# kronbichler/multigrid

Measured on AMD Instinct MI355X. Metric: DoFs/s for Laplace matvec + V-cycle, poisson_cube p=4 fp64, higher is better.
Workload: dtype f64; 1 GPU; poisson_cube FE_Q(4) 128^3 cells, 135005697 DoFs per GPU, 8 levels, step = 1 fp64 vmult + 1 V-cycle (Chebyshev degree 3, first kind); cells_per_dim=128, degree=4, n_dofs_per_gpu=135005697, global_dofs=135005697, parallelism=1 GPU

## Files before the change

### include/mgx.h

```cpp
#ifndef MGX_H
#define MGX_H

#include <stddef.h>
#include <stdint.h>

#ifdef __cplusplus
extern "C" {
#endif

#define MGX_OK 0
#define MGX_ERR_INVALID_ARGUMENT (-1)
#define MGX_ERR_NO_DEVICE (-2)
#define MGX_ERR_HIP (-3)
#define MGX_ERR_UNSUPPORTED (-4)
#define MGX_ERR_NOT_CONVERGED (-5)

#define MGX_F32 0
#define MGX_F64 1

#define MGX_INVALID_INDEX 0xFFFFFFFFu
#define MGX_MAX_DEGREE 9

typedef struct mgx_context_s  *mgx_context_t;
typedef struct mgx_operator_s *mgx_operator_t;
// ... 12 lines not shown
int mgx_device_memory_info(mgx_context_t ctx, size_t *free_bytes, size_t *total_bytes);
void *mgx_context_stream(mgx_context_t ctx);

typedef struct
{
  int   rank, size;
  void *user;
  int (*exchange)(void *user, int plan_id, int number, int n_neighbors, const int *ranks, const uint32_t *counts,
                  void *const *send, void *const *recv);
  int (*allreduce_sum)(void *user, double *values, int count);
  void *(*alloc_device)(void *user, size_t bytes);
} mgx_comm_desc;
int mgx_context_set_comm(mgx_context_t ctx, const mgx_comm_desc *comm);

#define MGX_RCCL_ID_BYTES 128
int mgx_rccl_unique_id(void *id_out);
int mgx_context_set_rccl(mgx_context_t ctx, int rank, int size, const void *id);
int mgx_context_use_rccl(mgx_context_t ctx, int enable);

typedef struct
{
  int                    plan_id;
  int                    n_neighbors;
  const int             *neighbor_rank;
  const uint32_t        *count;
  const uint32_t *const *index;
  const uint32_t        *shared;
  uint32_t               n_shared;
  const uint32_t        *not_owned;
  uint32_t               n_not_owned;
  void *const           *send_buf;
  void *const           *recv_buf;
} mgx_exchange_desc;

int mgx_profile_enable(mgx_context_t ctx, int enable);
int mgx_range_push(mgx_context_t ctx, const char *name);
int mgx_range_pop(mgx_context_t ctx);
int mgx_profile_read(mgx_context_t ctx, int form, uint64_t *launches, double *total_ms);

int mgx_malloc(mgx_context_t ctx, void **dptr, size_t bytes);
int mgx_free(mgx_context_t ctx, void *dptr);
int mgx_upload(mgx_context_t ctx, void *dptr, const void *hptr, size_t bytes);
int mgx_download(mgx_context_t ctx, void *hptr, const void *dptr, size_t bytes);
int mgx_memset_zero(mgx_context_t ctx, void *dptr, size_t bytes);
int mgx_copy_device(mgx_context_t ctx, void *dst, const void *src, size_t bytes);

int mgx_copy_cast(mgx_context_t ctx, void *dst, int dst_number, const void *src, int src_number, size_t n);
int mgx_add_cast(mgx_context_t ctx, void *dst, int dst_number, const void *src, int src_number, size_t n);
int mgx_sadd(mgx_context_t ctx, int number, void *x, double s, double a, const void *v, size_t n);
int mgx_dot(mgx_context_t ctx, int number, const void *x, const void *y, size_t n, double *result);
int mgx_l2_norm(mgx_context_t ctx, int number, const void *x, size_t n, double *result);
int mgx_operator_dot(mgx_operator_t op, const void *x, const void *y, double *result);
int mgx_operator_l2_norm(mgx_operator_t op, const void *x, double *result);
int mgx_set_entries(mgx_context_t ctx, int number, void *v, const uint32_t *idx_host,
                    const double *val_host, uint32_t count);

typedef struct
{
  int      degree;
  int      number;
  uint32_t n_cells;
  uint32_t n_dofs;
  const uint32_t *idx27;
  const uint32_t *idx27_plain;
  const uint32_t *constrained;
  uint32_t        n_constrained;
  double coef[6];
  const double *shape_values;
  const double *colloc_grad;
  const double *qweights;
  const uint8_t *brick_colour;
  const uint32_t *global_index;
  const mgx_exchange_desc *exchange;
  const double *coef_q;
} mgx_operator_desc;

int mgx_operator_create(mgx_context_t ctx, const mgx_operator_desc *desc, mgx_operator_t *op);
int mgx_operator_destroy(mgx_operator_t op);
uint32_t mgx_operator_n_dofs(mgx_operator_t op);
int mgx_operator_set_profiled(mgx_operator_t op, int profiled);
int mgx_operator_exchange_buffers(mgx_operator_t op, int k, void **send, void **recv, uint32_t *count, int *rank);
int mgx_exchange_add(mgx_operator_t op, void *vec);
int mgx_operator_number(mgx_operator_t op);
int mgx_vmult(mgx_operator_t op, void *dst, const void *src);
int mgx_compute_residual(mgx_operator_t op, void *dst, const void *src, const void *rhs_q);
int mgx_vmult_residual(mgx_operator_t op, const void *rhs, const void *lhs, void *residual);
int mgx_vmult_with_cg_update(mgx_operator_t op, double alpha, double beta, const void *r, void *q, void *p, void *x,
                             void *scratch, double sums[4]);
int mgx_compute_diagonal(mgx_operator_t op);
int mgx_get_inverse_diagonal(mgx_operator_t op, const void **dptr);

#define MGX_LAW_UNIT 0
#define MGX_LAW_MINIMAL_SURFACE 1
int mgx_operator_enable_coefficient_update(mgx_operator_t op, const double metric[6], double det_jacobian);
int mgx_operator_enable_coefficient_update_q(mgx_operator_t op, const double *unit_q, const double *jxw_q);
int mgx_evaluate_coefficient(mgx_operator_t op, int law, const void *state);
int mgx_compute_nonlinear_residual(mgx_operator_t op, int law, void *dst, const void *state);
int mgx_operator_get_coefficient(mgx_operator_t op, const void **dptr, size_t *n);

int mgx_smoother_create(mgx_operator_t op, double smoothing_range, int degree,
                        int eig_cg_n_iterations, mgx_smoother_t *smoother);
int mgx_smoother_destroy(mgx_smoother_t smoother);
typedef struct
{
  double lambda_min, lambda_max, theta, delta;
  int    degree, cg_iterations;
} mgx_smoother_info;
int mgx_smoother_get_info(mgx_smoother_t smoother, mgx_smoother_info *info);
#define MGX_CHEBYSHEV_FIRST_KIND 0
#define MGX_CHEBYSHEV_FOURTH_KIND 1
int mgx_smoother_set_polynomial_type(mgx_smoother_t smoother, int polynomial_type);
int mgx_smoother_vmult(mgx_smoother_t smoother, void *x, const void *b);
int mgx_smoother_step(mgx_smoother_t smoother, void *x, const void *b);

typedef struct
{
  const uint32_t *children;
  const double *prolong_1d;
  const uint8_t *weight_shift;
} mgx_transfer_desc;
int mgx_transfer_create(mgx_operator_t coarse, mgx_operator_t fine, const mgx_transfer_desc *desc,
                        mgx_transfer_t *transfer);
int mgx_transfer_destroy(mgx_transfer_t transfer);
int mgx_prolongate(mgx_transfer_t transfer, void *fine, const void *coarse, int add, int with_constraints);
int mgx_restrict_and_add(mgx_transfer_t transfer, void *coarse, const void *fine, int with_constraints);
int mgx_interpolate_to_coarse(mgx_transfer_t transfer, void *coarse, const void *fine);

typedef struct
{
  int n_levels;
  int degree_pre;
  int n_cycles;
  const mgx_operator_t *matrix;
  const mgx_operator_t *matrix_dp;
  const mgx_transfer_t *transfer;
  const mgx_transfer_t *transfer_dp;
  const double *const *rhs;
  const uint32_t *const *bc_index;
  const double *const   *bc_value;
  const uint32_t        *bc_count;
} mgx_solver_desc;

int mgx_solver_create(mgx_context_t ctx, const mgx_solver_desc *desc, mgx_solver_t *solver);
int mgx_solver_destroy(mgx_solver_t solver);
int mgx_solver_v_cycle(mgx_solver_t solver);
int mgx_solver_reset_smoother(mgx_solver_t solver, int level, double smoothing_range, int degree,
                              int eig_cg_n_iterations);
int mgx_solver_update_coefficient(mgx_solver_t solver, int law, const double *state_fine);
int mgx_solver_n_levels(mgx_solver_t solver);
int mgx_solver_get_operator(mgx_solver_t solver, int level, int fp64, mgx_operator_t *op);
int mgx_operator_device_indices(mgx_operator_t op, const uint32_t **idx27, uint32_t *n_cells, uint32_t *n_dofs,
                                int *degree);
int mgx_solver_set_polynomial_type(mgx_solver_t solver, int polynomial_type);
int mgx_solver_compute_rhs(mgx_solver_t solver, int level, const double *rhs_q);
int mgx_solver_solve(mgx_solver_t solver, int do_analyze, double *reduction_rate, double *trace);
typedef void (*mgx_level_hook)(void *user, int level, int stage);
int mgx_solver_solve_hooked(mgx_solver_t solver, int do_analyze, double *reduction_rate, double *trace,
                            mgx_level_hook hook, void *user);
int mgx_solver_solve_cg(mgx_solver_t solver, unsigned int *iterations, double *reduction_rate);
int mgx_solver_solve_cg_control(mgx_solver_t solver, unsigned int max_iterations, double abs_tol, double reduction,
                                unsigned int *iterations, double *reduction_rate);
int mgx_solver_cg_history(mgx_solver_t solver, double *history, int capacity, int *count);
int mgx_solver_vmult(mgx_solver_t solver, double *dst, const double *src);
int mgx_solver_set_agglomeration(mgx_solver_t solver, int level, mgx_solver_t coarse, const uint32_t *local_to_global,
                                 const uint8_t *owned, uint32_t n_local);
int mgx_solver_vmult_with_residual_update(mgx_solver_t solver, double *residual, double *update, double factor,
// ... 15 lines not shown
```

### multigrid_amd/__init__.py

```python
import ctypes as C
import os

import numpy as np

from . import _lib
from ._lib import F32, F64, INVALID_INDEX, MgxError, check

__all__ = ["Context", "DeviceVector", "Cube", "LaplaceOperator", "Chebyshev", "Transfer", "MultigridSolver",
           "Communicator", "process_grid", "F32", "F64", "INVALID_INDEX", "MgxError", "DGLaplaceOperator", "dg_cheby_mesh",
           "dg_box_neighbours", "dg_box_partition", "dg_partition", "DG_HERMITE", "DG_GAUSS_LOBATTO", "DG_GAUSS", "DGMultigridSolver",
           "spawn_ranks"]


def spawn_ranks(script, argv, n, one_gpu=False, grace=30.0):
    import os
    import socket
    import subprocess
    import sys
    import time
    with socket.socket() as sock:
        sock.bind(("127.0.0.1", 0))
        port = sock.getsockname()[1]
    procs = []
    for r in range(n):
# ... 441 lines not shown

    def rhs_quadrature(self, l):
        out = np.empty((self.n_cells(l), (self.degree + 1) ** 3))
        check(self.lib.mgx_cube_rhs_quadrature(self.h, l, out.ctypes.data_as(_lib.f64p)))
        return out

    def bc(self, l):
        n = self.lib.mgx_cube_bc_count(self.h, l)
        return self._arr("mgx_cube_bc_index", (n,), l), self._arr("mgx_cube_bc_value", (n,), l)

    def neighbors(self, l):
        out = []
        for k in range(self.lib.mgx_cube_n_neighbors(self.h, l)):
            n = self.lib.mgx_cube_neighbor_count(self.h, l, k)
            out.append((self.lib.mgx_cube_neighbor_rank(self.h, l, k),
                        self._arr("mgx_cube_neighbor_index", (n,), l, k)))
        return out

    def shared(self, l):
        return self._arr("mgx_cube_shared", (self.lib.mgx_cube_n_shared(self.h, l),), l)

    def not_owned(self, l):
        return self._arr("mgx_cube_not_owned", (self.lib.mgx_cube_n_not_owned(self.h, l),), l)

    def cells_per_dim3(self, l):
        a, b = (C.c_uint32 * 3)(), (C.c_uint32 * 3)()
        self.lib.mgx_cube_cells_per_dim3(self.h, l, C.byref(a), C.byref(b))
        return tuple(a), tuple(b)

    def l2_error_parts(self, l, solution):
        s = np.ascontiguousarray(solution, dtype=np.float64)
        e, v = C.c_double(), C.c_double()
        self.lib.mgx_cube_l2_error_parts(self.h, l, s.ctypes.data_as(_lib.f64p), C.byref(e), C.byref(v))
        return e.value, v.value

    def operator_desc(self, l, number=F64):
        d = _lib.OperatorDesc()
        check(self.lib.mgx_cube_operator_desc(self.h, l, number, C.byref(d)))
        return d

    def l2_error(self, l, solution):
        s = np.ascontiguousarray(solution, dtype=np.float64)
        assert s.size == self.n_dofs(l)
        return self.lib.mgx_cube_l2_error(self.h, l, s.ctypes.data_as(_lib.f64p))

    def seeded_vector(self, l, seed=42):
        out = np.empty(self.n_dofs(l))
        check(self.lib.mgx_cube_seeded_vector(self.h, l, seed, out.ctypes.data_as(_lib.f64p)))
        return out

    def affine_metric(self, l, jacobian=None):
        m, det = np.zeros(6), C.c_double()
        a = None if jacobian is None else np.ascontiguousarray(jacobian, dtype=np.float64).ravel()
        check(self.lib.mgx_cube_affine_metric(self.h, l, None if a is None else a.ctypes.data_as(_lib.f64p),
                                              m.ctypes.data_as(_lib.f64p), C.byref(det)))
        return m, det.value

    def unit_law_coefficient(self, l, jacobian=None):
        m, det = self.affine_metric(l, jacobian)
        w = self.qweights()
        jxw = (w[:, None, None] * w[None, :, None] * w[None, None, :]).ravel() * det
        return np.ascontiguousarray(np.broadcast_to(m[None, :, None] * jxw[None, None, :],
                                                    (self.n_cells(l), 6, jxw.size)))

    def dof_coordinates(self, l, jacobian=None):
        assert self.size == 1
        if self.shell is not None or (self.box_desc is not None and self.box_desc["geometry"] != "cartesian"):
            assert jacobian is None
            dofs = _cell_dofs(self.idx27_plain(l), self.degree)
            X = np.empty((self.n_dofs(l), 3))
            X[dofs.ravel()] = self.cell_nodes(l).transpose(0, 2, 1).reshape(-1, 3)
            return X
        p, g = self.degree, self.dof_grid(l).astype(np.int64)
        n = np.array(self.cells_per_dim3(l)[1], dtype=np.int64)
        G = n * p + 1
        ijk = np.stack([g % G[0], (g // G[0]) % G[1], g // (G[0] * G[1])], axis=1)
        cell = np.minimum(ijk // p, n[None, :] - 1)
        X = (cell + self.gll()[ijk - cell * p]) * self.cell_size(l)
        if jacobian is not None:
            X = X @ np.asarray(jacobian, dtype=np.float64).T
        return (-0.9 if self.box_desc is None else self.box_desc["origin"]) + X


def _cell_dofs(idx27, p):
    n = p + 1
    idx27 = np.asarray(idx27, dtype=np.int64).reshape(-1, 27)
    out = np.empty((idx27.shape[0], n, n, n), dtype=np.int64)
    code = [0 if a == 0 else (2 if a == p else 1) for a in range(n)]
    for k in range(n):
        for j in range(n):
            oz, oy = (k - 1 if code[k] == 1 else 0), (j - 1 if code[j] == 1 else 0)
            off = (p - 1 if code[j] == 1 else 1) * oz + oy
            for i in range(n):
                base = idx27[:, 9 * code[k] + 3 * code[j] + code[i]]
                out[:, k, j, i] = base + (off * (p - 1) + i - 1 if code[i] == 1 else off)
    return out.reshape(idx27.shape[0], n ** 3)


class LaplaceOperator:

    def __init__(self, ctx, desc=None, handle=None):
        self.ctx, self.lib = ctx, ctx.lib
        self.owned = handle is None
        if handle is None:
            h = C.c_void_p()
            check(self.lib.mgx_operator_create(ctx.h, C.byref(desc), C.byref(h)))
            self.h = h
        else:
            self.h = C.c_void_p(handle)
        self.number = self.lib.mgx_operator_number(self.h)

    @classmethod
    def from_cube(cls, ctx, cube, level, number=F64, coef_q=None):
        d = cube.operator_desc(level, number)
        if coef_q is not None:
            coef_q = np.ascontiguousarray(coef_q, dtype=np.float64)
            assert coef_q.size == cube.n_cells(level) * 6 * (cube.degree + 1) ** 3
            d.coef_q = coef_q.ctypes.data_as(_lib.f64p)
        return cls(ctx, d)

    def m(self):
        return self.lib.mgx_operator_n_dofs(self.h)

    def set_profiled(self, on=True):
        check(self.lib.mgx_operator_set_profiled(self.h, int(on)))

    def initialize_dof_vector(self):
        return DeviceVector(self.ctx, self.m(), self.number)

    def vmult(self, dst, src):
        check(self.lib.mgx_vmult(self.h, dst.ptr, src.ptr))

    def vmult_with_cg_update(self, alpha, beta, r, q, p, x):
        sums = np.zeros(4)
        check(self.lib.mgx_vmult_with_cg_update(self.h, alpha, beta, r.ptr, q.ptr, p.ptr, x.ptr, None,
                                                sums.ctypes.data_as(_lib.f64p)))
        return sums

    def vmult_residual(self, rhs, lhs, residual):
        check(self.lib.mgx_vmult_residual(self.h, rhs.ptr, lhs.ptr, residual.ptr))

    def compute_residual(self, dst, src=None, rhs_q=None):
        check(self.lib.mgx_compute_residual(self.h, dst.ptr, src.ptr if src is not None else None,
                                            rhs_q.ptr if rhs_q is not None else None))

    def compute_diagonal(self):
        check(self.lib.mgx_compute_diagonal(self.h))

    def enable_coefficient_update(self, metric, det_jacobian):
        m = np.ascontiguousarray(metric, dtype=np.float64)
        assert m.size == 6
        check(self.lib.mgx_operator_enable_coefficient_update(self.h, m.ctypes.data_as(_lib.f64p), float(det_jacobian)))

    def enable_coefficient_update_q(self, unit_q, jxw_q):
        u = np.ascontiguousarray(unit_q, dtype=np.float64)
        w = np.ascontiguousarray(jxw_q, dtype=np.float64)
        p, n = C.c_void_p(), C.c_size_t()
        check(self.lib.mgx_operator_get_coefficient(self.h, C.byref(p), C.byref(n)))
        assert u.size == n.value and 6 * w.size == n.value
        check(self.lib.mgx_operator_enable_coefficient_update_q(self.h, u.ctypes.data_as(_lib.f64p),
                                                                w.ctypes.data_as(_lib.f64p)))

    def evaluate_coefficient(self, law, state):
        check(self.lib.mgx_evaluate_coefficient(self.h, int(law), state.ptr))

    def compute_nonlinear_residual(self, law, dst, state):
        check(self.lib.mgx_compute_nonlinear_residual(self.h, int(law), dst.ptr, state.ptr))

    def get_coefficient(self):
        p, n = C.c_void_p(), C.c_size_t()
        check(self.lib.mgx_operator_get_coefficient(self.h, C.byref(p), C.byref(n)))
        return DeviceVector(self.ctx, n.value, self.number, ptr=p)

    def l2_norm(self, x):
        r = C.c_double()
        check(self.lib.mgx_operator_l2_norm(self.h, x.ptr, C.byref(r)))
        return r.value

    def get_matrix_diagonal_inverse(self):
        p = C.c_void_p()
        check(self.lib.mgx_get_inverse_diagonal(self.h, C.byref(p)))
        return DeviceVector(self.ctx, self.m(), self.number, ptr=p)

    def clear(self):
        if self.owned and self.h:
            self.lib.mgx_operator_destroy(self.h)
            self.h = None


class Chebyshev:

    POLYNOMIAL = {"first_kind": 0, "fourth_kind": 1}

    def __init__(self, op, smoothing_range=20., degree=3, eig_cg_n_iterations=15, handle=None, polynomial=None):
        self.op, self.lib = op, op.lib
        self.owned = handle is None
        if handle is None:
            h = C.c_void_p()
            check(self.lib.mgx_smoother_create(op.h, smoothing_range, degree, eig_cg_n_iterations, C.byref(h)))
            self.h = h
        else:
            self.h = C.c_void_p(handle)
        if polynomial is not None:
            self.set_polynomial_type(polynomial)

# ... 555 lines not shown
```

### multigrid_amd/_lib.py

```python
import ctypes as C
import os

_HERE = os.path.dirname(os.path.abspath(__file__))
LIB_PATH = os.environ.get("MGX_LIB_PATH") or os.path.join(_HERE, "libmgx.so")

F32, F64 = 0, 1
INVALID_INDEX = 0xFFFFFFFF

vp = C.c_void_p
u32p = C.POINTER(C.c_uint32)
f64p = C.POINTER(C.c_double)


class ExchangeDesc(C.Structure):
    _fields_ = [("plan_id", C.c_int), ("n_neighbors", C.c_int), ("neighbor_rank", C.POINTER(C.c_int)),
                ("count", u32p), ("index", C.POINTER(u32p)), ("shared", u32p), ("n_shared", C.c_uint32),
                ("not_owned", u32p), ("n_not_owned", C.c_uint32), ("send_buf", C.POINTER(vp)),
                ("recv_buf", C.POINTER(vp))]


EXCHANGE_FN = C.CFUNCTYPE(C.c_int, vp, C.c_int, C.c_int, C.c_int, C.POINTER(C.c_int), u32p, C.POINTER(vp), C.POINTER(vp))
ALLREDUCE_FN = C.CFUNCTYPE(C.c_int, vp, f64p, C.c_int)
ALLOC_FN = C.CFUNCTYPE(vp, vp, C.c_size_t)
LEVEL_HOOK_FN = C.CFUNCTYPE(None, vp, C.c_int, C.c_int)
# ... 15 lines not shown
                ("idx27", u32p), ("idx27_plain", u32p), ("constrained", u32p), ("n_constrained", C.c_uint32),
                ("coef", C.c_double * 6), ("shape_values", f64p), ("colloc_grad", f64p), ("qweights", f64p),
                ("brick_colour", C.POINTER(C.c_uint8)), ("global_index", u32p),
                ("exchange", C.POINTER(ExchangeDesc)), ("coef_q", f64p)]


class DGExchangeDesc(C.Structure):
    _fields_ = [("plan_id", C.c_int), ("n_neighbors", C.c_int), ("neighbor_rank", C.POINTER(C.c_int)),
                ("count", u32p), ("send_cells", C.POINTER(u32p)), ("recv_first", u32p)]


class DGOperatorDesc(C.Structure):
    _fields_ = [("degree", C.c_int), ("basis", C.c_int), ("number", C.c_int), ("n_cells", C.c_uint32),
                ("neighbours", C.POINTER(C.c_int32)), ("jacobian", C.c_double * 9),
                ("n_ghost_cells", C.c_uint32), ("exchange", C.POINTER(DGExchangeDesc))]


class DGSolverDesc(C.Structure):
    _fields_ = [("matrix_dg", vp), ("matrix_dg_dp", vp), ("cfe", vp), ("degree_pre", C.c_int),
                ("cell_global_id", u32p)]


class SmootherInfo(C.Structure):
    _fields_ = [("lambda_min", C.c_double), ("lambda_max", C.c_double), ("theta", C.c_double),
                ("delta", C.c_double), ("degree", C.c_int), ("cg_iterations", C.c_int)]


class TransferDesc(C.Structure):
    _fields_ = [("children", u32p), ("prolong_1d", f64p), ("weight_shift", C.POINTER(C.c_uint8))]


class SolverDesc(C.Structure):
    _fields_ = [("n_levels", C.c_int), ("degree_pre", C.c_int), ("n_cycles", C.c_int),
                ("matrix", C.POINTER(vp)), ("matrix_dp", C.POINTER(vp)),
                ("transfer", C.POINTER(vp)), ("transfer_dp", C.POINTER(vp)),
                ("rhs", C.POINTER(f64p)), ("bc_index", C.POINTER(u32p)), ("bc_value", C.POINTER(f64p)),
                ("bc_count", u32p)]


class CubeSolver(C.Structure):
    _fields_ = [("n_levels", C.c_int), ("matrix", C.POINTER(vp)), ("matrix_dp", C.POINTER(vp)),
                ("transfer", C.POINTER(vp)), ("transfer_dp", C.POINTER(vp)), ("solver", vp)]


SIGNATURES = {
    "mgx_last_error": (C.c_char_p, []),
    "mgx_version": (C.c_char_p, []),
    "mgx_context_create": (C.c_int, [C.POINTER(vp), C.c_int]),
    "mgx_context_set_option": (C.c_int, [vp, C.c_char_p, C.c_double]),
    "mgx_has_cells_form": (C.c_int, []),
    "mgx_context_destroy": (C.c_int, [vp]),
    "mgx_sync": (C.c_int, [vp]),
    "mgx_device_memory_info": (C.c_int, [vp, C.POINTER(C.c_size_t), C.POINTER(C.c_size_t)]),
    "mgx_context_stream": (vp, [vp]),
    "mgx_context_set_comm": (C.c_int, [vp, C.POINTER(CommDesc)]),
    "mgx_rccl_unique_id": (C.c_int, [vp]),
    "mgx_context_set_rccl": (C.c_int, [vp, C.c_int, C.c_int, vp]),
    "mgx_context_use_rccl": (C.c_int, [vp, C.c_int]),
    "mgx_copy_device": (C.c_int, [vp, vp, vp, C.c_size_t]),
    "mgx_operator_exchange_buffers": (C.c_int, [vp, C.c_int, C.POINTER(vp), C.POINTER(vp), u32p, C.POINTER(C.c_int)]),
    "mgx_exchange_add": (C.c_int, [vp, vp]),
    "mgx_profile_enable": (C.c_int, [vp, C.c_int]),
    "mgx_range_push": (C.c_int, [vp, C.c_char_p]),
    "mgx_range_pop": (C.c_int, [vp]),
    "mgx_profile_read": (C.c_int, [vp, C.c_int, C.POINTER(C.c_uint64), f64p]),
    "mgx_operator_set_profiled": (C.c_int, [vp, C.c_int]),
    "mgx_malloc": (C.c_int, [vp, C.POINTER(vp), C.c_size_t]),
    "mgx_free": (C.c_int, [vp, vp]),
    "mgx_upload": (C.c_int, [vp, vp, vp, C.c_size_t]),
    "mgx_download": (C.c_int, [vp, vp, vp, C.c_size_t]),
    "mgx_memset_zero": (C.c_int, [vp, vp, C.c_size_t]),
    "mgx_copy_cast": (C.c_int, [vp, vp, C.c_int, vp, C.c_int, C.c_size_t]),
    "mgx_add_cast": (C.c_int, [vp, vp, C.c_int, vp, C.c_int, C.c_size_t]),
    "mgx_sadd": (C.c_int, [vp, C.c_int, vp, C.c_double, C.c_double, vp, C.c_size_t]),
    "mgx_dot": (C.c_int, [vp, C.c_int, vp, vp, C.c_size_t, f64p]),
    "mgx_l2_norm": (C.c_int, [vp, C.c_int, vp, C.c_size_t, f64p]),
    "mgx_operator_dot": (C.c_int, [vp, vp, vp, f64p]),
    "mgx_operator_l2_norm": (C.c_int, [vp, vp, f64p]),
    "mgx_set_entries": (C.c_int, [vp, C.c_int, vp, u32p, f64p, C.c_uint32]),
    "mgx_operator_create": (C.c_int, [vp, C.POINTER(OperatorDesc), C.POINTER(vp)]),
    "mgx_operator_destroy": (C.c_int, [vp]),
    "mgx_operator_n_dofs": (C.c_uint32, [vp]),
    "mgx_operator_number": (C.c_int, [vp]),
    "mgx_vmult": (C.c_int, [vp, vp, vp]),
    "mgx_vmult_residual": (C.c_int, [vp, vp, vp, vp]),
    "mgx_compute_diagonal": (C.c_int, [vp]),
    "mgx_get_inverse_diagonal": (C.c_int, [vp, C.POINTER(vp)]),
    "mgx_smoother_create": (C.c_int, [vp, C.c_double, C.c_int, C.c_int, C.POINTER(vp)]),
    "mgx_smoother_destroy": (C.c_int, [vp]),
    "mgx_smoother_get_info": (C.c_int, [vp, C.POINTER(SmootherInfo)]),
    "mgx_smoother_vmult": (C.c_int, [vp, vp, vp]),
    "mgx_smoother_step": (C.c_int, [vp, vp, vp]),
    "mgx_transfer_create": (C.c_int, [vp, vp, C.POINTER(TransferDesc), C.POINTER(vp)]),
    "mgx_transfer_destroy": (C.c_int, [vp]),
    "mgx_prolongate": (C.c_int, [vp, vp, vp, C.c_int, C.c_int]),
    "mgx_restrict_and_add": (C.c_int, [vp, vp, vp, C.c_int]),
    "mgx_solver_create": (C.c_int, [vp, C.POINTER(SolverDesc), C.POINTER(vp)]),
    "mgx_solver_destroy": (C.c_int, [vp]),
    "mgx_solver_solve": (C.c_int, [vp, C.c_int, f64p, f64p]),
    "mgx_solver_solve_hooked": (C.c_int, [vp, C.c_int, f64p, f64p, LEVEL_HOOK_FN, vp]),
    "mgx_solver_solve_cg": (C.c_int, [vp, C.POINTER(C.c_uint), f64p]),
    "mgx_solver_cg_history": (C.c_int, [vp, f64p, C.c_int, C.POINTER(C.c_int)]),
    "mgx_solver_solve_cg_fused": (C.c_int, [vp, C.POINTER(C.c_uint), f64p]),
    "mgx_solver_vmult_with_residual_update": (C.c_int, [vp, vp, vp, C.c_double, f64p]),
    "mgx_vmult_with_cg_update": (C.c_int, [vp, C.c_double, C.c_double, vp, vp, vp, vp, vp, f64p]),
    "mgx_solver_vmult": (C.c_int, [vp, vp, vp]),
    "mgx_solver_do_matvec": (C.c_int, [vp]),
    "mgx_solver_do_matvec_smoother": (C.c_int, [vp]),
    "mgx_solver_get_solution": (C.c_int, [vp, C.c_int, C.c_int, C.POINTER(vp)]),
    "mgx_solver_get_vector": (C.c_int, [vp, C.c_int, C.c_int, C.POINTER(vp)]),
    "mgx_solver_get_smoother": (C.c_int, [vp, C.c_int, C.POINTER(vp)]),
    "mgx_solver_get_timings": (C.c_int, [vp, f64p]),
    "mgx_solver_enable_timings": (C.c_int, [vp, C.c_int]),
    "mgx_cube_create": (C.c_int, [C.c_int, C.c_int, C.c_int, C.POINTER(vp)]),
    "mgx_cube_create_numbered": (C.c_int, [C.c_int, C.c_int, C.c_int, C.c_int, C.POINTER(vp)]),
    "mgx_cube_create_box": (C.c_int, [C.POINTER(CubeBoxDesc), C.POINTER(vp)]),
    "mgx_cube_create_shell": (C.c_int, [C.c_int, C.c_int, C.c_int, C.c_int, C.POINTER(vp)]),
    "mgx_cube_create_shell_ranks": (C.c_int, [C.c_int, C.c_int, C.c_int, C.c_int, C.c_int, C.c_int, C.POINTER(vp)]),
    "mgx_cube_level_offset": (C.c_int, [vp]),
    "mgx_cube_cell_nodes": (C.c_int, [vp, C.c_int, f64p]),
    "mgx_cube_entity_multiplicity": (C.POINTER(C.c_uint8), [vp, C.c_int]),
    "mgx_cube_rank": (C.c_int, [vp]),
    "mgx_cube_size": (C.c_int, [vp]),
    "mgx_cube_cells_per_dim3": (None, [vp, C.c_int, C.POINTER(C.c_uint32 * 3), C.POINTER(C.c_uint32 * 3)]),
    "mgx_cube_n_neighbors": (C.c_int, [vp, C.c_int]),
    "mgx_cube_neighbor_rank": (C.c_int, [vp, C.c_int, C.c_int]),
    "mgx_cube_neighbor_count": (C.c_uint32, [vp, C.c_int, C.c_int]),
    "mgx_cube_neighbor_index": (u32p, [vp, C.c_int, C.c_int]),
    "mgx_cube_n_shared": (C.c_uint32, [vp, C.c_int]),
    "mgx_cube_shared": (u32p, [vp, C.c_int]),
    "mgx_cube_n_not_owned": (C.c_uint32, [vp, C.c_int]),
    "mgx_cube_not_owned": (u32p, [vp, C.c_int]),
    "mgx_cube_weight_shift": (C.POINTER(C.c_uint8), [vp, C.c_int]),
    "mgx_cube_exchange_desc": (C.c_int, [vp, C.c_int, C.c_int, C.POINTER(ExchangeDesc), C.POINTER(u32p),
                                        C.POINTER(C.c_int), u32p]),
    "mgx_cube_l2_error_parts": (None, [vp, C.c_int, f64p, f64p, f64p]),
    "mgx_cube_destroy": (C.c_int, [vp]),
    "mgx_cube_n_levels": (C.c_int, [vp]),
    "mgx_cube_degree": (C.c_int, [vp]),
    "mgx_cube_n_cells": (C.c_uint32, [vp, C.c_int]),
    "mgx_cube_n_dofs": (C.c_uint32, [vp, C.c_int]),
    "mgx_cube_n_constrained": (C.c_uint32, [vp, C.c_int]),
    "mgx_cube_cells_per_dim": (C.c_uint32, [vp, C.c_int]),
    "mgx_cube_cell_size": (C.c_double, [vp, C.c_int]),
    "mgx_cube_idx27": (u32p, [vp, C.c_int]),
    "mgx_cube_idx27_plain": (u32p, [vp, C.c_int]),
    "mgx_cube_constrained": (u32p, [vp, C.c_int]),
    "mgx_cube_children": (u32p, [vp, C.c_int]),
    "mgx_cube_cell_coords": (u32p, [vp, C.c_int]),
    "mgx_cube_dof_grid": (u32p, [vp, C.c_int]),
    "mgx_cube_shape_values": (f64p, [vp]),
    "mgx_cube_colloc_grad": (f64p, [vp]),
    "mgx_cube_qweights": (f64p, [vp]),
    "mgx_cube_qpoints": (f64p, [vp]),
    "mgx_cube_gll": (f64p, [vp]),
    "mgx_cube_prolong_1d": (f64p, [vp]),
    "mgx_cube_rhs": (f64p, [vp, C.c_int]),
    "mgx_cube_coef_q": (f64p, [vp, C.c_int]),
    "mgx_cube_jxw_q": (f64p, [vp, C.c_int]),
    "mgx_cube_bc_count": (C.c_uint32, [vp, C.c_int]),
    "mgx_cube_bc_index": (u32p, [vp, C.c_int]),
    "mgx_cube_bc_value": (f64p, [vp, C.c_int]),
    "mgx_cube_operator_desc": (C.c_int, [vp, C.c_int, C.c_int, C.POINTER(OperatorDesc)]),
    "mgx_cube_l2_error": (C.c_double, [vp, C.c_int, f64p]),
    "mgx_cube_seeded_vector": (C.c_int, [vp, C.c_int, C.c_uint64, f64p]),
    "mgx_cube_solver_create": (C.c_int, [vp, vp, C.c_int, C.c_int, C.c_int, C.POINTER(CubeSolver)]),
# ... 78 lines not shown
```

### multigrid_amd/csrc/mgx_api.cpp

```cpp
#include "../../include/mgx.h"
#include "mgx_bricks.hpp"
#include "mgx_internal.hpp"

#include <hip/hip_runtime.h>
#include <rccl/rccl.h>

#include <dlfcn.h>

#include <algorithm>
#include <chrono>
#include <cmath>
#include <cstdio>
#include <cstdlib>
#include <cstring>
#include <memory>
#include <string>
#include <type_traits>
#include <utility>
#include <vector>

using namespace mgx;

namespace
{
// ... 23 lines not shown
        return s_;        \
    }                     \
  while (0)

#define MGX_REQUIRE(cond, msg)                        \
  do                                                  \
    {                                                 \
      if (!(cond))                                    \
        return fail(MGX_ERR_INVALID_ARGUMENT, (msg)); \
    }                                                 \
  while (0)

  inline size_t number_size(int number) { return number == MGX_F64 ? 8 : 4; }

  bool g_trace = false;
  bool trace_on() { return g_trace; }
#define MGX_TRACE(...)                  \
  do                                    \
    {                                   \
      if (trace_on())                   \
        {                               \
          std::fprintf(stderr, "[mgx] " __VA_ARGS__); \
          std::fputc('\n', stderr);     \
          std::fflush(stderr);          \
        }                               \
    }                                   \
  while (0)
}

int mgx::report_error(int code, const char *message) { return fail(code, message ? message : ""); }

#ifndef MGX_CELLS_FORM
#define MGX_CELLS_FORM 0
#endif
extern "C" int mgx_has_cells_form(void) { return MGX_CELLS_FORM; }

mgx::Tunables mgx::Tunables::from_environment()
{
  Tunables t;
  auto     num = [](const char *name, uint32_t dflt) {
    const char *e = std::getenv(name);
    return e ? (uint32_t)std::strtoul(e, nullptr, 10) : dflt;
  };
  t.trace               = std::getenv("MGX_TRACE") != nullptr;
  t.brick_min           = num("MGX_BRICK_MIN", t.brick_min);
  t.brick_min_from_env  = std::getenv("MGX_BRICK_MIN") != nullptr;
  t.overlap_min         = num("MGX_OVERLAP_MIN_BRICKS", t.overlap_min);
  t.restrict_colour_min = num("MGX_RESTRICT_COLOUR_MIN", t.restrict_colour_min);
  t.cell_colour_min     = num("MGX_CELL_COLOUR_MIN", t.cell_colour_min);
  t.free_max_bricks     = num("MGX_FREE_MAX_BRICKS", t.free_max_bricks);
  t.free_one_max        = num("MGX_FREE_ONE_MAX", t.free_one_max);
  t.graph_max_dofs      = num("MGX_GRAPH_MAX_DOFS", t.graph_max_dofs);
  return t;
}

bool mgx::Tunables::set(const std::string &name, double value)
{
  const bool     on = value != 0.;
  const uint32_t u  = value <= 0. ? 0u : (value >= 4294967295. ? 0xFFFFFFFFu : (uint32_t)value);
  struct Entry
  {
    const char *name;
    bool       *flag;
    uint32_t   *number;
  };
  const Entry table[] = {
    {"trace", &trace, nullptr},
    {"brick_min", nullptr, &brick_min},
    {"overlap_min_bricks", nullptr, &overlap_min},
    {"restrict_colour_min", nullptr, &restrict_colour_min},
    {"cell_colour_min", nullptr, &cell_colour_min},
    {"free_max_bricks", nullptr, &free_max_bricks},
    {"free_one_max", nullptr, &free_one_max},
    {"graph_max_dofs", nullptr, &graph_max_dofs},
    {"general_kernel", &general_kernel, nullptr},
    {"no_bricks", &no_bricks, nullptr},
#if MGX_CELLS_FORM
    {"cells_form", &cells_form, nullptr},
    {"brick_wide_max", nullptr, &wide_max},
#endif
    {"macro_wg_per_cu_x16", nullptr, &macro_wg_x16},
    {"no_diag_table", &no_diag_table, nullptr},
    {"no_macro_v2", &no_macro_v2, nullptr},
    {"no_general_bricks", &no_general_bricks, nullptr},
    {"general_brick_min", nullptr, &general_brick_min},
    {"fused_prolong_min_bricks", nullptr, &fused_prolong_min_bricks},
    {"roctx", &roctx, nullptr},
    {"no_fused_init", &no_fused_init, nullptr},
    {"no_fused_restrict", &no_fused_restrict, nullptr},
    {"no_fused_prolong", &no_fused_prolong, nullptr},
    {"force_fused_transfers", &force_fused_transfers, nullptr},
    {"transfer_v1", &transfer_v1, nullptr},
    {"restrict_atomic", &restrict_atomic, nullptr},
    {"exchange_unfused", &exchange_unfused, nullptr},
    {"no_graph", &no_graph, nullptr},
    {"dg_no_overlap", &dg_no_overlap, nullptr},
    {"dg_unmerged_restrict", &dg_unmerged_restrict, nullptr},
    {"no_fused_decomposed", &no_fused_decomposed, nullptr},
    {"no_fused_assembly", &no_fused_assembly, nullptr},
    {"no_fused_residual", &no_fused_residual, nullptr},
    {"no_restrict_scratch", &no_restrict_scratch, nullptr},
    {"rccl_selftest", &rccl_selftest, nullptr},
  };
  for (const Entry &e : table)
    if (name == e.name)
      {
        if (e.flag)
          *e.flag = on;
        else
          *e.number = u;
        if (name == "brick_min")
          brick_min_from_env = true;
        return true;
      }
  return false;
}

struct ExchangePlan
{
  std::vector<uint32_t> not_owned_host;
  int                    plan_id = 0, number = MGX_F64, self_pos = 0;
  std::vector<int>       rank;
  std::vector<uint32_t>  count;
  std::vector<uint32_t *> index_dev;
  std::vector<void *>    send, recv;
  std::vector<uint8_t>   owns_buffers;
  uint32_t              *shared_dev = nullptr, *not_owned_dev = nullptr;
  uint32_t               n_shared = 0, n_not_owned = 0;
  void                  *own_buf = nullptr;
  std::vector<uint32_t>  start;
  uint32_t              *all_index_dev = nullptr, *csr_start_dev = nullptr, *csr_pos_dev = nullptr;
  uint8_t               *all_seg_dev = nullptr, *csr_k_dev = nullptr;
  bool                   fused = false;
};

struct RcclApi
{
  void *lib = nullptr;
  decltype(&ncclGetUniqueId)    GetUniqueId    = nullptr;
  decltype(&ncclCommInitRank)   CommInitRank   = nullptr;
  decltype(&ncclCommDestroy)    CommDestroy    = nullptr;
  decltype(&ncclGroupStart)     GroupStart     = nullptr;
  decltype(&ncclGroupEnd)       GroupEnd       = nullptr;
  decltype(&ncclSend)           Send           = nullptr;
  decltype(&ncclRecv)           Recv           = nullptr;
  decltype(&ncclAllReduce)      AllReduce      = nullptr;
  decltype(&ncclGetErrorString) GetErrorString = nullptr;
  bool load()
  {
    if (lib)
      return true;
    const char *names[] = {"librccl.so", "librccl.so.1", "/opt/rocm/lib/librccl.so.1"};
    for (const char *n : names)
      if ((lib = dlopen(n, RTLD_NOW | RTLD_NOLOAD)))
        break;
    if (!lib)
      for (const char *n : names)
        if ((lib = dlopen(n, RTLD_NOW | RTLD_GLOBAL)))
          break;
    if (!lib)
      return false;
#define MGX_RCCL_SYM(name)                                        \
  name = reinterpret_cast<decltype(name)>(dlsym(lib, "nccl" #name)); \
  if (!name)                                                      \
    {                                                             \
      lib = nullptr;                                              \
// ... 1113 lines not shown
              const int inner = (e % 3 == 1) + ((e / 3) % 3 == 1) + (e / 9 == 1);
              if (inner == 3 || (inner > 0 && pm1 == 0) || ix[e] == MGX_INVALID_INDEX)
                continue;
              mask |= used[ix[e]];
            }
          int col = 0;
          while (col < 32 && (mask >> col) & 1u)
            ++col;
          if (col == 32)
            {
              ok = false;
              break;
            }
          colour[c] = (uint8_t)col;
          ++count[col];
          n_colours = std::max(n_colours, col + 1);
          for (int e = 0; e < 27; ++e)
            {
              const int inner = (e % 3 == 1) + ((e / 3) % 3 == 1) + (e / 9 == 1);
              if (inner == 3 || (inner > 0 && pm1 == 0) || ix[e] == MGX_INVALID_INDEX)
                continue;
              used[ix[e]] |= 1u << col;
            }
        }
      if (ok)
        {
          std::vector<uint32_t> order(desc->n_cells), fill(33, 0);
          d.cell_colour_start[0] = 0;
          for (int k = 0; k < n_colours; ++k)
            d.cell_colour_start[k + 1] = d.cell_colour_start[k] + count[k];
          for (int k = 0; k < n_colours; ++k)
            fill[k] = d.cell_colour_start[k];
          for (uint32_t c = 0; c < desc->n_cells; ++c)
            order[fill[colour[c]]++] = c;
          d.n_cell_colours = n_colours;
          MGX_HIP(hipMalloc((void **)&d.cell_order, sizeof(uint32_t) * (size_t)desc->n_cells));
          MGX_HIP(hipMemcpy(d.cell_order, order.data(), sizeof(uint32_t) * (size_t)desc->n_cells, hipMemcpyHostToDevice));
          MGX_TRACE("operator_create: general branch, %u cells in %d colours", desc->n_cells, n_colours);
        }
    }
  const bool macro_covers = d.separable && (uint64_t)desc->n_dofs * number_size(d.number) < 0xFFFFFFF0ull;
  if (!tun.no_bricks && !general && (MGX_CELLS_FORM ? (p <= 4 || d.separable) : macro_covers))
    {
      BrickHost   bh;
      std::string why;
      const mgx_exchange_desc *ex = desc->exchange;
      const uint32_t brick_min   = tun.brick_min_from_env ? tun.brick_min : (p <= 2 ? 2 * tun.brick_min : tun.brick_min);
      const uint32_t brick_cells = p <= 4 ? 64u : 8u;
      const uint32_t overlap_min = tun.overlap_min;
      if (desc->n_dofs >= 0x3FFFFFFFu)
        MGX_TRACE("operator_create: per-cell kernel (%u DoFs do not fit the 30-bit entity index)", desc->n_dofs);
      else if (desc->n_cells / brick_cells < brick_min)
        MGX_TRACE("operator_create: per-cell kernel (%u bricks < %u)", desc->n_cells / brick_cells, brick_min);
      else if (build_bricks(p, desc->n_cells, desc->n_dofs, desc->idx27, desc->idx27_plain, desc->brick_colour,
                            ex ? ex->shared : nullptr, ex ? ex->n_shared : 0,
                            ex && desc->n_cells / brick_cells >= overlap_min, bh, why))
        {
          BrickData &b = d.bricks;
          b.n_bricks   = bh.n_bricks;
          b.n_colours  = bh.n_colours;
          b.n_iface_groups = bh.n_iface_groups;
          b.order      = bh.order;
          for (int c = 0; c <= bh.n_colours; ++c)
            b.colour_start[c] = bh.colour_start[c];
          for (size_t i = 0; i < bh.ent_base.size(); ++i)
            if (bh.ent_base[i] != MGX_INVALID_INDEX)
              bh.ent_base[i] |= (uint32_t)(bh.ent_flags[i] & 3u) << 30;
          MGX_HIP(hipMalloc((void **)&b.ent_base, sizeof(uint32_t) * bh.ent_base.size()));
          MGX_HIP(hipMemcpy(b.ent_base, bh.ent_base.data(), sizeof(uint32_t) * bh.ent_base.size(),
                            hipMemcpyHostToDevice));
          b.ent_flags = nullptr;
          if (d.separable)
            {
              std::vector<uint32_t> map;
              build_item_map(p, map);
              MGX_HIP(hipMalloc((void **)&b.item_map, sizeof(uint32_t) * map.size()));
              MGX_HIP(hipMemcpy(b.item_map, map.data(), sizeof(uint32_t) * map.size(), hipMemcpyHostToDevice));
              {
                std::vector<uint32_t> map2;
                build_item_map2(p, map2);
                MGX_HIP(hipMalloc((void **)&b.item_map2, sizeof(uint32_t) * map2.size()));
                MGX_HIP(hipMemcpy(b.item_map2, map2.data(), sizeof(uint32_t) * map2.size(), hipMemcpyHostToDevice));
              }
              const int n_classes = b.n_bricks <= tun.free_one_max ? 1 : 2;
              FreeHost  fh;
              if (!MGX_MACRO_PAIRS && !tun.cells_form && b.n_bricks <= tun.free_max_bricks &&
                  (uint64_t)desc->n_dofs * number_size(d.number) < 0xFFFFFFF0ull &&
                  build_free_schedule(p, bh, desc->n_dofs, ex ? ex->shared : nullptr, ex ? ex->n_shared : 0,
                                      bh.n_iface_groups > 0, n_classes, map, fh) &&
                  (size_t)b.n_bricks * fh.n_surf * number_size(d.number) < 0xFFFFFFF0ull && fh.n_groups <= 8)
                {
                  FreeSchedule &fr  = b.fr;
                  fr.n_classes      = n_classes;
                  fr.n_groups       = fh.n_groups;
                  fr.n_iface_groups = fh.n_iface_groups;
                  for (int g = 0; g <= fh.n_groups; ++g)
                    fr.group_start[g] = fh.group_start[g];
                  fr.n_surf        = fh.n_surf;
                  fr.n_surf_dofs   = (uint32_t)fh.surf_dof.size();
                  fr.n_surf_shared = fh.n_surf_shared;
                  fh.surf_dof.push_back(0);
                  fh.surf_pos.push_back(0);
                  auto up = [&](uint32_t *&dev, const std::vector<uint32_t> &v) {
                    if (hipMalloc((void **)&dev, sizeof(uint32_t) * v.size()) != hipSuccess)
                      return false;
                    return hipMemcpy(dev, v.data(), sizeof(uint32_t) * v.size(), hipMemcpyHostToDevice) == hipSuccess;
                  };
                  MGX_REQUIRE(up(fr.surf_off, fh.surf_off) && up(fr.surf_dof, fh.surf_dof) && up(fr.surf_start, fh.surf_start) &&
                                up(fr.surf_pos, fh.surf_pos),
                              "mgx_operator_create: out of device memory (reduced-colour schedule)");
                  MGX_HIP(hipMalloc(&fr.priv, (size_t)b.n_bricks * fh.n_surf * number_size(d.number) + 16));
                  MGX_REQUIRE(up(fr.ent, fh.ent), "mgx_operator_create: out of device memory (reduced-colour schedule)");
                  MGX_TRACE("operator_create: reduced-colour schedule, %d classes, %d groups, %u private values per brick, %u "
                            "private DoFs (%u shared)",
                            n_classes, fr.n_groups, fr.n_surf, fr.n_surf_dofs, fr.n_surf_shared);
                }
            }
          MGX_TRACE("operator_create: %u bricks, %d colours", b.n_bricks, b.n_colours);
        }
      else
        MGX_TRACE("operator_create: per-cell kernel (%s)", why.c_str());
    }
  if (general && p == 4 && !desc->exchange && !tun.no_bricks && !tun.no_general_bricks && desc->n_dofs < 0x3FFFFFFFu &&
      (uint64_t)desc->n_dofs * number_size(d.number) < 0xFFFFFFF0ull &&
      desc->n_cells / 64 >= tun.general_brick_min)
    {
      BrickHost   bh;
      std::string why;
      FreeHost    fh;
      std::vector<uint32_t> map;
      build_item_map(p, map);
      if (build_bricks(p, desc->n_cells, desc->n_dofs, desc->idx27, desc->idx27_plain, nullptr, nullptr, 0, false, bh, why) &&
          build_free_schedule(p, bh, desc->n_dofs, nullptr, 0, false, 1, map, fh) && fh.n_groups == 1 &&
          (size_t)bh.n_bricks * fh.n_surf * number_size(d.number) < 0xFFFFFFF0ull)
        {
          BrickData &g = d.gbricks;
          g.n_bricks   = bh.n_bricks;
          FreeSchedule &fr = g.fr;
          fr.n_classes = 1;
          fr.n_groups  = 1;
          fr.group_start[0] = 0;
          fr.group_start[1] = bh.n_bricks;
          fr.n_surf        = fh.n_surf;
          fr.n_surf_dofs   = (uint32_t)fh.surf_dof.size();
          fr.n_surf_shared = 0;
          fh.surf_dof.push_back(0);
          fh.surf_pos.push_back(0);
          auto up = [&](uint32_t *&dev, const std::vector<uint32_t> &v) {
            if (hipMalloc((void **)&dev, sizeof(uint32_t) * v.size()) != hipSuccess)
              return false;
            return hipMemcpy(dev, v.data(), sizeof(uint32_t) * v.size(), hipMemcpyHostToDevice) == hipSuccess;
          };
          MGX_REQUIRE(up(g.order_dev, bh.order) && up(g.item_map, map) && up(fr.surf_off, fh.surf_off) && up(fr.surf_dof, fh.surf_dof) &&
                        up(fr.surf_start, fh.surf_start) && up(fr.surf_pos, fh.surf_pos) && up(fr.ent, fh.ent),
                      "mgx_operator_create: out of device memory (brick schedule of the general operator)");
          MGX_HIP(hipMalloc(&fr.priv, (size_t)bh.n_bricks * fh.n_surf * number_size(d.number) + 16));
          MGX_TRACE("operator_create: general branch on %u bricks, %u private values per brick, %u private DoFs", bh.n_bricks,
                    fr.n_surf, fr.n_surf_dofs);
        }
      else
        MGX_TRACE("operator_create: general branch without bricks (%s)", why.c_str());
    }
  {
    const size_t     n3 = (size_t)n * n * n, n_local = n3 * desc->n_cells;
    if (!d.bricks.available() && !d.cell_order && n_local <= kAssemblyMaxEntries)
      {
// ... 158 lines not shown
                  }
                cnt[j]++;
              }
          if (ok)
            {
              std::vector<uint32_t> cs(e.n_shared + 1, 0);
              for (uint32_t j = 0; j < e.n_shared; ++j)
                cs[j + 1] = cs[j] + cnt[j] + 1;
              std::vector<uint8_t>  ck(cs.back() + 1, 0);
              std::vector<uint32_t> cp(cs.back() + 1, 0), fill(cs.begin(), cs.end() - 1);
              for (int k = 0; k <= e.n_neighbors; ++k)
                {
                  if (k == P->self_pos)
                    for (uint32_t j = 0; j < e.n_shared; ++j)
                      ck[fill[j]++] = 255;
                  if (k < e.n_neighbors)
                    for (uint32_t i = 0; i < e.count[k]; ++i)
                      {
                        const uint32_t j = slot[e.index[k][i]];
                        ck[fill[j]]   = (uint8_t)k;
                        cp[fill[j]++] = i;
                      }
                }
              MGX_HIP(hipMalloc((void **)&P->all_index_dev, sizeof(uint32_t) * all_index.size()));
              MGX_HIP(hipMalloc((void **)&P->all_seg_dev, all_seg.size()));
              MGX_HIP(hipMalloc((void **)&P->csr_start_dev, sizeof(uint32_t) * cs.size()));
              MGX_HIP(hipMalloc((void **)&P->csr_k_dev, ck.size()));
              MGX_HIP(hipMalloc((void **)&P->csr_pos_dev, sizeof(uint32_t) * cp.size()));
              MGX_HIP(hipMemcpy(P->all_index_dev, all_index.data(), sizeof(uint32_t) * all_index.size(), hipMemcpyHostToDevice));
              MGX_HIP(hipMemcpy(P->all_seg_dev, all_seg.data(), all_seg.size(), hipMemcpyHostToDevice));
              MGX_HIP(hipMemcpy(P->csr_start_dev, cs.data(), sizeof(uint32_t) * cs.size(), hipMemcpyHostToDevice));
              MGX_HIP(hipMemcpy(P->csr_k_dev, ck.data(), ck.size(), hipMemcpyHostToDevice));
              MGX_HIP(hipMemcpy(P->csr_pos_dev, cp.data(), sizeof(uint32_t) * cp.size(), hipMemcpyHostToDevice));
              P->fused = true;
            }
        }
      ctx->plans.push_back({(size_t)desc->n_dofs, P.get()});
      op->plan = std::move(P);
    }
  *out = op.release();
  return MGX_OK;
}

int mgx_operator_exchange_buffers(mgx_operator_t op, int k, void **send, void **recv, uint32_t *count, int *rank)
{
  MGX_REQUIRE(op && op->plan && k >= 0 && k < (int)op->plan->rank.size(), "mgx_operator_exchange_buffers: bad argument");
  if (send)
    *send = op->plan->send[k];
  if (recv)
    *recv = op->plan->recv[k];
  if (count)
    *count = op->plan->count[k];
  if (rank)
    *rank = op->plan->rank[k];
  return MGX_OK;
}

int mgx_exchange_add(mgx_operator_t op, void *vec)
{
  MGX_REQUIRE(op && vec, "mgx_exchange_add: null argument");
  return exchange_add(op, vec);
}

int mgx_operator_destroy(mgx_operator_t op)
{
  if (!op)
    return MGX_OK;
  (void)hipStreamSynchronize(op->ctx->stream);
  (void)hipFree(op->d.idx27);
  (void)hipFree(op->d.idx27_plain);
  (void)hipFree(op->d.constrained);
  (void)hipFree(op->d.basis);
  (void)hipFree(op->d.inv_diag);
  (void)hipFree(op->d.coef_q);
  (void)hipFree(op->d.grad_1d);
  (void)hipFree(op->d.cell_order);
  (void)hipFree(op->d.asm_start);
  (void)hipFree(op->d.asm_pos);
  (void)hipFree(op->d.cell_scratch);
  (void)hipFree(op->d.bricks.ent_base);
  (void)hipFree(op->d.bricks.ent_flags);
  (void)hipFree(op->d.bricks.item_map);
  (void)hipFree(op->d.bricks.item_map2);
  (void)hipFree(op->d.bricks.fr.ent);
  (void)hipFree(op->d.bricks.fr.surf_off);
  (void)hipFree(op->d.bricks.fr.priv);
  (void)hipFree(op->d.bricks.fr.surf_dof);
  (void)hipFree(op->d.bricks.fr.surf_start);
  (void)hipFree(op->d.bricks.fr.surf_pos);
  (void)hipFree(op->d.gbricks.item_map);
  (void)hipFree(op->d.gbricks.order_dev);
  (void)hipFree(op->d.gbricks.fr.ent);
  (void)hipFree(op->d.gbricks.fr.surf_off);
  (void)hipFree(op->d.gbricks.fr.priv);
  (void)hipFree(op->d.gbricks.fr.surf_dof);
  (void)hipFree(op->d.gbricks.fr.surf_start);
  (void)hipFree(op->d.gbricks.fr.surf_pos);
  (void)hipFree(op->d.diag_items);
  (void)hipFree(op->d.diag_items2);
  (void)hipFree(op->cg_partials);
  (void)hipFree(op->cg_result);
  (void)hipFree(op->cg_carrier);
  (void)hipFree(op->unit_q);
  (void)hipFree(op->jxw_q);
  (void)hipFree(op->global_index_dev);
  if (op->plan)
    {
      ExchangePlan *P = op->plan.get();
      auto         &v = op->ctx->plans;
      v.erase(std::remove_if(v.begin(), v.end(), [P](const std::pair<size_t, ExchangePlan *> &x) { return x.second == P; }),
              v.end());
      for (size_t k = 0; k < P->rank.size(); ++k)
        {
          (void)hipFree(P->index_dev[k]);
          if (P->owns_buffers[k])
            {
              (void)hipFree(P->send[k]);
              (void)hipFree(P->recv[k]);
            }
        }
      (void)hipFree(P->shared_dev);
      (void)hipFree(P->not_owned_dev);
      (void)hipFree(P->own_buf);
      (void)hipFree(P->all_index_dev);
      (void)hipFree(P->all_seg_dev);
      (void)hipFree(P->csr_start_dev);
      (void)hipFree(P->csr_k_dev);
      (void)hipFree(P->csr_pos_dev);
    }
  delete op;
  return MGX_OK;
}

uint32_t mgx_operator_n_dofs(mgx_operator_t op) { return op ? op->d.n_dofs : 0; }

int mgx_operator_set_profiled(mgx_operator_t op, int profiled)
{
  MGX_REQUIRE(op, "mgx_operator_set_profiled: null operator");
  op->profiled = profiled != 0;
  return MGX_OK;
}
int      mgx_operator_number(mgx_operator_t op) { return op ? op->d.number : -1; }

int mgx_vmult(mgx_operator_t op, void *dst, const void *src)
{
  MGX_REQUIRE(op && dst && src, "mgx_vmult: null argument");
  MGX_REQUIRE(dst != src, "mgx_vmult: dst and src must not alias (laplace_operator.h:573-601)");
  hipStream_t s = op->ctx->stream;
  bool identity_done = false;
  MGX_TRY(apply_plain(op, dst, src, true, &identity_done));
  if (!identity_done)
    launch_constrained_copy(s, op->d.number, dst, src, op->d.constrained, op->d.n_constrained);
  MGX_HIP(hipGetLastError());
  return MGX_OK;
}

int mgx_vmult_residual(mgx_operator_t op, const void *rhs, const void *lhs, void *res)
{
  MGX_REQUIRE(op && rhs && lhs && res, "mgx_vmult_residual: null argument");
  MGX_REQUIRE(res != lhs && res != rhs, "mgx_vmult_residual: residual must not alias rhs/lhs");
  hipStream_t s = op->ctx->stream;
  if (op->d.bricks.available())
    {
      const bool fr = op->d.bricks.fr.available();
      MGX_TRY(brick_loop_with_exchange(
        op, 1, res,
        [&](hipStream_t st, int g0, int g1) {
          launch_brick_loop(st, op->d, 1, lhs, rhs, nullptr, res, res, 0., 0., nullptr, 0., nullptr, nullptr, g0, g1, fr);
        },
        [&](hipStream_t st) {
          launch_list_residual(st, op->d.number, res, rhs, op->plan->shared_dev, op->plan->n_shared);
        },
        fr,
        [&](hipStream_t st, uint32_t first, uint32_t count) {
          launch_surf_finish(st, op->d, 1, first, count, res, lhs, res, rhs, nullptr, nullptr, 0., 0., 0.);
        }));
    }
  else
    {
      MGX_TRY(apply_plain(op, res, lhs));
      launch_rhs_minus(s, op->d.number, res, rhs, op->d.n_dofs);
    }
  launch_constrained_residual(s, op->d.number, res, rhs, lhs, op->d.constrained, op->d.n_constrained);
  MGX_HIP(hipGetLastError());
  return MGX_OK;
}

int mgx_vmult_with_cg_update(mgx_operator_t op, double alpha, double beta, const void *r, void *q, void *p, void *x,
                             void *scratch, double sums[4])
{
  MGX_REQUIRE(op && r && q && p && x && sums, "mgx_vmult_with_cg_update: null argument");
  MGX_REQUIRE(q != p && q != x && p != x && r != q && r != p && r != x, "mgx_vmult_with_cg_update: vectors must not alias");
  mgx_context_t ctx = op->ctx;
  hipStream_t   s   = ctx->stream;
  const int     num = op->d.number;
  const size_t  n   = op->d.n_dofs;
  constexpr uint32_t kCapacity = 1u << 16;
  if (!op->cg_partials)
    {
      MGX_HIP(hipMalloc((void **)&op->cg_partials, sizeof(double) * 4 * kCapacity));
      MGX_HIP(hipMalloc((void **)&op->cg_result, sizeof(double) * 4));
    }
  bool fused = op->d.bricks.available() && op->d.separable && op->d.bricks.item_map && !op->plan;
  if (fused)
    {
      void *carrier = scratch;
      if (!carrier)
        {
          if (!op->cg_carrier)
            MGX_HIP(hipMalloc(&op->cg_carrier, number_size(num) * n));
          carrier = op->cg_carrier;
        }
      uint32_t used = 0;
      {
        ProfileBracket pb(op, 8);
        fused = num == MGX_F64 ? launch_macro_cg_update_f64(s, op->d, alpha, beta, r, q, p, x, carrier, op->cg_partials,
                                                            kCapacity - 2048, &used)
                               : launch_macro_cg_update_f32(s, op->d, alpha, beta, r, q, p, x, carrier, op->cg_partials,
                                                            kCapacity - 2048, &used);
      }
      if (fused)
        {
          used += launch_cg_list_update(s, num, op->d.constrained, op->d.n_constrained, alpha, beta, r, q, p, x,
                                        op->cg_partials + 4 * (size_t)used);
          launch_reduce4(s, op->cg_partials, used, nullptr, op->cg_result);
// ... 207 lines not shown
      MGX_HIP(hipMemsetAsync(dst, 0, number_size(op->d.number) * op->d.n_dofs, s));
      launch_cell_nl_residual(s, op->d, ms, op->metric, op->det_jacobian, op->unit_q, op->jxw_q, dst, state, op->d.cell_order, op->d.cell_colour_start,
                              op->d.n_cell_colours);
    }
  else
    return fail(MGX_ERR_UNSUPPORTED, "mgx_compute_nonlinear_residual: the level has neither cell colours nor the ordered-assembly "
                                     "tables (more than 32 colours): no reproducible assembly");
  MGX_HIP(hipGetLastError());
  return MGX_OK;
}

int mgx_compute_diagonal(mgx_operator_t op)
{
  MGX_REQUIRE(op, "mgx_compute_diagonal: null argument");
  hipStream_t s = op->ctx->stream;
  const int   n = op->d.p + 1;
  double a1d[kMaxN], m1d[kMaxN];
  for (int i = 0; i < n; ++i)
    {
      double a = 0, m = 0;
      for (int q = 0; q < n; ++q)
        {
          double g = 0;
          for (int r = 0; r < n; ++r)
            g += op->D[q * n + r] * op->S[r * n + i];
          a += op->w[q] * g * g;
          m += op->w[q] * op->S[q * n + i] * op->S[q * n + i];
        }
      a1d[i] = a;
      m1d[i] = m;
    }
  MGX_HIP(hipMemsetAsync(op->d.inv_diag, 0, number_size(op->d.number) * op->d.n_dofs, s));
  if (op->d.bricks.available())
    {
      std::vector<uint32_t> lists, list_start;
      brick_cell_lists(op, lists, list_start);
      uint32_t *lists_dev = nullptr;
      MGX_HIP(hipMalloc((void **)&lists_dev, sizeof(uint32_t) * (lists.size() + 1)));
      MGX_HIP(hipMemcpyAsync(lists_dev, lists.data(), sizeof(uint32_t) * lists.size(), hipMemcpyHostToDevice, s));
      launch_cell_diagonal(s, op->d, op->d.inv_diag, a1d, m1d, lists_dev, list_start.data(), (int)list_start.size() - 1);
      MGX_HIP(hipStreamSynchronize(s));
      MGX_HIP(hipFree(lists_dev));
    }
  else if (op->d.cell_order)
    launch_cell_diagonal(s, op->d, op->d.inv_diag, a1d, m1d, op->d.cell_order, op->d.cell_colour_start, op->d.n_cell_colours);
  else
    launch_cell_diagonal(s, op->d, op->d.inv_diag, a1d, m1d);
  MGX_TRY(exchange_add(op, op->d.inv_diag));
  launch_constrained_set(s, op->d.number, op->d.inv_diag, 1.0, op->d.constrained, op->d.n_constrained);
  launch_invert(s, op->d.number, op->d.inv_diag, op->d.n_dofs);
  MGX_HIP(hipGetLastError());
  op->has_diag = true;
  for (int which = 0; which < 2; ++which)
    {
      void          *&slot = which == 0 ? op->d.diag_items : op->d.diag_items2;
      const uint32_t *map  = which == 0 ? op->d.bricks.item_map : op->d.bricks.item_map2;
      if (slot)
        {
          MGX_HIP(hipFree(slot));
          slot = nullptr;
        }
      if (!map || !op->d.separable || op->ctx->tun.no_diag_table)
        continue;
      const uint32_t nb = op->d.p <= 4 ? 4 : 2, g = nb * op->d.p + 1, npts = g * g * g;
      void          *table = nullptr;
      uint32_t      *flag  = nullptr, mismatch = 1;
      MGX_HIP(hipMalloc(&table, number_size(op->d.number) * npts));
      MGX_HIP(hipMalloc((void **)&flag, sizeof(uint32_t)));
      MGX_HIP(hipMemsetAsync(table, 0, number_size(op->d.number) * npts, s));
      MGX_HIP(hipMemsetAsync(flag, 0, sizeof(uint32_t), s));
      if (op->d.number == MGX_F64)
        macro_diag_table_f64(s, op->d, map, table, flag);
      else
        macro_diag_table_f32(s, op->d, map, table, flag);
      MGX_HIP(hipMemcpyAsync(&mismatch, flag, sizeof(uint32_t), hipMemcpyDeviceToHost, s));
      MGX_HIP(hipStreamSynchronize(s));
      MGX_HIP(hipFree(flag));
      if (mismatch == 0)
        slot = table;
      else
        MGX_HIP(hipFree(table));
      if (which == 0)
        MGX_TRACE("compute_diagonal: diagonal %s per brick item", mismatch == 0 ? "uniform" : "not uniform");
    }
  return MGX_OK;
}

int mgx_get_inverse_diagonal(mgx_operator_t op, const void **dptr)
{
  MGX_REQUIRE(op && dptr, "mgx_get_inverse_diagonal: null argument");
  MGX_REQUIRE(op->has_diag, "mgx_get_inverse_diagonal: call mgx_compute_diagonal first");
  *dptr = op->d.inv_diag;
  return MGX_OK;
}

int mgx_smoother_create(mgx_operator_t op, double smoothing_range, int degree, int eig_cg_n_iterations,
                        mgx_smoother_t *out)
{
  MGX_REQUIRE(op && out, "mgx_smoother_create: null argument");
  MGX_REQUIRE(eig_cg_n_iterations > 2, "mgx_smoother_create: eig_cg_n_iterations must be > 2");
  if (!op->has_diag)
    MGX_TRY(mgx_compute_diagonal(op));
  mgx_context_t ctx = op->ctx;
  hipStream_t   s   = ctx->stream;
  const int     num = op->d.number;
  const size_t  n   = op->d.n_dofs, bytes = number_size(num) * n;
  std::unique_ptr<mgx_smoother_s, int (*)(mgx_smoother_t)> sm(new mgx_smoother_s, mgx_smoother_destroy);
  sm->op            = op;
  sm->req_range     = smoothing_range;
  sm->req_degree    = degree;
  sm->req_eig_its   = eig_cg_n_iterations;
  MGX_HIP(hipMalloc(&sm->x_old, bytes));
  MGX_HIP(hipMalloc(&sm->tmp, bytes));
  void *r = nullptr, *z = nullptr, *d = nullptr, *h = sm->tmp, *x = sm->x_old;
  struct Scratch
  {
    void *&a, *&b, *&c;
    ~Scratch()
    {
      (void)hipFree(a);
      (void)hipFree(b);
      (void)hipFree(c);
    }
  } scratch{r, z, d};
  MGX_HIP(hipMalloc(&r, bytes));
  MGX_HIP(hipMalloc(&z, bytes));
  MGX_HIP(hipMalloc(&d, bytes));
  {
    double sc[2] = {op->start_sum, op->start_count};
    MGX_TRY(comm_allreduce(ctx, sc, 2));
    launch_index_mod11(s, num, r, op->global_index_dev, sc[0] / sc[1], n);
  }
  MGX_HIP(hipMemsetAsync(x, 0, bytes, s));
  std::vector<double> diag, off;
  double              res = 0, rz = 0, rz_old = 0, alpha = 0, alpha_old = 0, beta = 0;
  MGX_TRY(dot(ctx, num, r, r, n, &res, op->plan.get()));
  res    = std::sqrt(res);
  int it = 0;
  MGX_TRACE("smoother_create: n=%zu eig_its=%d res0=%g", n, eig_cg_n_iterations, res);
  while (it < eig_cg_n_iterations && res > 1e-10)
    {
      ++it;
      rz_old = rz;
      launch_jacobi_dot(s, num, z, op->d.inv_diag, r, n, ctx->partial_dev, ctx->result_dev);
      if (ctx->has_comm)
        MGX_TRY(dot(ctx, num, r, z, n, &rz, op->plan.get()));
      else
        MGX_TRY(read_result(ctx, &rz));
      if (it > 1)
        {
          beta = rz / rz_old;
          launch_xpby(s, num, d, z, beta, n);
        }
      else
        launch_copy_cast(s, d, num, z, num, n);
      alpha_old = alpha;
      MGX_TRY(mgx_vmult(op, h, d));
      double dh = 0;
      MGX_TRY(dot(ctx, num, d, h, n, &dh, op->plan.get()));
      alpha = rz / dh;
      launch_cg_update(s, num, x, r, d, h, alpha, n, ctx->partial_dev, ctx->result_dev);
      if (ctx->has_comm)
        MGX_TRY(dot(ctx, num, r, r, n, &res, op->plan.get()));
      else
        MGX_TRY(read_result(ctx, &res));
      res = std::sqrt(res);
// ... 1839 lines not shown
```

### multigrid_amd/csrc/mgx_bricks.cpp

```cpp
#include "mgx_bricks.hpp"

#include <omp.h>

#include <algorithm>
#include <array>
#include <cstring>
#include <parallel/algorithm>

namespace mgx
{
  namespace
  {
    constexpr uint32_t kInvalid    = 0xFFFFFFFFu;
    constexpr int      kMaxColours = 32;
    constexpr uint32_t kUnset      = 0xFFFFFFFEu;

    inline int compact3(int m)
    {
      return (m & 1) | ((m >> 2) & 2);
    }

    struct SurfaceRef
    {
      uint32_t key;
// ... 458 lines not shown
      for (int m = 0; m < NB * NB * NB; ++m)
        {
          const int bx = compact3(m), by = compact3(m >> 1), bz = compact3(m >> 2);
          for (int j = 0; j < 8; ++j)
            {
              const int  cx = 1 + (j & 1), cy = 1 + ((j >> 1) & 1), cz = 1 + (j >> 2);
              const int  nx = cx == 1 ? p - 1 : 1, ny = cy == 1 ? p - 1 : 1, nz = cz == 1 ? p - 1 : 1;
              ItemEntity e;
              e.slot = ((2 * bz + cz) * E1 + 2 * by + cy) * E1 + 2 * bx + cx;
              for (int kl = 0; kl < nx * ny * nz; ++kl)
                {
                  const int ox = kl % nx, oy = (kl / nx) % ny, oz = kl / (nx * ny);
                  const int lx = cx == 1 ? 1 + ox : p, ly = cy == 1 ? 1 + oy : p, lz = cz == 1 ? 1 + oz : p;
                  e.pnt.push_back(((bz * p + lz) * G + by * p + ly) * G + bx * p + lx);
                }
              if (!e.pnt.empty())
                ents.push_back(e);
            }
        }
      for (int ez = 0; ez < E1; ++ez)
        for (int ey = 0; ey < E1; ++ey)
          for (int ex = 0; ex < E1; ++ex)
            {
              if (ex != 0 && ey != 0 && ez != 0)
                continue;
              const int  nx = (ex & 1) ? p - 1 : 1, ny = (ey & 1) ? p - 1 : 1, nz = (ez & 1) ? p - 1 : 1;
              ItemEntity e;
              e.slot = (ez * E1 + ey) * E1 + ex;
              for (int kl = 0; kl < nx * ny * nz; ++kl)
                {
                  const int ox = kl % nx, oy = (kl / nx) % ny, oz = kl / (nx * ny);
                  const int gx = (ex / 2) * p + ((ex & 1) ? 1 + ox : 0), gy = (ey / 2) * p + ((ey & 1) ? 1 + oy : 0),
                            gz = (ez / 2) * p + ((ez & 1) ? 1 + oz : 0);
                  e.pnt.push_back((gz * G + gy) * G + gx);
                }
              if (!e.pnt.empty())
                ents.push_back(e);
            }
    }
  }

  void build_item_map(int p, std::vector<uint32_t> &map)
  {
    const int               NB = p <= 4 ? 4 : 2, G = NB * p + 1;
    std::vector<ItemEntity> ents;
    enumerate_item_entities(p, ents);
    map.clear();
    map.reserve((size_t)G * G * G);
    if (MGX_MACRO_PAIRS)
      {
        for (const ItemEntity &e : ents)
          for (size_t k = 0; k + 1 < e.pnt.size(); k += 2)
            {
              map.push_back(item_word(e.slot, e.pnt[k], (int)k));
              map.push_back(item_word(e.slot, e.pnt[k + 1], (int)k + 1));
            }
        for (const ItemEntity &e : ents)
          if (e.pnt.size() % 2)
            map.push_back(item_word(e.slot, e.pnt.back(), (int)e.pnt.size() - 1));
      }
    else
      for (const ItemEntity &e : ents)
        for (size_t k = 0; k < e.pnt.size(); ++k)
          map.push_back(item_word(e.slot, e.pnt[k], (int)k));
  }

  void build_item_map2(int p, std::vector<uint32_t> &map)
  {
    const int               NB = p <= 4 ? 4 : 2, G = NB * p + 1, E1 = 2 * NB + 1;
    std::vector<ItemEntity> ents;
    enumerate_item_entities(p, ents);
    auto on_surface = [&](int slot) {
      const int ex = slot % E1, ey = (slot / E1) % E1, ez = slot / (E1 * E1);
      return ex == 0 || ex == E1 - 1 || ey == 0 || ey == E1 - 1 || ez == 0 || ez == E1 - 1;
    };
    map.clear();
    map.reserve((size_t)G * G * G);
    for (int pass = 0; pass < 2; ++pass)
      for (const ItemEntity &e : ents)
        if ((int)on_surface(e.slot) == pass)
          for (size_t k = 0; k < e.pnt.size(); ++k)
            map.push_back(item_word(e.slot, e.pnt[k], (int)k));
  }
}
```

### multigrid_amd/csrc/mgx_bricks.hpp

```cpp
#pragma once

#include <cstdint>
#include <string>
#include <vector>

namespace mgx
{
  struct BrickHost
  {
    uint32_t              n_bricks  = 0;
    int                   n_colours = 0;
    int                   n_iface_groups = 0;
    int                   n_entities = 729;
    std::vector<uint32_t> colour_start;
    std::vector<uint32_t> ent_base;
    std::vector<uint8_t>  ent_flags;
    std::vector<uint32_t> order;
  };

  bool build_bricks(int p, uint32_t n_cells, uint32_t n_dofs, const uint32_t *idx27, const uint32_t *idx27_plain,
                    const uint8_t *colour_hint, const uint32_t *shared, uint32_t n_shared, bool split_interface,
                    BrickHost &out, std::string &why);

  struct FreeHost
  {
    int                   n_groups = 0, n_iface_groups = 0;
    std::vector<uint32_t> group_start;
    std::vector<uint32_t> ent;
    std::vector<uint32_t> surf_off;
    uint32_t              n_surf = 0;
    std::vector<uint32_t> surf_dof, surf_start, surf_pos;
    uint32_t              n_surf_shared = 0;
  };
  bool build_free_schedule(int p, const BrickHost &bh, uint32_t n_dofs, const uint32_t *shared, uint32_t n_shared,
                           bool split_interface, int n_classes, const std::vector<uint32_t> &item_map, FreeHost &out);

#ifndef MGX_MACRO_PAIRS
#define MGX_MACRO_PAIRS 0
#endif
  void build_item_map(int p, std::vector<uint32_t> &map);
  void build_item_map2(int p, std::vector<uint32_t> &map);
}
```

### multigrid_amd/csrc/mgx_internal.hpp

```cpp
#pragma once

#include <hip/hip_runtime.h>

#include <cstddef>
#include <cstdint>
#include <string>
#include <vector>

struct mgx_context_s;

namespace mgx
{
  constexpr int      kMaxN    = 10;
  constexpr uint32_t kInvalid = 0xFFFFFFFFu;

  struct Tunables
  {
    bool     trace            = false;
    bool     general_kernel   = false;
    bool     no_bricks        = false;
    uint32_t brick_min        = 512;
    bool     brick_min_from_env = false;
    uint32_t overlap_min      = 16384;
    bool     cells_form       = false;
    uint32_t wide_max         = 1024;
    bool     dg_no_overlap    = false;
    bool     no_restrict_scratch = false;
    bool     no_fused_residual = false;
    bool     no_fused_assembly = false;
    bool     no_fused_decomposed = false;
    bool     dg_unmerged_restrict = false;
    uint32_t macro_wg_x16     = 0;
    bool     no_diag_table    = false;
    bool     roctx            = false;
    uint32_t fused_prolong_min_bricks = 8192;
    bool     no_general_bricks = false;
    uint32_t general_brick_min = 2048;
    bool     no_macro_v2      = false;
    bool     no_fused_init    = false;
    bool     no_fused_restrict = false;
    bool     no_fused_prolong = false;
    bool     force_fused_transfers = false;
    bool     transfer_v1      = false;
    bool     restrict_atomic  = false;
    uint32_t restrict_colour_min = 16384;
    bool     exchange_unfused = false;
    uint32_t cell_colour_min  = 0xFFFFFFFFu;
    uint32_t free_max_bricks  = 16384;
    uint32_t free_one_max     = 1024;
    bool     no_graph         = false;
    uint32_t graph_max_dofs   = 600000;
    bool     rccl_selftest    = false;
    static Tunables from_environment();
    bool            set(const std::string &name, double value);
  };

  template <typename T>
  struct EOMat
  {
    T ee[(kMaxN / 2) * (kMaxN / 2)];
    T eo[(kMaxN / 2) * (kMaxN / 2)];
    T mc[kMaxN / 2];
    T mhh;
  };

  template <typename T>
  struct Basis1D
  {
    T S[kMaxN * kMaxN];
    T D[kMaxN * kMaxN];
    T w[kMaxN];
    T P1[2 * kMaxN * kMaxN];
    EOMat<T> mass, lapl;
    T P1eo[2 * kMaxN * kMaxN];
  };

  struct FreeSchedule
  {
    int       n_classes = 0;
    int       n_groups = 0, n_iface_groups = 0;
    uint32_t  group_start[9] = {0};
    uint32_t *ent         = nullptr;
    uint32_t *surf_off    = nullptr;
    uint32_t  n_surf      = 0;
    void     *priv        = nullptr;
    uint32_t *surf_dof    = nullptr, *surf_start = nullptr, *surf_pos = nullptr;
    uint32_t  n_surf_dofs = 0, n_surf_shared = 0;
    bool      available() const { return ent != nullptr; }
  };

  struct BrickData
  {
    uint32_t  n_bricks  = 0;
    int       n_colours = 0;
    int       n_iface_groups = 0;
    uint32_t  colour_start[33] = {0};
    uint32_t *ent_base  = nullptr;
    uint8_t  *ent_flags = nullptr;
    uint32_t *item_map  = nullptr;
    uint32_t *item_map2 = nullptr;
    std::vector<uint32_t> order;
    uint32_t *order_dev = nullptr;
    bool      available() const { return n_bricks > 0; }
    FreeSchedule fr;
  };
  constexpr int kBrickEntities = 729;
  constexpr int kMaxColours    = 32;

  struct OperatorData
  {
    int       p        = 0;
    int       number   = 1;
    uint32_t  n_cells  = 0;
    uint32_t  n_dofs   = 0;
    uint32_t  n_constrained = 0;
    uint32_t *idx27         = nullptr;
    uint32_t *idx27_plain   = nullptr;
    uint32_t *constrained   = nullptr;
    void     *basis         = nullptr;
    void     *inv_diag      = nullptr;
    double    coef[6]       = {0, 0, 0, 0, 0, 0};
    bool      full_tensor   = false;
    void     *coef_q        = nullptr;
    void     *grad_1d       = nullptr;
    uint32_t *cell_order    = nullptr;
    int       n_cell_colours = 0;
    uint32_t  cell_colour_start[33] = {0};
    uint32_t *asm_start     = nullptr;
    uint32_t *asm_pos       = nullptr;
    void     *cell_scratch  = nullptr;
    BrickData bricks;
    BrickData gbricks;
    bool      cells_form    = false;
    uint32_t  wide_max      = 1024;
    uint32_t  macro_wg_x16  = 0;
    bool      separable     = true;
    void     *diag_items    = nullptr;
    void     *diag_items2   = nullptr;
    bool      macro_v2      = true;
  };

  struct TransferData
  {
    const OperatorData *coarse = nullptr, *fine = nullptr;
    uint32_t           *children = nullptr;
    uint8_t            *weight_shift = nullptr;
    uint32_t           *own27 = nullptr;
    uint32_t           *patch = nullptr;
    uint32_t           *coarse_blocks = nullptr;
    void               *coarse_scratch = nullptr;
    uint32_t           *cs_start = nullptr, *cs_pos = nullptr;
    uint32_t           *ifr_cdof = nullptr, *ifr_start = nullptr, *ifr_fdof = nullptr;
    void               *ifr_w = nullptr;
    uint32_t            n_ifr = 0;
    uint32_t           *ifp_start = nullptr, *ifp_cdof = nullptr;
    void               *ifp_w = nullptr;
    uint32_t            n_ifp = 0;
    mutable uint32_t    pipe_grid[4] = {0, 0, 0, 0};
    bool                owner_weights = false;
    bool                coarse_coloured = false;
    uint32_t            n_cus = 256;
    uint32_t            colour_min = 16384;
  };

  int  exchange_buffers(struct ::mgx_context_s *ctx, int plan_id, int number, int n_neighbors, const int *ranks,
                        const uint32_t *counts, void *const *send, void *const *recv, hipStream_t stream = nullptr);
  hipStream_t side_stream_begin(struct ::mgx_context_s *ctx);
  int         side_stream_end(struct ::mgx_context_s *ctx);
  int  allreduce_sum(struct ::mgx_context_s *ctx, double *values, int count);
  int  dot_owned_prefix(struct ::mgx_context_s *ctx, int number, const void *x, const void *y, size_t n, double *out);
  bool context_has_comm(struct ::mgx_context_s *ctx);
  const Tunables &context_tunables(struct ::mgx_context_s *ctx);

  int report_error(int code, const char *message);

  void launch_prolongate_pipe(hipStream_t s, const TransferData &t, void *fine, const void *coarse, bool add,
                              bool with_constraints);
  void launch_restrict_add_pipe(hipStream_t s, const TransferData &t, void *coarse, const void *fine,
                                bool with_constraints);

  struct ChebPost
  {
    void       *x_old;
    const void *b, *dinv;
    double      f1, f2;
    bool        three_term;
  };
  void launch_cell_loop(hipStream_t s, const OperatorData &op, void *dst, const void *src, const void *tail_src = nullptr,
                        uint32_t n_head = 0,
                        const ChebPost *post = nullptr);
  void launch_general_bricks(hipStream_t s, const OperatorData &op, void *dst, const void *src);
  void launch_assemble(hipStream_t s, const OperatorData &op, int mode, void *dst, const void *tail_src, uint32_t n_head);
  void launch_brick_loop(hipStream_t s, const OperatorData &op, int mode, const void *src, const void *a,
                         const void *b, void *out, void *partial, double f1, double f2, const void *old = nullptr,
                         double f0 = 0., void *coarse = nullptr, const uint32_t *coarse_blocks = nullptr,
                         int group_begin = 0, int group_end = -1, bool free_schedule = false);
  void launch_cell_residual(hipStream_t s, const OperatorData &op, void *dst, const void *src, const void *rhs_q,
                            const uint32_t *lists = nullptr, const uint32_t *list_start = nullptr, int n_lists = 0);
  void launch_cell_nl_residual(hipStream_t s, const OperatorData &op, bool minimal_surface, const double *metric, double det,
                               const void *unit_q, const void *jxw_q, void *dst, const void *src, const uint32_t *lists = nullptr,
                               const uint32_t *list_start = nullptr, int n_lists = 0);
  void launch_evaluate_coefficient(hipStream_t s, const OperatorData &op, void *coef_q, int coef_number, bool minimal_surface,
                                   const double *metric, double det, const void *unit_q, const void *jxw_q, const void *state);
  void launch_interpolate_to_coarse(hipStream_t s, const TransferData &t, const void *r1d, const uint32_t *own_c, void *coarse,
                                    const void *fine);
  void launch_surf_finish(hipStream_t s, const OperatorData &op, int mode, uint32_t first, uint32_t count, void *carrier,
                          const void *x, void *out, const void *a, const void *dinv, const void *old, double f1, double f2,
                          double f0, const uint32_t *constrained = nullptr, uint32_t n_constrained = 0,
                          const FreeSchedule *schedule = nullptr);
  bool launch_macro_loop_f64(hipStream_t s, const OperatorData &op, int mode, const void *src, const void *a,
                             const void *b, void *out, void *partial, double f1, double f2, const void *old,
                             double f0, void *coarse, const uint32_t *coarse_blocks, int group_begin, int group_end,
                             bool free_schedule);
  bool launch_macro_loop_f32(hipStream_t s, const OperatorData &op, int mode, const void *src, const void *a,
                             const void *b, void *out, void *partial, double f1, double f2, const void *old,
                             double f0, void *coarse, const uint32_t *coarse_blocks, int group_begin, int group_end,
                             bool free_schedule);
  bool launch_macro_cg_update_f64(hipStream_t s, const OperatorData &op, double alpha, double beta, const void *r, void *q,
                                  void *p, void *x, void *carrier, double *partials, uint32_t capacity,
                                  uint32_t *n_partials);
  bool launch_macro_cg_update_f32(hipStream_t s, const OperatorData &op, double alpha, double beta, const void *r, void *q,
// ... 95 lines not shown
```

### multigrid_amd/csrc/mgx_macro.hip

```cpp
#include "mgx_macro_device.hpp"

#include <hip/hip_runtime.h>

#include <algorithm>
#include <cstdlib>

#ifndef MGX_MACRO_CHUNK
#define MGX_MACRO_CHUNK (MGX_MACRO_PAIRS ? 3 : 4)
#endif
#ifndef MGX_MACRO_CHUNK_CHEB
#define MGX_MACRO_CHUNK_CHEB (MGX_MACRO_PAIRS ? 2 : 3)
#endif
#ifndef MGX_MACRO_T
#define MGX_MACRO_T double
#endif

#ifdef MGX_MACRO_STAMPS
#ifndef MGX_MACRO_STAMP_MODE
#define MGX_MACRO_STAMP_MODE -1
#endif
__device__ unsigned long long g_mgx_stamps[8192 * 16];
#define MGX_STAMP(k)                                                                    \
  do                                                                                    \
    {                                                                                   \
      if (threadIdx.x == 0 && blockIdx.x < 8192 && (MGX_MACRO_STAMP_MODE < 0 || MODE == MGX_MACRO_STAMP_MODE)) \
        g_mgx_stamps[blockIdx.x * 16 + (k)] = ((k) == 15 || (k) == 13) ? __builtin_amdgcn_s_memrealtime() \
                                                        : __builtin_amdgcn_s_memtime();  \
    }                                                                                   \
  while (0)
extern "C" int mgx_debug_read_stamps(unsigned long long *host, int n_blocks)
{
  return (int)hipMemcpyFromSymbol(host, HIP_SYMBOL(g_mgx_stamps), sizeof(unsigned long long) * 16 * n_blocks);
}
#define MGX_STAMP_IT(k)      \
  do                         \
    {                        \
      if (mgx_iter == 3)     \
        MGX_STAMP(k);        \
    }                        \
  while (0)
#define MGX_STAMP_NEXT() ++mgx_iter
#define mgx_iter_is(k) (mgx_iter == (k))
#else
#define MGX_STAMP(k) ((void)0)
#define MGX_STAMP_IT(k) ((void)0)
#define MGX_STAMP_NEXT() ((void)0)
#define mgx_iter_is(k) false
#endif

namespace mgx
{
  template <int P, typename T, int MODE, bool DTAB, bool FREE = false>
  __global__ void __launch_bounds__((MCfg<P, T>::THREADS), (MCfg<P, T>::MINW))
    brick_macro_kernel(const T *__restrict__ src, uint32_t brick_first, uint32_t brick_count,
                       const uint32_t *__restrict__ ent_base, const uint32_t *__restrict__ item_map,
                       const Basis1D<T> *__restrict__ B, T c0, T c1, T c2, BrickPost<T> post, uint32_t vec_bytes)
  {
    using C              = MCfg<P, T>;
    constexpr int G      = C::G;
    constexpr int NT     = C::THREADS;
    constexpr int IT     = C::IT;
    constexpr int LINES  = C::LINES;
    constexpr int NEW    = (C::NE + NT - 1) / NT;
    constexpr int N = P + 1, NB = C::NB;
    constexpr int REM    = LINES - NT;
    constexpr bool kKeepX = is_cheb_mode(MODE) || MODE == kCgUpdate;
    constexpr int  NG     = ((MODE == kChebInit && !DTAB) || MODE == kCgUpdate) ? 2 : 1;
    __shared__ T U[C::ASZ];
    __shared__ T W[C::ASZ];

    const int tid = threadIdx.x;
    uint32_t  b   = blockIdx.x;
    if (b >= brick_count)
      return;
    MGX_STAMP(0);
    MGX_STAMP(15);
#ifdef MGX_MACRO_STAGGER
    if (__builtin_amdgcn_s_getreg(6 | (0 << 6) | ((8 - 1) << 11)) != 0)
      for (int i = 0; i < MGX_MACRO_STAGGER; ++i)
        __builtin_amdgcn_s_sleep(64);
#endif
    constexpr int NP = C::NPAIR, NS = C::NSINGLE, JP = C::JP, JS = C::JS, NU = JP + JS;
    auto live_p = [&](int j) { return (j + 1) * NT <= NP || tid + j * NT < NP; };
    auto live_s = [&](int j) { return (j + 1) * NT <= NS || tid + j * NT < NS; };
    auto live   = [&](int v) { return v < 2 * JP ? live_p(v / 2) : live_s(v - 2 * JP); };
    uint32_t mw[IT];
#pragma unroll
    for (int j = 0; j < JP; ++j)
      {
        const int     q = tid + j * NT;
        const u32x2_t m = reinterpret_cast<const u32x2_t *>(item_map)[q < NP ? q : 0];
        mw[2 * j]       = m.x;
        mw[2 * j + 1]   = m.y;
      }
#pragma unroll
    for (int j = 0; j < JS; ++j)
      {
        const int q    = tid + j * NT;
        mw[2 * JP + j] = item_map[2 * NP + (q < NS ? q : 0)];
      }
    T dv[DTAB ? IT : 1];
    if (DTAB)
      {
#pragma unroll
        for (int j = 0; j < JP; ++j)
          {
            const int q                = tid + j * NT;
            dv[DTAB ? 2 * j : 0]       = post.b[2 * (q < NP ? q : 0)];
            dv[DTAB ? 2 * j + 1 : 0]   = post.b[2 * (q < NP ? q : 0) + 1];
          }
#pragma unroll
        for (int j = 0; j < JS; ++j)
          {
            const int q               = tid + j * NT;
            dv[DTAB ? 2 * JP + j : 0] = post.b[2 * NP + (q < NS ? q : 0)];
          }
      }
    const rsrc_t      rsrc = make_rsrc(src, vec_bytes);
    const PostRsrc<T> R{make_rsrc(post.a, vec_bytes),   make_rsrc(post.b, vec_bytes),       make_rsrc(post.old, vec_bytes),
                        make_rsrc(post.out, vec_bytes), make_rsrc(post.partial, vec_bytes), rsrc,
                        make_rsrc((MODE == kCgUpdate || MODE == kChebFirstProlong) ? post.src_w : post.out, vec_bytes),
                        make_rsrc(MODE == kCgUpdate ? post.x_w : post.out, vec_bytes),
                        make_rsrc(FREE ? (const void *)post.priv : (const void *)post.out, FREE ? post.priv_bytes : vec_bytes)};
    double cg[4] = {0., 0., 0., 0.};
    const EOMat<T>   &M = B->mass, &K = B->lapl;

    uint32_t ec[NEW], en[NEW];
    uint32_t sc[FREE ? NEW : 1];
    if (FREE)
      {
#pragma unroll
        for (int j = 0; j < NEW; ++j)
          {
            const int i      = tid + j * NT;
            sc[FREE ? j : 0] = post.surf_off[i < C::NE ? i : 0];
          }
      }
    auto table_load = [&](uint32_t brick, uint32_t(&e)[NEW]) {
#pragma unroll
      for (int j = 0; j < NEW; ++j)
        {
          const int i = tid + j * NT;
          e[j]        = ent_base[(size_t)(brick_first + brick) * C::NE + (i < C::NE ? i : 0)];
        }
    };
    auto table_store = [&](uint32_t *E, const uint32_t(&e)[NEW]) {
#pragma unroll
      for (int j = 0; j < NEW; ++j)
        if (tid + j * NT < C::NE)
          E[tid + j * NT] = e[j];
    };
    auto unit_offset = [&](uint32_t w, uint32_t m, int it = 0, uint32_t brick = 0) {
#ifdef MGX_MACRO_CONTIG
      return w != kInvalid ? ((brick_first + brick) * (uint32_t)(C::NB * C::NB * C::NB * P * P * P) + (uint32_t)(tid + it * NT)) * (uint32_t)sizeof(T) : kOob;
#else
      return w != kInvalid ? (ent_index(w) + item_offset(m)) * (uint32_t)sizeof(T) : kOob;
#endif
    };
    constexpr bool kProlong = MODE == kChebFirstProlong;
    constexpr int  CNP = (C::NB / 2) * P + 1, NCV = CNP * CNP * CNP / NT + 1, CE3 = (C::NB + 1) * (C::NB + 1) * (C::NB + 1);
    T              cvv[NCV];
    T    g[NG][IT];
    uint32_t cw[NCV];
    auto coarse_words = [&](uint32_t brick) {
      if (kProlong)
        {
          const uint32_t *ctab = post.coarse_blocks + (size_t)(brick_first + brick) * CE3;
#pragma unroll
          for (int k = 0; k < NCV; ++k)
            {
              const int l = tid + k * NT;
              int       slot = 0, pnt;
              uint32_t  off;
              if (l < CNP * CNP * CNP)
                coarse_point<P>(l, slot, off, pnt);
              cw[k] = ctab[slot];
            }
        }
    };
    auto coarse_values = [&]() {
      if (kProlong)
        {
#pragma unroll
          for (int k = 0; k < NCV; ++k)
            {
              const int l = tid + k * NT;
              cvv[k]      = T(0);
              if (l < CNP * CNP * CNP)
                {
                  int      slot, pnt;
                  uint32_t off;
                  coarse_point<P>(l, slot, off, pnt);
                  const uint32_t w = cw[k];
                  const T        v = post.coarse[w != kInvalid ? w + off : 0u];
                  cvv[k]           = w != kInvalid ? v : T(0);
                }
            }
        }
    };
    auto gather_issue = [&](const uint32_t *E, uint32_t brick) {
      const rsrc_t r0 = MODE == kChebInit ? (DTAB ? R.a : R.b) : rsrc;
      const rsrc_t r1 = MODE == kCgUpdate ? R.b : R.a;
#pragma unroll
      for (int j = 0; j < JP; ++j)
        {
#pragma unroll
          for (int e = 0; e < 2; ++e)
            g[0][2 * j + e] = g[NG - 1][2 * j + e] = T(0);
          if (live_p(j))
            {
              const uint32_t off = unit_offset(E[item_slot(mw[2 * j])], mw[2 * j], 2 * j, brick);
              buf_ld2(r0, off, g[0][2 * j], g[0][2 * j + 1]);
              if (NG == 2)
                buf_ld2(r1, off, g[NG - 1][2 * j], g[NG - 1][2 * j + 1]);
            }
        }
#pragma unroll
      for (int j = 0; j < JS; ++j)
        {
          const int v = 2 * JP + j;
          g[0][v] = g[NG - 1][v] = T(0);
          if (live_s(j))
            {
              const uint32_t off = unit_offset(E[item_slot(mw[v])], mw[v], v, brick);
              g[0][v]            = buf_ld(r0, off, T());
              if (NG == 2)
                g[NG - 1][v] = buf_ld(r1, off, T());
            }
        }
    };
    T    xs[kKeepX ? IT : 1];
    auto gather_land = [&]() {
#pragma unroll
      for (int it = 0; it < IT; ++it)
        {
          T v = g[0][it];
          if (MODE == kChebInit)
            v = DTAB ? post.f0 * dv[DTAB ? it : 0] * g[0][it] : post.f0 * g[0][it] * g[NG - 1][it];
          if (MODE == kCgUpdate)
            v = post.f1 == T(0) ? g[NG - 1][it] : post.f2 * g[0][it] + g[NG - 1][it];
          if (live(it))
            U[item_point(mw[it])] = v;
          if (kKeepX)
            xs[it] = v;
        }
    };

    auto interpolate = [&]() {
      if (kProlong)
        {
          lds_barrier();
          prolong_brick<P, T, NT>(tid, W, B->P1eo, cvv);
        }
    };
    auto add_correction = [&]() {
      if (kProlong)
        {
#pragma unroll
          for (int it = 0; it < IT; ++it)
            if (live(it))
              {
                const uint32_t pnt = item_point(mw[it]);
                xs[kKeepX ? it : 0] += W[pnt];
                U[pnt] = xs[kKeepX ? it : 0];
              }
        }
    };

    table_load(b, ec);
    table_store(reinterpret_cast<uint32_t *>(W), ec);
    __syncthreads();
    MGX_STAMP(1);
    gather_issue(reinterpret_cast<const uint32_t *>(W), b);
    coarse_words(b);
    coarse_values();
    interpolate();
    gather_land();
    add_correction();
    MGX_STAMP(2);
    __syncthreads();

#ifdef MGX_MACRO_STAMPS
    int mgx_iter = 0;
#endif
    for (;;)
      {
        if (mgx_iter_is(4))
          MGX_STAMP(11);
        const uint32_t bn       = b + gridDim.x;
        const bool     has_next = bn < brick_count;
        MGX_STAMP_IT(3);
        if (has_next)
          {
            table_load(bn, en);
            coarse_words(bn);
          }
#pragma unroll
        for (int it = 0; it < IT; ++it)
          asm volatile("" : "+v"(mw[it]));
        if (DTAB && (MODE == kChebInit || MODE == kChebOldInit))
          {
#pragma unroll
            for (int it = 0; it < IT; ++it)
              asm volatile("" : "+v"(dv[DTAB ? it : 0]));
          }
#ifndef MGX_MACRO_NOSWEEP
        if (kSlicedSweeps<P, MODE>)
          brick_sweeps_sliced<P, T>(
            tid, U, W, B, c0, c1, c2, [&](int i) { MGX_STAMP_IT(4 + i); }, [&]() { __syncthreads(); });
        else
          {
        if (tid < LINES)
          {
            const int l = tid;
            T         in[G], t1[G], k1[G];
#pragma unroll
            for (int j = 0; j < G; ++j)
              in[j] = U[l * G + j];
            macro_apply2<P, T>(M, K, in, t1, k1);
#pragma unroll
            for (int j = 0; j < G; ++j)
              {
                W[l * G + j] = t1[j];
                U[l * G + j] = k1[j];
              }
          }
        if (REM > 0 && tid < REM * NB)
          {
            const int l = NT + tid / NB, c = tid % NB, base = l * G + c * P;
            T         seg[N], y[N], z[N];
#pragma unroll
            for (int i = 0; i < N; ++i)
              seg[i] = U[base + i];
            cell_apply2<P, T>(M, K, seg, y, z);
            const T yn = next_lane(y[0]), zn = next_lane(z[0]);
            if (c + 1 < NB)
              {
                y[P] += yn;
                z[P] += zn;
              }
#pragma unroll
            for (int i = 1; i < N; ++i)
              {
                W[base + i] = y[i];
                U[base + i] = z[i];
// ... 52 lines not shown
            for (int j = 0; j < G; ++j)
              W[base + j * G] = t2[j];
#pragma unroll
            for (int j = 0; j < G; ++j)
              a[j] = U[base + j * G];
            macro_apply<P, T>(M, a, t2);
#pragma unroll
            for (int j = 0; j < G; ++j)
              U[base + j * G] = fma(c0, t2[j], c1 * s2[j]);
          }
        __syncthreads();
        MGX_STAMP_IT(5);
        if (REM > 0 && tid < REM * NB)
          {
            const int l = NT + tid / NB, c = tid % NB, base = l + c * P * (G * G);
            T         seg[N], y[N], r[N];
#pragma unroll
            for (int i = 0; i < N; ++i)
              seg[i] = W[base + i * (G * G)];
            cell_apply<P, T>(K, seg, r);
#pragma unroll
            for (int i = 0; i < N; ++i)
              seg[i] = U[base + i * (G * G)];
            cell_apply<P, T>(M, seg, y);
#pragma unroll
            for (int i = 0; i < N; ++i)
              y[i] = fma(c2, r[i], y[i]);
            const T yn = next_lane(y[0]);
            if (c + 1 < NB)
              y[P] += yn;
#pragma unroll
            for (int i = 1; i < N; ++i)
              W[base + i * (G * G)] = y[i];
            if (c == 0)
              W[base] = y[0];
          }
        if (tid < LINES)
          {
            const int l = tid;
            T         a[G], r[G], o[G];
#pragma unroll
            for (int j = 0; j < G; ++j)
              a[j] = W[l + j * (G * G)];
            macro_apply<P, T>(K, a, r);
#pragma unroll
            for (int j = 0; j < G; ++j)
              a[j] = U[l + j * (G * G)];
            macro_apply<P, T>(M, a, o);
#pragma unroll
            for (int j = 0; j < G; ++j)
              W[l + j * (G * G)] = fma(c2, r[j], o[j]);
          }
          }
#endif
        __syncthreads();
        MGX_STAMP_IT(6);
        uint32_t *ebase = reinterpret_cast<uint32_t *>(U), *E2 = ebase + C::NE;
        table_store(ebase, ec);
        if (has_next)
          table_store(E2, en);
        const uint32_t *sbase = ebase + 2 * C::NE;
        if (FREE)
          {
#pragma unroll
            for (int j = 0; j < NEW; ++j)
              if (tid + j * NT < C::NE)
                ebase[2 * C::NE + tid + j * NT] = sc[FREE ? j : 0];
          }
        __syncthreads();
        constexpr bool kPipeGather = (MODE != kChebInit || DTAB) && MODE != kCgUpdate && MODE != kChebFirstProlong;
        if (has_next && kPipeGather)
          gather_issue(E2, bn);
        if (has_next)
          coarse_values();
        MGX_STAMP_IT(7);

        {
          constexpr int kChunk = MODE == kPlain ? NU : (MODE == kResidual ? (NU + 1) / 2 : (kKeepX ? MGX_MACRO_CHUNK_CHEB : MGX_MACRO_CHUNK)),
                        NCH    = (NU + kChunk - 1) / kChunk;
          PostOps<T>    ops[2][kChunk];
          uint32_t      iw[2][kChunk];
          uint32_t      pw[2][FREE ? kChunk : 1];
          const uint32_t priv0 = FREE ? (brick_first + b) * post.n_surf : 0u;
          auto slot0 = [&](int u) { return u < JP ? 2 * u : JP + u; };
          auto ulive = [&](int u) { return u < JP ? live_p(u) : live_s(u - JP); };
          auto issue = [&](int c, PostOps<T>(&o)[kChunk], uint32_t(&w)[kChunk], uint32_t(&pv)[FREE ? kChunk : 1]) {
#pragma unroll
            for (int j = 0; j < kChunk; ++j)
              {
                const int u = c * kChunk + j;
                w[j]        = kInvalid;
                if (u < NU && ulive(u))
                  w[j] = ebase[item_slot(mw[slot0(u)])];
                if (FREE)
                  {
                    const uint32_t so = (u < NU && ulive(u)) ? sbase[item_slot(mw[slot0(u < NU ? u : 0)])] : kInvalid;
                    const bool     vd = w[j] != kInvalid;
                    if (vd && so != kInvalid)
                      w[j] = ent_index(w[j]) | 0x40000000u;
                    pv[FREE ? j : 0] = (vd && so != kInvalid)
                                         ? (priv0 + so + item_offset(mw[slot0(u < NU ? u : 0)])) * (uint32_t)sizeof(T)
                                         : kOob;
                  }
              }
#pragma unroll
            for (int j = 0; j < kChunk; ++j)
              {
                const int u = c * kChunk + j;
                if (u < JP)
                  post_issue<T, MODE, DTAB, true>(R, w[j], unit_offset(w[j], mw[slot0(u < NU ? u : 0)], slot0(u < NU ? u : 0), b), o[j]);
                else if (u < NU)
                  post_issue<T, MODE, DTAB, false>(R, w[j], unit_offset(w[j], mw[slot0(u < NU ? u : 0)], slot0(u < NU ? u : 0), b), o[j]);
              }
          };
          issue(0, ops[0], iw[0], pw[0]);
#pragma unroll
          for (int c = 0; c < NCH; ++c)
            {
              if (c + 1 < NCH)
                issue(c + 1, ops[(c + 1) & 1], iw[(c + 1) & 1], pw[(c + 1) & 1]);
              __builtin_amdgcn_sched_barrier(0);
              T val[kChunk][2];
#pragma unroll
              for (int j = 0; j < kChunk; ++j)
                {
                  const int u = c * kChunk + j;
                  val[j][0] = val[j][1] = T(0);
                  if (u < NU && ulive(u))
                    {
                      val[j][0] = W[item_point(mw[slot0(u)])];
                      if (u < JP)
                        val[j][1] = W[item_point(mw[slot0(u) + 1])];
                    }
                }
#pragma unroll
              for (int j = 0; j < kChunk; ++j)
                {
                  const int u = c * kChunk + j;
                  if (u < NU)
                    {
                      const int         v0   = slot0(u);
                      const bool        pair = u < JP;
                      const uint32_t    w    = iw[c & 1][j];
                      const bool        vld  = w != kInvalid, last = vld && (w >> 31);
                      const uint32_t    off  = unit_offset(w, mw[v0], v0, b);
                      const PostOps<T> &o    = ops[c & 1][j];
                      T                 res[2];
#pragma unroll
                      for (int e = 0; e < 2; ++e)
                        res[e] = (e == 0 || pair)
                                   ? post_finish<T, MODE>(post, o.pv[e], o.av[e], o.ov[e], DTAB ? dv[DTAB ? v0 + e : 0] : o.bv[e],
                                                          last, val[j][e], xs[kKeepX ? v0 + e : 0])
                                   : T(0);
                      constexpr int kStAux = (MODE == kPlain || MODE == kResidual) ? kAuxNt : 0;
                      auto          st     = [&](rsrc_t r, uint32_t f) {
                        if (pair)
                          buf_st2(r, f, res[0], res[1]);
                        else
                          buf_st<kStAux>(r, f, res[0]);
                      };
                      if (MODE == kResidualRestrict)
                        {
                          if (ulive(u))
                            {
                              W[item_point(mw[v0])] = vld ? res[0] : T(0);
                              if (pair)
                                W[item_point(mw[v0 + 1])] = vld ? res[1] : T(0);
                            }
                        }
                      else if (MODE == kCgUpdate)
                        {
                          st(R.out, last ? off : kOob);
                          if (__builtin_amdgcn_ballot_w64(vld && !last) != 0)
                            st(R.partial, last ? kOob : off);
                          const T xn = o.ov[0] + post.f1 * o.bv[0];
                          buf_st(R.srcw, last ? off : kOob, xs[kKeepX ? v0 : 0]);
                          if (post.f1 != T(0))
                            buf_st(R.xw, last ? off : kOob, xn);
                          if (last)
                            {
                              const double qv = (double)res[0], pn = (double)xs[kKeepX ? v0 : 0], rv = (double)o.av[0];
                              cg[0] += qv * pn;
                              cg[1] += rv * rv;
                              cg[2] += qv * rv;
                              cg[3] += qv * qv;
                            }
                        }
                      else
                        {
                          st(R.out, last ? off : kOob);
                          if (FREE)
                            {
                              const uint32_t po = pw[c & 1][FREE ? j : 0];
                              if (__builtin_amdgcn_ballot_w64(po != kOob) != 0)
                                st(R.priv, po);
                              if (__builtin_amdgcn_ballot_w64(vld && !last && po == kOob) != 0)
                                st(R.partial, (last || po != kOob) ? kOob : off);
                            }
#ifndef MGX_MACRO_NOCARRIER
                          else if (__builtin_amdgcn_ballot_w64(vld && !last) != 0)
                            st(R.partial, last ? kOob : off);
#endif
                          if (MODE == kChebFirstProlong)
                            buf_st(R.srcw, last ? off : kOob, xs[kKeepX ? v0 : 0]);
                        }
                    }
                }
              __builtin_amdgcn_sched_barrier(0);
            }
        }
        MGX_STAMP_IT(8);
        if (MODE == kResidualRestrict)
          {
            constexpr int CE1 = C::NB + 1;
            __syncthreads();
            const uint32_t *ctab = post.coarse_blocks + (size_t)(brick_first + b) * (CE1 * CE1 * CE1);
            if (post.coarse_scratch)
              restrict_brick<P, T, NT, true>(tid, W, B->P1eo, nullptr, ctab,
                                             post.coarse_scratch + (size_t)(brick_first + b) * (CNP * CNP * CNP));
            else
              restrict_brick<P, T, NT, false>(tid, W, B->P1eo, post.coarse, ctab);
          }
        if (!has_next)
          break;
        if (!kPipeGather)
          gather_issue(E2, bn);
        __syncthreads();
#pragma unroll
        for (int j = 0; j < NEW; ++j)
          ec[j] = en[j];
        interpolate();
        gather_land();
        add_correction();
        MGX_STAMP_IT(9);
        __syncthreads();
        MGX_STAMP_IT(10);
        b = bn;
        MGX_STAMP_NEXT();
      }
    if (MODE == kCgUpdate)
      {
        static_assert(MODE != kCgUpdate || !MGX_MACRO_PAIRS, "kCgUpdate is written for single items");
        __syncthreads();
        double *red = reinterpret_cast<double *>(U);
#pragma unroll
        for (int k = 0; k < 4; ++k)
          red[k * NT + tid] = cg[k];
        __syncthreads();
        constexpr int P2 = NT <= 64 ? 64 : (NT <= 128 ? 128 : (NT <= 256 ? 256 : 512));
        for (int stride = P2 / 2; stride > 0; stride >>= 1)
// ... 2 lines not shown
              {
#pragma unroll
                for (int k = 0; k < 4; ++k)
                  red[k * NT + tid] += red[k * NT + tid + stride];
              }
            __syncthreads();
          }
        if (tid < 4)
          post.sums[blockIdx.x * 4 + tid] = red[tid * NT];
      }
#ifdef MGX_MACRO_STAMPS
    asm volatile("s_waitcnt vmcnt(0)" ::: "memory");
    MGX_STAMP(14);
    MGX_STAMP(13);
#endif
  }

  static uint32_t macro_cus(const OperatorData &op)
  {
    static const int cus = [] {
      int dev = 0, n = 256;
      if (hipGetDevice(&dev) == hipSuccess)
        (void)hipDeviceGetAttribute(&n, hipDeviceAttributeMultiprocessorCount, dev);
      return std::max(1, n);
    }();
    return op.macro_wg_x16 ? std::max<uint32_t>(1u, (uint32_t)cus * op.macro_wg_x16 / 16u) : (uint32_t)cus;
  }

  template <int P, typename T, int MODE>
  static void macro_launch_free(hipStream_t s, const OperatorData &op, const T *src, const BrickPost<T> &post_in, int g0, int g1)
  {
    using C             = MCfg<P, T>;
    const FreeSchedule &fr = op.bricks.fr;
    BrickPost<T>        post = post_in;
    post.priv       = (T *)fr.priv;
    post.surf_off   = fr.surf_off;
    post.n_surf     = fr.n_surf;
    post.priv_bytes = (uint32_t)((size_t)op.bricks.n_bricks * fr.n_surf * sizeof(T));
    constexpr bool kUsesDiag = is_cheb_mode(MODE);
    if (kUsesDiag && op.diag_items)
      post.b = (const T *)op.diag_items;
    for (int g = g0; g < g1; ++g)
      {
        const uint32_t first = fr.group_start[g], count = fr.group_start[g + 1] - first;
        if (count == 0)
          continue;
        const uint32_t grid = std::min<uint32_t>(count, (uint32_t)(op.macro_wg_x16 ? 1 : C::WGS) * macro_cus(op));
        if (kUsesDiag && op.diag_items)
          hipLaunchKernelGGL((brick_macro_kernel<P, T, MODE, kUsesDiag, true>), dim3(grid), dim3(C::THREADS), 0, s, src, first,
                             count, fr.ent, op.bricks.item_map, (const Basis1D<T> *)op.basis, (T)op.coef[0], (T)op.coef[1],
                             (T)op.coef[2], post, (uint32_t)(op.n_dofs * sizeof(T)));
        else
          hipLaunchKernelGGL((brick_macro_kernel<P, T, MODE, false, true>), dim3(grid), dim3(C::THREADS), 0, s, src, first,
                             count, fr.ent, op.bricks.item_map, (const Basis1D<T> *)op.basis, (T)op.coef[0], (T)op.coef[1],
                             (T)op.coef[2], post, (uint32_t)(op.n_dofs * sizeof(T)));
      }
  }

  template <int P, typename T, int MODE>
  static void macro_launch(hipStream_t s, const OperatorData &op, const T *src, const BrickPost<T> &post, int g0, int g1,
                           bool free_schedule = false)
  {
    using C             = MCfg<P, T>;
    const BrickData &bd = op.bricks;
    if (free_schedule)
      {
        if constexpr (MODE <= kChebOldInit)
          return macro_launch_free<P, T, MODE>(s, op, src, post, g0, g1);
      }
    const bool one_launch = MODE == kResidualRestrict && post.coarse_scratch != nullptr;
    for (int c = g0; c < g1; ++c)
      {
        uint32_t first = bd.colour_start[c], count = bd.colour_start[c + 1] - first;
        if (one_launch)
          {
            if (c != g0)
              break;
            count = bd.colour_start[g1] - first;
          }
        if (count == 0)
          continue;
        const uint32_t grid = std::min<uint32_t>(count, (uint32_t)(op.macro_wg_x16 ? 1 : C::WGS) * macro_cus(op));
        constexpr bool kUsesDiag = is_cheb_mode(MODE);
        if (kUsesDiag && op.diag_items)
          {
            BrickPost<T> pt = post;
            pt.b            = (const T *)op.diag_items;
            hipLaunchKernelGGL((brick_macro_kernel<P, T, MODE, kUsesDiag>), dim3(grid), dim3(C::THREADS), 0, s, src, first,
                               count, bd.ent_base, bd.item_map, (const Basis1D<T> *)op.basis, (T)op.coef[0],
                               (T)op.coef[1], (T)op.coef[2], pt, (uint32_t)(op.n_dofs * sizeof(T)));
          }
        else
          hipLaunchKernelGGL((brick_macro_kernel<P, T, MODE, false>), dim3(grid), dim3(C::THREADS), 0, s, src, first,
                             count, bd.ent_base, bd.item_map, (const Basis1D<T> *)op.basis, (T)op.coef[0],
                             (T)op.coef[1], (T)op.coef[2], post, (uint32_t)(op.n_dofs * sizeof(T)));
      }
  }

  template <int P, typename T>
  static void macro_modes(hipStream_t s, const OperatorData &op, int mode, const T *src, const BrickPost<T> &post, int g0,
                          int g1, bool fr)
  {
    switch (mode)
      {
        case kPlain: macro_launch<P, T, kPlain>(s, op, src, post, g0, g1, fr); break;
        case kResidual: macro_launch<P, T, kResidual>(s, op, src, post, g0, g1, fr); break;
        case kCheb: macro_launch<P, T, kCheb>(s, op, src, post, g0, g1, fr); break;
        case kChebFirst: macro_launch<P, T, kChebFirst>(s, op, src, post, g0, g1, fr); break;
        case kChebZeroOld: macro_launch<P, T, kChebZeroOld>(s, op, src, post, g0, g1, fr); break;
        case kChebInit: macro_launch<P, T, kChebInit>(s, op, src, post, g0, g1, fr); break;
        case kChebOldInit: macro_launch<P, T, kChebOldInit>(s, op, src, post, g0, g1, fr); break;
        case kResidualRestrict: macro_launch<P, T, kResidualRestrict>(s, op, src, post, g0, g1); break;
        case kChebFirstProlong: macro_launch<P, T, kChebFirstProlong>(s, op, src, post, g0, g1); break;
        default: break;
      }
  }

#if MGX_MACRO_IS_F64
  __global__ void reduce4_kernel(const double *__restrict__ partials, uint32_t n, const double *__restrict__ extra,
                                 double *__restrict__ sums)
  {
    __shared__ double red[4 * 256];
    const int         tid = threadIdx.x;
    double            acc[4] = {0., 0., 0., 0.};
    for (uint32_t i = tid; i < n; i += 256)
      for (int k = 0; k < 4; ++k)
        acc[k] += partials[4 * (size_t)i + k];
    for (int k = 0; k < 4; ++k)
      red[k * 256 + tid] = acc[k];
    __syncthreads();
    for (int stride = 128; stride > 0; stride >>= 1)
      {
        if (tid < stride)
          for (int k = 0; k < 4; ++k)
            red[k * 256 + tid] += red[k * 256 + tid + stride];
        __syncthreads();
      }
    if (tid < 4)
      sums[tid] = red[tid * 256] + (extra ? extra[tid] : 0.);
  }
#endif

  template <typename T, bool VERIFY>
  __global__ void diag_table_kernel(const T *__restrict__ inv_diag, const uint32_t *__restrict__ ent_base,
                                    const uint32_t *__restrict__ item_map, uint32_t ne, uint32_t npts, T *table,
                                    uint32_t *flag)
  {
    const uint32_t brick = blockIdx.x;
    for (uint32_t i = threadIdx.x; i < npts; i += blockDim.x)
      {
        const uint32_t m = item_map[i], w = ent_base[(size_t)brick * ne + item_slot(m)];
        if (w == kInvalid)
          continue;
        const T v = inv_diag[ent_index(w) + item_offset(m)];
        if (!VERIFY)
          table[i] = v;
        else
          {
            const T    t   = table[i];
            const T    tol = (sizeof(T) == 8 ? T(1e-14) : T(2e-6)) * (t < 0 ? -t : t);
            const T    dvt = v - t;
            const bool same = (dvt < 0 ? -dvt : dvt) <= tol;
            if (!same)
              atomicOr(flag, 1u);
          }
      }
  }

#define MGX_CAT2(a, b) a##b
#define MGX_CAT(a, b) MGX_CAT2(a, b)
  void MGX_CAT(macro_diag_table_, MGX_MACRO_SUFFIX)(hipStream_t s, const OperatorData &op, const uint32_t *item_map, void *table,
                                                    uint32_t *flag_dev)
  {
    using T             = MGX_MACRO_T;
    const BrickData &bd = op.bricks;
    const uint32_t   nb = op.p <= 4 ? 4 : 2, g = nb * op.p + 1, npts = g * g * g, e1 = 2 * nb + 1, ne = e1 * e1 * e1;
    hipLaunchKernelGGL((diag_table_kernel<T, false>), dim3(bd.n_bricks), dim3(256), 0, s, (const T *)op.inv_diag,
                       bd.ent_base, item_map, ne, npts, (T *)table, flag_dev);
    hipLaunchKernelGGL((diag_table_kernel<T, true>), dim3(bd.n_bricks), dim3(256), 0, s, (const T *)op.inv_diag,
                       bd.ent_base, item_map, ne, npts, (T *)table, flag_dev);
  }

  bool MGX_CAT(launch_macro_cg_update_, MGX_MACRO_SUFFIX)(hipStream_t s, const OperatorData &op, double alpha, double beta,
                                                           const void *r, void *q, void *p, void *x, void *carrier,
                                                           double *partials, uint32_t capacity, uint32_t *n_partials)
  {
    using T = MGX_MACRO_T;
    if (MGX_MACRO_PAIRS || (uint64_t)op.n_dofs * sizeof(T) >= 0xFFFFFFF0ull)
      return false;
    BrickPost<T> post{};
    post.a       = (const T *)r;
    post.b       = (const T *)q;
    post.old     = (const T *)x;
    post.out     = (T *)q;
    post.partial = (T *)carrier;
    post.f1      = (T)alpha;
    post.f2      = (T)beta;
    post.src_w   = (T *)p;
    post.x_w     = (T *)x;
    const BrickData &bd   = op.bricks;
    uint32_t         used = 0;
    auto             run  = [&](auto cfg) {
      using C = decltype(cfg);
      uint64_t total = 0;
      for (int c = 0; c < bd.n_colours; ++c)
        total += std::min<uint32_t>(bd.colour_start[c + 1] - bd.colour_start[c],
                                    (uint32_t)(op.macro_wg_x16 ? 1 : C::WGS) * macro_cus(op));
      if (total > capacity)
        return false;
      for (int c = 0; c < bd.n_colours; ++c)
        {
          const uint32_t first = bd.colour_start[c], count = bd.colour_start[c + 1] - first;
          if (count == 0)
            continue;
          const uint32_t grid = std::min<uint32_t>(count, (uint32_t)(op.macro_wg_x16 ? 1 : C::WGS) * macro_cus(op));
          post.sums = partials + 4 * (size_t)used;
          used += grid;
          hipLaunchKernelGGL((brick_macro_kernel<C::N - 1, T, kCgUpdate, false>), dim3(grid), dim3(C::THREADS), 0, s,
                             (const T *)p, first, count, bd.ent_base, bd.item_map, (const Basis1D<T> *)op.basis,
                             (T)op.coef[0], (T)op.coef[1], (T)op.coef[2], post, (uint32_t)(op.n_dofs * sizeof(T)));
        }
      return true;
    };
    bool ok = false;
    switch (op.p)
      {
#ifdef MGX_MACRO_ONLY_P
        case MGX_MACRO_ONLY_P: ok = run(MCfg<MGX_MACRO_ONLY_P, T>()); break;
#else
        case 1: ok = run(MCfg<1, T>()); break;
        case 2: ok = run(MCfg<2, T>()); break;
        case 3: ok = run(MCfg<3, T>()); break;
        case 4: ok = run(MCfg<4, T>()); break;
        case 5: ok = run(MCfg<5, T>()); break;
        case 6: ok = run(MCfg<6, T>()); break;
        case 7: ok = run(MCfg<7, T>()); break;
        case 8: ok = run(MCfg<8, T>()); break;
        case 9: ok = run(MCfg<9, T>()); break;
#endif
        default: break;
      }
    *n_partials = used;
    return ok;
  }

#if MGX_MACRO_IS_F64
  void launch_reduce4(hipStream_t s, const double *partials, uint32_t n, const double *extra, double *sums)
  {
    hipLaunchKernelGGL(reduce4_kernel, dim3(1), dim3(256), 0, s, partials, n, extra, sums);
  }
#endif

  bool MGX_CAT(launch_macro_loop_, MGX_MACRO_SUFFIX)(hipStream_t s, const OperatorData &op, int mode, const void *src,
                                                     const void *a, const void *b, void *out, void *partial,
                                                     double f1, double f2, const void *old, double f0, void *coarse,
                                                     const uint32_t *coarse_blocks, int g0, int g1, bool free_schedule)
  {
    using T = MGX_MACRO_T;
    const bool fr = free_schedule && op.bricks.fr.available() && mode <= kChebOldInit && !MGX_MACRO_PAIRS;
    if (free_schedule && !fr)
      return false;
    if (!free_schedule && op.macro_v2 && !MGX_MACRO_PAIRS &&
        MGX_CAT(launch_macro2_loop_, MGX_MACRO_SUFFIX)(s, op, mode, src, a, out, partial, coarse, coarse_blocks, g0, g1, f1, f2, f0, old))
// ... 38 lines not shown
```

### multigrid_amd/csrc/mgx_macro2.hip

```cpp
#include "mgx_macro_device.hpp"

#include <hip/hip_runtime.h>

#include <algorithm>
#include <cstdlib>

#ifndef MGX_MACRO_T
#define MGX_MACRO_T double
#endif
#ifndef MGX_MACRO2_CHUNK
#define MGX_MACRO2_CHUNK 3
#endif

#ifdef MGX_MACRO_STAMPS
#ifndef MGX_MACRO_STAMP_MODE
#define MGX_MACRO_STAMP_MODE -1
#endif
__device__ unsigned long long g_mgx_stamps2[8192 * 16];
#define MGX_STAMP(k)                                                                                              \
  do                                                                                                              \
    {                                                                                                             \
      if (threadIdx.x == 0 && blockIdx.x < 8192 && (MGX_MACRO_STAMP_MODE < 0 || MODE == MGX_MACRO_STAMP_MODE))      \
        g_mgx_stamps2[blockIdx.x * 16 + (k)] = ((k) == 15 || (k) == 13) ? __builtin_amdgcn_s_memrealtime()         \
                                                                         : __builtin_amdgcn_s_memtime();           \
// ... 116 lines not shown
            z[P] += zn;
          }
#pragma unroll
        for (int i = 1; i < N; ++i)
          {
            W[base + i * G] = y[i];
            U[base + i * G] = z[i];
          }
        if (c == 0)
          {
            W[base] = y[0];
            U[base] = z[0];
          }
      }
    if (tid < LINES)
      {
        const int l    = tid;
        const int base = (l / G) * (G * G) + l % G;
        T         a[G], t2[G], s2[G];
#pragma unroll
        for (int j = 0; j < G; ++j)
          a[j] = W[base + j * G];
        macro_apply2<P, T>(M, K, a, t2, s2);
#pragma unroll
        for (int j = 0; j < G; ++j)
          W[base + j * G] = t2[j];
#pragma unroll
        for (int j = 0; j < G; ++j)
          a[j] = U[base + j * G];
        macro_apply<P, T>(M, a, t2);
#pragma unroll
        for (int j = 0; j < G; ++j)
          U[base + j * G] = fma(c0, t2[j], c1 * s2[j]);
      }
    lds_barrier();
    mark(1);
    if (REM > 0 && tid < REM * NB)
      {
        const int l = NT + tid / NB, c = tid % NB, base = l + c * P * (G * G);
        T         seg[N], y[N], r[N];
#pragma unroll
        for (int i = 0; i < N; ++i)
          seg[i] = W[base + i * (G * G)];
        cell_apply<P, T>(K, seg, r);
#pragma unroll
        for (int i = 0; i < N; ++i)
          seg[i] = U[base + i * (G * G)];
        cell_apply<P, T>(M, seg, y);
#pragma unroll
        for (int i = 0; i < N; ++i)
          y[i] = fma(c2, r[i], y[i]);
        const T yn = next_lane(y[0]);
        if (c + 1 < NB)
          y[P] += yn;
#pragma unroll
        for (int i = 1; i < N; ++i)
          W[base + i * (G * G)] = y[i];
        if (c == 0)
          W[base] = y[0];
      }
    if (tid < LINES)
      {
        const int l = tid;
        T         a[G], r[G], o[G];
#pragma unroll
        for (int j = 0; j < G; ++j)
          a[j] = W[l + j * (G * G)];
        macro_apply<P, T>(K, a, r);
#pragma unroll
        for (int j = 0; j < G; ++j)
          a[j] = U[l + j * (G * G)];
        macro_apply<P, T>(M, a, o);
#pragma unroll
        for (int j = 0; j < G; ++j)
          W[l + j * (G * G)] = fma(c2, r[j], o[j]);
      }
  }

  __host__ __device__ constexpr bool macro2_covers(int mode, int p = 4)
  {
    return mode == kPlain || mode == kResidual || ((mode == kResidualRestrict || mode == kChebInit) && p <= 4) || mode == kChebOldInit;
  }

  template <int P, typename T, int MODE>
  __global__ void __launch_bounds__((M2Cfg<P, T>::THREADS), (M2Cfg<P, T>::MINW))
    brick_macro2_kernel(const T *__restrict__ src, uint32_t brick_first, uint32_t brick_count,
                        const uint32_t *__restrict__ ent_base, const uint32_t *__restrict__ item_map,
                        const Basis1D<T> *__restrict__ B, T c0, T c1, T c2, BrickPost<T> post, uint32_t vec_bytes)
  {
    static_assert(macro2_covers(MODE, (MODE == kResidualRestrict || MODE == kChebInit) ? 4 : P), "form not covered by this pipeline");
    using C            = M2Cfg<P, T>;
    constexpr int NT   = C::THREADS, IT = C::IT, JINT = C::JINT, JSURF = C::JSURF, NE = C::NE;
    constexpr int NEW  = (NE + NT - 1) / NT;
    __shared__ T        U[C::ASZ];
    __shared__ T        W[C::ASZ];
    __shared__ uint32_t E[NE];

    const int tid = threadIdx.x;
    uint32_t  b   = blockIdx.x;
    if (b >= brick_count)
      return;
    MGX_STAMP(0);
    MGX_STAMP(15);
#ifdef MGX_MACRO_STAMPS
    int mgx_iter = 0;
#endif
    auto live = [&](int j) { return (j + 1) * NT <= C::NPTS || tid + j * NT < C::NPTS; };
    uint32_t mw[IT];
#pragma unroll
    for (int j = 0; j < IT; ++j)
      mw[j] = item_map[live(j) ? tid + j * NT : 0];
    const rsrc_t rsrc = make_rsrc(src, vec_bytes), r_a = make_rsrc(post.a, vec_bytes), r_out = make_rsrc(post.out, vec_bytes),
                 r_partial = make_rsrc(post.partial, vec_bytes), r_old = make_rsrc(post.old, vec_bytes);
    const EOMat<T> &M = B->mass, &K = B->lapl;
    constexpr bool kKeepX = is_cheb_mode(MODE);
    T              dv[kKeepX ? IT : 1];
    if (kKeepX)
      {
#pragma unroll
        for (int j = 0; j < IT; ++j)
          dv[kKeepX ? j : 0] = post.b[live(j) ? tid + j * NT : 0];
      }

    uint32_t en[NEW] = {};
    auto     table_load = [&](uint32_t brick, uint32_t(&e)[NEW]) {
#pragma unroll
      for (int j = 0; j < NEW; ++j)
        {
          const int i = tid + j * NT;
          e[j]        = ent_base[(size_t)(brick_first + brick) * NE + (i < NE ? i : 0)];
        }
    };
    auto table_store = [&](uint32_t *dst, const uint32_t(&e)[NEW]) {
#pragma unroll
      for (int j = 0; j < NEW; ++j)
        if (tid + j * NT < NE)
          dst[tid + j * NT] = e[j];
    };
    auto unit_offset = [&](uint32_t w, uint32_t m) {
      return w != kInvalid ? (ent_index(w) + item_offset(m)) * (uint32_t)sizeof(T) : kOob;
    };
    T    g[IT];
    auto gather_issue = [&](const uint32_t *tab) {
#pragma unroll
      for (int j = 0; j < IT; ++j)
        {
          g[j] = T(0);
          if (live(j))
            g[j] = buf_ld(MODE == kChebInit ? r_a : rsrc, unit_offset(tab[item_slot(mw[j])], mw[j]), T());
        }
    };
    T    xs[kKeepX ? IT : 1];
    auto gather_land = [&]() {
#pragma unroll
      for (int j = 0; j < IT; ++j)
        {
          T v = g[j];
          if (MODE == kChebInit)
            v = post.f0 * dv[kKeepX ? j : 0] * g[j];
          if (live(j))
            U[item_point(mw[j])] = v;
          if (kKeepX)
            xs[kKeepX ? j : 0] = v;
        }
    };
    constexpr bool kCarrier = MODE != kResidualRestrict;
    T              pp[JSURF];
    auto           partial_issue = [&]() {
#pragma unroll
      for (int j = JINT; j < IT; ++j)
        {
          pp[j - JINT] = T(0);
          if (!kCarrier)
            continue;
#ifndef MGX_MACRO_NOCARRIER
          const uint32_t w    = live(j) ? E[item_slot(mw[j])] : kInvalid;
          const bool     need = w != kInvalid && !(w & 0x40000000u);
          if (__builtin_amdgcn_ballot_w64(need) != 0)
            pp[j - JINT] = buf_ld(r_partial, need ? unit_offset(w, mw[j]) : kOob, T());
#endif
        }
    };

    constexpr bool kRhs = MODE == kResidual || MODE == kResidualRestrict;
    T              av[kRhs ? IT : 1];
    auto           rhs_issue = [&]() {
      if (kRhs)
        {
#pragma unroll
          for (int j = 0; j < IT; ++j)
            {
              const uint32_t w    = live(j) ? E[item_slot(mw[j])] : kInvalid;
              const bool     last = w != kInvalid && (j < JINT || (w >> 31));
              av[kRhs ? j : 0]    = buf_ld(r_a, last ? unit_offset(w, mw[j]) : kOob, T());
            }
        }
    };

    {
      uint32_t e0[NEW];
      table_load(b, e0);
      if (b + gridDim.x < brick_count)
        table_load(b + gridDim.x, en);
      table_store(E, e0);
      lds_barrier();
      MGX_STAMP(1);
      gather_issue(E);
      gather_land();
      MGX_STAMP(2);
      lds_barrier();
    }

    for (;;)
      {
        const uint32_t bn = b + gridDim.x;
        const bool     has_next = bn < brick_count;
        MGX_STAMP_IT(3);
#ifdef MGX_MACRO_STAMPS
        if (mgx_iter == 4)
          MGX_STAMP(11);
#endif
        partial_issue();
        rhs_issue();
#pragma unroll
        for (int j = 0; j < IT; ++j)
          asm volatile("" : "+v"(mw[j]));
        if (MODE == kChebInit || MODE == kChebOldInit)
          {
#pragma unroll
            for (int j = 0; j < IT; ++j)
              asm volatile("" : "+v"(dv[kKeepX ? j : 0]));
          }
        MGX_STAMP_IT(4);
#ifndef MGX_MACRO_NOSWEEP
        if (kSlicedSweeps<P, MODE> && P >= 9)
          brick_sweeps_sliced<P, T>(
            tid, U, W, B, c0, c1, c2, [&](int k) { MGX_STAMP_IT(5 + k); }, [&]() { lds_barrier(); });
        else
          brick_sweeps<P, T>(tid, U, W, M, K, c0, c1, c2, [&](int k) { MGX_STAMP_IT(5 + k); });
#endif
        lds_barrier();
        MGX_STAMP_IT(7);
        if (has_next)
          {
            table_store(reinterpret_cast<uint32_t *>(U), en);
            lds_barrier();
            gather_issue(reinterpret_cast<const uint32_t *>(U));
          }
        MGX_STAMP_IT(8);

        if constexpr (kKeepX)
          {
            constexpr int kChunk = MGX_MACRO2_CHUNK < IT ? MGX_MACRO2_CHUNK : IT, NCH = (IT + kChunk - 1) / kChunk;
            struct Ops
            {
              T        av, ov;
              uint32_t w, off;
            };
            Ops  ops[2][kChunk];
            auto issue = [&](int c, Ops(&o)[kChunk]) {
#pragma unroll
              for (int k = 0; k < kChunk; ++k)
                {
                  const int j = c * kChunk + k;
                  if (j < IT)
                    o[k].w = live(j) ? E[item_slot(mw[j])] : kInvalid;
                }
#pragma unroll
              for (int k = 0; k < kChunk; ++k)
                {
                  const int j = c * kChunk + k;
                  if (j >= IT)
                    continue;
                  if (j < JINT && o[k].w != kInvalid)
                    o[k].w |= 0xC0000000u;
                  const bool last  = o[k].w != kInvalid && (o[k].w >> 31);
                  o[k].off         = unit_offset(o[k].w, mw[j]);
                  const uint32_t ol = last ? o[k].off : kOob;
                  o[k].av          = buf_ld(r_a, ol, T());
                  o[k].ov          = MODE == kCheb ? buf_ld(r_old, ol, T()) : T(0);
                }
            };
            issue(0, ops[0]);
#pragma unroll
            for (int c = 0; c < NCH; ++c)
              {
                if (c + 1 < NCH)
                  issue(c + 1, ops[(c + 1) & 1]);
                __builtin_amdgcn_sched_barrier(0);
                T val[kChunk];
#pragma unroll
                for (int k = 0; k < kChunk; ++k)
                  {
                    const int j = c * kChunk + k;
                    val[k]      = (j < IT && live(j)) ? W[item_point(mw[j])] : T(0);
                  }
#pragma unroll
                for (int k = 0; k < kChunk; ++k)
                  {
                    const int j = c * kChunk + k;
                    if (j >= IT)
                      continue;
                    const Ops &o   = ops[c & 1][k];
                    const bool vld = o.w != kInvalid, last = vld && (o.w >> 31);
                    const T    res = post_finish<T, MODE>(post, j >= JINT ? pp[j >= JINT ? j - JINT : 0] : T(0), o.av, o.ov,
                                                          dv[kKeepX ? j : 0], last, val[k], xs[kKeepX ? j : 0]);
                    if (j < JINT)
                      buf_st(r_out, o.off, res);
                    else
                      {
                        buf_st(r_out, last ? o.off : kOob, res);
#ifndef MGX_MACRO_NOCARRIER
                        if (__builtin_amdgcn_ballot_w64(vld && !last) != 0)
                          buf_st(r_partial, last ? kOob : o.off, res);
#endif
                      }
                  }
                __builtin_amdgcn_sched_barrier(0);
              }
          }
        else
          {
          {
            uint32_t w[IT];
  #pragma unroll
            for (int j = 0; j < IT; ++j)
              w[j] = live(j) ? E[item_slot(mw[j])] : kInvalid;
  #pragma unroll
            for (int j = 0; j < IT; ++j)
              {
                if (j < JINT && w[j] != kInvalid)
                  w[j] |= 0xC0000000u;
                const bool     vld = w[j] != kInvalid, last = vld && (w[j] >> 31);
                const uint32_t off = unit_offset(w[j], mw[j]);
                T              val = live(j) ? W[item_point(mw[j])] : T(0);
                if (j >= JINT && kCarrier)
                  val += pp[j >= JINT ? j - JINT : 0];
                if (MODE == kResidualRestrict)
                  {
                    if (live(j))
                      W[item_point(mw[j])] = vld ? (last ? av[kRhs ? j : 0] : T(0)) - val : T(0);
                    continue;
                  }
                if (MODE == kResidual && last)
                  val = av[kRhs ? j : 0] - val;
                if (j < JINT)
                  buf_st<kAuxNt>(r_out, off, val);
                else
                  {
                    buf_st<kAuxNt>(r_out, last ? off : kOob, val);
  #ifndef MGX_MACRO_NOCARRIER
                    if (__builtin_amdgcn_ballot_w64(vld && !last) != 0)
                      buf_st(r_partial, last ? kOob : off, val);
  #endif
                  }
              }
          }
          }
        if (MODE == kResidualRestrict)
          {
            constexpr int CE1 = C::NB + 1, CNP = (C::NB / 2) * P + 1;
            lds_barrier();
            const uint32_t *ctab = post.coarse_blocks + (size_t)(brick_first + b) * (CE1 * CE1 * CE1);
            if (post.coarse_scratch)
              restrict_brick<P, T, NT, true>(tid, W, B->P1eo, nullptr, ctab,
                                             post.coarse_scratch + (size_t)(brick_first + b) * (CNP * CNP * CNP));
            else
              restrict_brick<P, T, NT, false>(tid, W, B->P1eo, post.coarse, ctab);
          }
        MGX_STAMP_IT(9);
        if (!has_next)
          break;
        lds_barrier();
        gather_land();
        table_store(E, en);
        if (bn + gridDim.x < brick_count)
          table_load(bn + gridDim.x, en);
        MGX_STAMP_IT(10);
        lds_barrier();
        b = bn;
#ifdef MGX_MACRO_STAMPS
        ++mgx_iter;
#endif
      }
#ifdef MGX_MACRO_STAMPS
    asm volatile("s_waitcnt vmcnt(0)" ::: "memory");
    MGX_STAMP(14);
    MGX_STAMP(13);
#endif
  }

  static uint32_t macro2_cus(const OperatorData &op)
  {
    static const int cus = [] {
      int dev = 0, n = 256;
      if (hipGetDevice(&dev) == hipSuccess)
        (void)hipDeviceGetAttribute(&n, hipDeviceAttributeMultiprocessorCount, dev);
      return std::max(1, n);
    }();
    return op.macro_wg_x16 ? std::max<uint32_t>(1u, (uint32_t)cus * op.macro_wg_x16 / 16u) : (uint32_t)cus;
  }

  template <int P, typename T, int MODE>
  static void macro2_launch(hipStream_t s, const OperatorData &op, const T *src, const BrickPost<T> &post, int g0, int g1)
  {
    using C             = M2Cfg<P, T>;
    const BrickData &bd = op.bricks;
    const bool one_launch = MODE == kResidualRestrict && post.coarse_scratch != nullptr;
    for (int c = g0; c < g1; ++c)
      {
        uint32_t first = bd.colour_start[c], count = bd.colour_start[c + 1] - first;
        if (one_launch)
          {
            if (c != g0)
              break;
            count = bd.colour_start[g1] - first;
          }
        if (count == 0)
          continue;
        const uint32_t grid = std::min<uint32_t>(count, (uint32_t)(op.macro_wg_x16 ? 1 : C::WGS) * macro2_cus(op));
        hipLaunchKernelGGL((brick_macro2_kernel<P, T, MODE>), dim3(grid), dim3(C::THREADS), 0, s, src, first, count, bd.ent_base,
                           bd.item_map2, (const Basis1D<T> *)op.basis, (T)op.coef[0], (T)op.coef[1], (T)op.coef[2], post,
                           (uint32_t)(op.n_dofs * sizeof(T)));
      }
  }

  template <int P, typename T>
  static void macro2_modes(hipStream_t s, const OperatorData &op, int mode, const T *src, const BrickPost<T> &post, int g0, int g1)
  {
    switch (mode)
      {
        case kPlain: macro2_launch<P, T, kPlain>(s, op, src, post, g0, g1); break;
        case kResidual: macro2_launch<P, T, kResidual>(s, op, src, post, g0, g1); break;
        case kChebInit:
          if constexpr (P <= 4)
            macro2_launch<P, T, kChebInit>(s, op, src, post, g0, g1);
          break;
        case kChebOldInit: macro2_launch<P, T, kChebOldInit>(s, op, src, post, g0, g1); break;
        case kResidualRestrict:
          if constexpr (P <= 4)
            macro2_launch<P, T, kResidualRestrict>(s, op, src, post, g0, g1);
          break;
        default: break;
      }
  }

#define MGX_CAT2(a, b) a##b
#define MGX_CAT(a, b) MGX_CAT2(a, b)
  bool MGX_CAT(launch_macro2_loop_, MGX_MACRO_SUFFIX)(hipStream_t s, const OperatorData &op, int mode, const void *src, const void *a,
                                                      void *out, void *partial, void *coarse, const uint32_t *coarse_blocks, int g0,
                                                      int g1, double f1, double f2, double f0, const void *old)
  {
    using T = MGX_MACRO_T;
    if (!macro2_covers(mode, op.p) || !op.bricks.item_map2 || (uint64_t)op.n_dofs * sizeof(T) >= 0xFFFFFFF0ull)
      return false;
    if (is_cheb_mode(mode) && !op.diag_items2)
      return false;
    BrickPost<T> post{};
    post.b   = (const T *)op.diag_items2;
    post.old = (const T *)old;
    post.f1  = (T)f1;
    post.f2  = (T)f2;
    post.f0  = (T)f0;
    post.a              = (const T *)a;
    post.out            = (T *)out;
    post.partial        = (T *)partial;
    post.coarse         = (T *)coarse;
    post.coarse_blocks  = coarse_blocks;
    post.coarse_scratch = mode == kResidualRestrict ? (T *)partial : nullptr;
    switch (op.p)
      {
#ifdef MGX_MACRO_ONLY_P
        case MGX_MACRO_ONLY_P: macro2_modes<MGX_MACRO_ONLY_P, T>(s, op, mode, (const T *)src, post, g0, g1); break;
#else
        case 1: macro2_modes<1, T>(s, op, mode, (const T *)src, post, g0, g1); break;
        case 2: macro2_modes<2, T>(s, op, mode, (const T *)src, post, g0, g1); break;
        case 3: macro2_modes<3, T>(s, op, mode, (const T *)src, post, g0, g1); break;
        case 4: macro2_modes<4, T>(s, op, mode, (const T *)src, post, g0, g1); break;
        case 5: macro2_modes<5, T>(s, op, mode, (const T *)src, post, g0, g1); break;
        case 6: macro2_modes<6, T>(s, op, mode, (const T *)src, post, g0, g1); break;
        case 7: macro2_modes<7, T>(s, op, mode, (const T *)src, post, g0, g1); break;
        case 8: macro2_modes<8, T>(s, op, mode, (const T *)src, post, g0, g1); break;
        case 9: macro2_modes<9, T>(s, op, mode, (const T *)src, post, g0, g1); break;
#endif
        default: return false;
      }
    return true;
  }
}
```

### multigrid_amd/csrc/mgx_macro_device.hpp

```cpp
#pragma once

#include "mgx_brick_device.hpp"
#include "mgx_bricks.hpp"

#include <hip/hip_runtime.h>

namespace mgx
{
  template <int P, typename T>
  struct MCfg
  {
    using C = BCfg<P>;
    static constexpr int NB = C::NB, G = C::G, NE = C::NE, N = P + 1;
    static constexpr int LINES   = G * G;
    static constexpr int THREADS = (LINES > 128 && LINES % 64 <= 40) ? (LINES / 64) * 64 : ((LINES + 63) / 64) * 64;
    static constexpr int NPTS    = G * G * G;
    static constexpr int ent_count(int t) { return (t == 0 || t == 3 ? 1 : 3) * ipow(NB, t) * ipow(NB + 1, 3 - t); }
    static constexpr int ipow(int b, int e) { return e == 0 ? 1 : b * ipow(b, e - 1); }
    static constexpr int ent_size(int t) { return ipow(P - 1, t); }
    static constexpr int NPAIR   = MGX_MACRO_PAIRS ? ent_count(0) * (ent_size(0) / 2) + ent_count(1) * (ent_size(1) / 2) +
                                                     ent_count(2) * (ent_size(2) / 2) + ent_count(3) * (ent_size(3) / 2)
                                                 : 0;
    static constexpr int NSINGLE = NPTS - 2 * NPAIR;
    static constexpr int JP      = (NPAIR + THREADS - 1) / THREADS;
// ... 174 lines not shown
#pragma unroll
        for (int j = 0; j < G; ++j)
          a[j] = U[lb + j * G];
        macro_apply<P, T>(M, a, t2);
#pragma unroll
        for (int j = 0; j < G; ++j)
          U[lb + j * G] = fma(c0, t2[j], c1 * s2[j]);
      }
    if (rm)
      {
        T         seg[N], y[N], z[N], r[N];
        const int base = (rl / G) * (G * G) + rl % G + rc * P * G;
#pragma unroll
        for (int i = 0; i < N; ++i)
          seg[i] = W[base + i * G];
        cell_apply<P, T>(coef_reload(&B->lapl), seg, z);
        const EOMat<T> &M = coef_reload(&B->mass);
        cell_apply<P, T>(M, seg, y);
#pragma unroll
        for (int i = 0; i < N; ++i)
          seg[i] = U[base + i * G];
        cell_apply<P, T>(M, seg, r);
#pragma unroll
        for (int i = 0; i < N; ++i)
          z[i] = fma(c0, r[i], c1 * z[i]);
        seam(y);
        seam(z);
#pragma unroll
        for (int i = 1; i < N; ++i)
          {
            W[base + i * G] = y[i];
            U[base + i * G] = z[i];
          }
        if (rc == 0)
          {
            W[base] = y[0];
            U[base] = z[0];
          }
      }
    barrier();
    mark(1);
    if (ln)
      {
        T a[G], r[G], o[G];
#pragma unroll
        for (int j = 0; j < G; ++j)
          a[j] = W[tid + j * (G * G)];
        macro_apply<P, T>(coef_reload(&B->lapl), a, r);
#pragma unroll
        for (int j = 0; j < G; ++j)
          a[j] = U[tid + j * (G * G)];
        macro_apply<P, T>(coef_reload(&B->mass), a, o);
#pragma unroll
        for (int j = 0; j < G; ++j)
          W[tid + j * (G * G)] = fma(c2, r[j], o[j]);
      }
    if (rm)
      {
        T         seg[N], y[N], q[N];
        const int base = rl + rc * P * (G * G);
#pragma unroll
        for (int i = 0; i < N; ++i)
          seg[i] = W[base + i * (G * G)];
        cell_apply<P, T>(coef_reload(&B->lapl), seg, q);
#pragma unroll
        for (int i = 0; i < N; ++i)
          seg[i] = U[base + i * (G * G)];
        cell_apply<P, T>(coef_reload(&B->mass), seg, y);
#pragma unroll
        for (int i = 0; i < N; ++i)
          y[i] = fma(c2, q[i], y[i]);
        seam(y);
#pragma unroll
        for (int i = 1; i < N; ++i)
          W[base + i * (G * G)] = y[i];
        if (rc == 0)
          W[base] = y[0];
      }
  }

  __device__ __forceinline__ uint32_t item_slot(uint32_t m) { return m & 1023u; }
  __device__ __forceinline__ uint32_t item_point(uint32_t m) { return (m >> 10) & 8191u; }
  __device__ __forceinline__ uint32_t item_offset(uint32_t m) { return m >> 23; }

  __host__ __device__ constexpr bool is_cheb_mode(int mode)
  {
    return (mode >= kCheb && mode <= kChebOldInit) || mode == kChebFirstProlong;
  }

  using rsrc_t = __amdgpu_buffer_rsrc_t;
  typedef unsigned int u32x2_t __attribute__((ext_vector_type(2)));
  constexpr uint32_t kOob = 0xFFFFFFF0u;
  constexpr int kAuxNt = 2;
  __device__ __forceinline__ rsrc_t make_rsrc(const void *p, uint32_t bytes)
  {
    return __builtin_amdgcn_make_buffer_rsrc(const_cast<void *>(p), 0, bytes, 0x00020000);
  }
  __device__ __forceinline__ double buf_ld(rsrc_t r, uint32_t off, double)
  {
    return __builtin_bit_cast(double, __builtin_amdgcn_raw_buffer_load_b64(r, off, 0, 0));
  }
  __device__ __forceinline__ float buf_ld(rsrc_t r, uint32_t off, float)
  {
    return __builtin_bit_cast(float, __builtin_amdgcn_raw_buffer_load_b32(r, off, 0, 0));
  }
  template <int AUX = 0>
  __device__ __forceinline__ void buf_st(rsrc_t r, uint32_t off, double v)
  {
    __builtin_amdgcn_raw_buffer_store_b64(__builtin_bit_cast(u32x2_t, v), r, off, 0, AUX);
  }
  template <int AUX = 0>
  __device__ __forceinline__ void buf_st(rsrc_t r, uint32_t off, float v)
  {
    __builtin_amdgcn_raw_buffer_store_b32(__builtin_bit_cast(unsigned int, v), r, off, 0, AUX);
  }

  typedef unsigned int u32x4_t __attribute__((ext_vector_type(4)));
  __device__ __forceinline__ void buf_ld2(rsrc_t r, uint32_t off, double &a, double &b)
  {
    const u32x4_t v = __builtin_bit_cast(u32x4_t, __builtin_amdgcn_raw_buffer_load_b128(r, off, 0, 0));
    a               = __builtin_bit_cast(double, u32x2_t{v.x, v.y});
    b               = __builtin_bit_cast(double, u32x2_t{v.z, v.w});
  }
  __device__ __forceinline__ void buf_ld2(rsrc_t r, uint32_t off, float &a, float &b)
  {
    const unsigned long long u = __builtin_bit_cast(unsigned long long, __builtin_amdgcn_raw_buffer_load_b64(r, off, 0, 0));
    a                          = __builtin_bit_cast(float, (unsigned int)u);
    b                          = __builtin_bit_cast(float, (unsigned int)(u >> 32));
  }
  __device__ __forceinline__ void buf_st2(rsrc_t r, uint32_t off, double a, double b)
  {
    const u32x2_t lo = __builtin_bit_cast(u32x2_t, a), hi = __builtin_bit_cast(u32x2_t, b);
    __builtin_amdgcn_raw_buffer_store_b128(u32x4_t{lo.x, lo.y, hi.x, hi.y}, r, off, 0, 0);
  }
  __device__ __forceinline__ void buf_st2(rsrc_t r, uint32_t off, float a, float b)
  {
    __builtin_amdgcn_raw_buffer_store_b64(u32x2_t{__builtin_bit_cast(unsigned int, a), __builtin_bit_cast(unsigned int, b)}, r,
                                          off, 0, 0);
  }

  template <typename T>
  struct PostRsrc
  {
    rsrc_t a, b, old, out, partial, src, srcw, xw, priv;
  };

  template <typename T>
  struct PostOps
  {
    T pv[2], av[2], bv[2], ov[2];
  };

  template <typename T, int MODE, bool DTAB, bool PAIR>
  __device__ __forceinline__ void post_issue(const PostRsrc<T> &R, uint32_t w, uint32_t off, PostOps<T> &o)
  {
    const bool valid        = w != kInvalid;
    const bool need_partial = valid && !(w & 0x40000000u) && MODE != kResidualRestrict;
    const bool last         = valid && (w >> 31);
    o.pv[0] = o.pv[1] = o.av[0] = o.av[1] = o.bv[0] = o.bv[1] = o.ov[0] = o.ov[1] = T(0);
    const uint32_t ol = last ? off : kOob, op = need_partial ? off : kOob;
    auto           ld = [&](rsrc_t r, uint32_t f, T(&v)[2]) {
      if (PAIR)
        buf_ld2(r, f, v[0], v[1]);
      else
        v[0] = buf_ld(r, f, T());
    };
#ifndef MGX_MACRO_NOCARRIER
    if (__builtin_amdgcn_ballot_w64(need_partial) != 0)
      ld(R.partial, op, o.pv);
#endif
    if (MODE != kPlain)
      ld(R.a, ol, o.av);
    if (is_cheb_mode(MODE) && !DTAB)
      ld(R.b, ol, o.bv);
    if (MODE == kCheb || MODE == kCgUpdate)
      ld(R.old, ol, o.ov);
    if (MODE == kCgUpdate)
      ld(R.src, ol, o.bv);
  }

  template <typename T, int MODE>
  __device__ __forceinline__ T post_finish(const BrickPost<T> &post, T pv, T av, T ov, T bv, bool last, T val, T xi)
  {
    val += pv;
    if (MODE == kPlain || MODE == kCgUpdate)
      return val;
    else if (MODE == kResidualRestrict)
// ... 17 lines not shown
```

Before: 14.83 billion DoFs/s.

## Compress per-brick entity table into 27 group words with shared offsets

Replaces the per-brick table of entity base words (one word per entity slot) with 27 group words per brick plus a brick-independent offset table. Item-map words are re-encoded to carry the group index and offset, and the diagonal tables are permuted to match. This cuts the index metadata each workgroup loads per brick and double-buffers the table prefetch. The cost is extra host-side construction and validation, a fallback path when the compression does not fit, and more complex kernel addressing.

```diff
diff --git a/include/mgx.h b/include/mgx.h
--- a/include/mgx.h
+++ b/include/mgx.h
@@ -118,6 +118,11 @@
 int mgx_operator_exchange_buffers(mgx_operator_t op, int k, void **send, void **recv, uint32_t *count, int *rank);
 int mgx_exchange_add(mgx_operator_t op, void *vec);
 int mgx_operator_number(mgx_operator_t op);
+int mgx_operator_uses_group_table(mgx_operator_t op);
+int mgx_host_group_table(int degree, uint32_t n_cells, uint32_t n_dofs, const uint32_t *idx27, const uint32_t *idx27_plain,
+                         const uint8_t *brick_colour, const uint32_t *shared, uint32_t n_shared, int split_interface,
+                         uint32_t *n_bricks, uint32_t *n_entities, uint32_t *ent_words, uint32_t *grp, uint32_t *ent_off,
+                         uint32_t *item_map, int *grouped);
 int mgx_vmult(mgx_operator_t op, void *dst, const void *src);
 int mgx_compute_residual(mgx_operator_t op, void *dst, const void *src, const void *rhs_q);
 int mgx_vmult_residual(mgx_operator_t op, const void *rhs, const void *lhs, void *residual);
diff --git a/multigrid_amd/__init__.py b/multigrid_amd/__init__.py
--- a/multigrid_amd/__init__.py
+++ b/multigrid_amd/__init__.py
@@ -547,6 +547,26 @@
         return (-0.9 if self.box_desc is None else self.box_desc["origin"]) + X
 
 
+def host_group_table(cube, level, split_interface=False):
+    lib, p = _lib.load(), cube.degree
+    nb, ne, grouped = C.c_uint32(), C.c_uint32(), C.c_int()
+    idx, plain = lib.mgx_cube_idx27(cube.h, level), lib.mgx_cube_idx27_plain(cube.h, level)
+    desc = cube.operator_desc(level)
+    shared = np.ascontiguousarray(cube.shared(level), dtype=np.uint32)
+    args = (p, cube.n_cells(level), cube.n_dofs(level), idx, plain, desc.brick_colour,
+            shared.ctypes.data_as(_lib.u32p) if shared.size else None, shared.size, int(split_interface), C.byref(nb), C.byref(ne))
+    check(lib.mgx_host_group_table(*args, None, None, None, None, None))
+    g = (4 if p <= 4 else 2) * p + 1
+    words = np.empty((nb.value, ne.value), np.uint32)
+    grp, off, items = np.empty((nb.value, 27), np.uint32), np.empty(ne.value, np.uint32), np.empty(g ** 3, np.uint32)
+    ptr = lambda a: a.ctypes.data_as(_lib.u32p)
+    check(lib.mgx_host_group_table(*args, ptr(words), ptr(grp), ptr(off), ptr(items), C.byref(grouped)))
+    out = {"n_bricks": nb.value, "n_entities": ne.value, "ent_words": words, "grouped": bool(grouped.value)}
+    if grouped.value:
+        out.update(grp=grp, ent_off=off, item_map=items)
+    return out
+
+
 def _cell_dofs(idx27, p):
     n = p + 1
     idx27 = np.asarray(idx27, dtype=np.int64).reshape(-1, 27)
@@ -586,6 +606,9 @@
 
     def m(self):
         return self.lib.mgx_operator_n_dofs(self.h)
+
+    def uses_group_table(self):
+        return bool(self.lib.mgx_operator_uses_group_table(self.h))
 
     def set_profiled(self, on=True):
         check(self.lib.mgx_operator_set_profiled(self.h, int(on)))
diff --git a/multigrid_amd/_lib.py b/multigrid_amd/_lib.py
--- a/multigrid_amd/_lib.py
+++ b/multigrid_amd/_lib.py
@@ -121,6 +121,9 @@
     "mgx_operator_destroy": (C.c_int, [vp]),
     "mgx_operator_n_dofs": (C.c_uint32, [vp]),
     "mgx_operator_number": (C.c_int, [vp]),
+    "mgx_operator_uses_group_table": (C.c_int, [vp]),
+    "mgx_host_group_table": (C.c_int, [C.c_int, C.c_uint32, C.c_uint32, u32p, u32p, C.POINTER(C.c_uint8), u32p, C.c_uint32,
+                                      C.c_int, u32p, u32p, u32p, u32p, u32p, u32p, C.POINTER(C.c_int)]),
     "mgx_vmult": (C.c_int, [vp, vp, vp]),
     "mgx_vmult_residual": (C.c_int, [vp, vp, vp, vp]),
     "mgx_compute_diagonal": (C.c_int, [vp]),
diff --git a/multigrid_amd/csrc/mgx_api.cpp b/multigrid_amd/csrc/mgx_api.cpp
--- a/multigrid_amd/csrc/mgx_api.cpp
+++ b/multigrid_amd/csrc/mgx_api.cpp
@@ -129,6 +129,7 @@
     {"macro_wg_per_cu_x16", nullptr, &macro_wg_x16},
     {"no_diag_table", &no_diag_table, nullptr},
     {"no_macro_v2", &no_macro_v2, nullptr},
+    {"no_group_table", &no_group_table, nullptr},
     {"no_general_bricks", &no_general_bricks, nullptr},
     {"general_brick_min", nullptr, &general_brick_min},
     {"fused_prolong_min_bricks", nullptr, &fused_prolong_min_bricks},
@@ -1408,6 +1409,24 @@
                 MGX_HIP(hipMalloc((void **)&b.item_map2, sizeof(uint32_t) * map2.size()));
                 MGX_HIP(hipMemcpy(b.item_map2, map2.data(), sizeof(uint32_t) * map2.size(), hipMemcpyHostToDevice));
               }
+              if (tun.no_group_table || MGX_MACRO_PAIRS || tun.cells_form)
+                MGX_TRACE("operator_create: no group table (%s)", tun.no_group_table ? "option no_group_table" : "build option");
+              else
+                {
+                  GroupHost   gh;
+                  std::string no;
+                  if (build_group_table(p, bh.n_bricks, bh.ent_base.data(), gh, no))
+                    {
+                      MGX_HIP(hipMalloc((void **)&b.grp, sizeof(uint32_t) * gh.grp.size()));
+                      MGX_HIP(hipMemcpy(b.grp, gh.grp.data(), sizeof(uint32_t) * gh.grp.size(), hipMemcpyHostToDevice));
+                      MGX_HIP(hipMalloc((void **)&b.item_map_g, sizeof(uint32_t) * gh.item_map.size()));
+                      MGX_HIP(hipMemcpy(b.item_map_g, gh.item_map.data(), sizeof(uint32_t) * gh.item_map.size(), hipMemcpyHostToDevice));
+                      b.item_map_g_host = gh.item_map;
+                      MGX_TRACE("operator_create: group table, 27 words per brick");
+                    }
+                  else
+                    MGX_TRACE("operator_create: no group table (%s)", no.c_str());
+                }
               const int n_classes = b.n_bricks <= tun.free_one_max ? 1 : 2;
               FreeHost  fh;
               if (!MGX_MACRO_PAIRS && !tun.cells_form && b.n_bricks <= tun.free_max_bricks &&
@@ -1732,6 +1751,8 @@
   (void)hipFree(op->d.bricks.ent_flags);
   (void)hipFree(op->d.bricks.item_map);
   (void)hipFree(op->d.bricks.item_map2);
+  (void)hipFree(op->d.bricks.grp);
+  (void)hipFree(op->d.bricks.item_map_g);
   (void)hipFree(op->d.bricks.fr.ent);
   (void)hipFree(op->d.bricks.fr.surf_off);
   (void)hipFree(op->d.bricks.fr.priv);
@@ -1748,6 +1769,8 @@
   (void)hipFree(op->d.gbricks.fr.surf_pos);
   (void)hipFree(op->d.diag_items);
   (void)hipFree(op->d.diag_items2);
+  (void)hipFree(op->d.diag_items_g);
+  (void)hipFree(op->d.diag_items2_g);
   (void)hipFree(op->cg_partials);
   (void)hipFree(op->cg_result);
   (void)hipFree(op->cg_carrier);
@@ -1791,6 +1814,44 @@
   return MGX_OK;
 }
 int      mgx_operator_number(mgx_operator_t op) { return op ? op->d.number : -1; }
+
+int mgx_operator_uses_group_table(mgx_operator_t op)
+{
+  if (!op || !op->d.bricks.grp)
+    return 0;
+  const bool diag_ok = (!op->d.diag_items || op->d.diag_items_g) && (!op->d.diag_items2 || op->d.diag_items2_g);
+  return diag_ok ? 1 : 0;
+}
+
+int mgx_host_group_table(int degree, uint32_t n_cells, uint32_t n_dofs, const uint32_t *idx27, const uint32_t *idx27_plain,
+                         const uint8_t *brick_colour, const uint32_t *shared, uint32_t n_shared, int split_interface,
+                         uint32_t *n_bricks, uint32_t *n_entities, uint32_t *ent_words, uint32_t *grp, uint32_t *ent_off,
+                         uint32_t *item_map, int *grouped)
+{
+  MGX_REQUIRE(idx27 && n_bricks && n_entities && (shared || n_shared == 0), "mgx_host_group_table: null argument");
+  BrickHost   bh;
+  std::string why;
+  if (!build_bricks(degree, n_cells, n_dofs, idx27, idx27_plain, brick_colour, shared, n_shared, split_interface != 0, bh, why))
+    return mgx::report_error(MGX_ERR_INVALID_ARGUMENT, ("mgx_host_group_table: " + why).c_str());
+  for (size_t i = 0; i < bh.ent_base.size(); ++i)
+    if (bh.ent_base[i] != MGX_INVALID_INDEX)
+      bh.ent_base[i] |= (uint32_t)(bh.ent_flags[i] & 3u) << 30;
+  *n_bricks   = bh.n_bricks;
+  *n_entities = (uint32_t)bh.n_entities;
+  if (ent_words)
+    std::memcpy(ent_words, bh.ent_base.data(), sizeof(uint32_t) * bh.ent_base.size());
+  GroupHost  gh;
+  const bool ok = build_group_table(degree, bh.n_bricks, bh.ent_base.data(), gh, why);
+  if (grouped)
+    *grouped = ok;
+  if (ok && grp)
+    std::memcpy(grp, gh.grp.data(), sizeof(uint32_t) * gh.grp.size());
+  if (ok && ent_off)
+    std::memcpy(ent_off, gh.ent_off.data(), sizeof(uint32_t) * gh.ent_off.size());
+  if (ok && item_map)
+    std::memcpy(item_map, gh.item_map.data(), sizeof(uint32_t) * gh.item_map.size());
+  return MGX_OK;
+}
 
 int mgx_vmult(mgx_operator_t op, void *dst, const void *src)
 {
@@ -2164,6 +2225,32 @@
         MGX_HIP(hipFree(table));
       if (which == 0)
         MGX_TRACE("compute_diagonal: diagonal %s per brick item", mismatch == 0 ? "uniform" : "not uniform");
+      void *&slot_g = which == 0 ? op->d.diag_items_g : op->d.diag_items2_g;
+      if (slot_g)
+        {
+          MGX_HIP(hipFree(slot_g));
+          slot_g = nullptr;
+        }
+      const std::vector<uint32_t> &map_g = op->d.bricks.item_map_g_host;
+      if (slot && op->d.bricks.grp)
+        {
+          MGX_REQUIRE(map_g.size() == npts, "mgx_compute_diagonal: group-form item table of another size");
+          std::vector<uint32_t> host_map;
+          if (which == 0)
+            build_item_map(op->d.p, host_map);
+          else
+            build_item_map2(op->d.p, host_map);
+          const size_t         ns = number_size(op->d.number);
+          std::vector<uint32_t> at_point(npts, 0);
+          for (uint32_t i = 0; i < npts; ++i)
+            at_point[(host_map[i] >> 10) & 8191u] = i;
+          std::vector<char> in(ns * npts), out(ns * npts);
+          MGX_HIP(hipMemcpy(in.data(), slot, ns * npts, hipMemcpyDeviceToHost));
+          for (uint32_t i = 0; i < npts; ++i)
+            std::memcpy(&out[ns * i], &in[ns * at_point[map_g[i] >> 18]], ns);
+          MGX_HIP(hipMalloc(&slot_g, ns * npts));
+          MGX_HIP(hipMemcpy(slot_g, out.data(), ns * npts, hipMemcpyHostToDevice));
+        }
     }
   return MGX_OK;
 }
diff --git a/multigrid_amd/csrc/mgx_bricks.cpp b/multigrid_amd/csrc/mgx_bricks.cpp
--- a/multigrid_amd/csrc/mgx_bricks.cpp
+++ b/multigrid_amd/csrc/mgx_bricks.cpp
@@ -564,4 +564,89 @@
           for (size_t k = 0; k < e.pnt.size(); ++k)
             map.push_back(item_word(e.slot, e.pnt[k], (int)k));
   }
+
+  bool build_group_table(int p, uint32_t n_bricks, const uint32_t *ent_words, GroupHost &out, std::string &why)
+  {
+    out = GroupHost();
+    const int NB = p <= 4 ? 4 : 2, G = NB * p + 1, E1 = 2 * NB + 1, NE = E1 * E1 * E1;
+    constexpr uint32_t kIndex = 0x3FFFFFFFu;
+    auto ent_size = [&](int slot) {
+      const int ex = slot % E1, ey = (slot / E1) % E1, ez = slot / (E1 * E1);
+      return ((ex & 1) ? p - 1 : 1) * ((ey & 1) ? p - 1 : 1) * ((ez & 1) ? p - 1 : 1);
+    };
+    out.grp.assign((size_t)n_bricks * 27, kInvalid);
+#pragma omp parallel for schedule(static)
+    for (uint32_t b = 0; b < n_bricks; ++b)
+      for (int slot = 0; slot < NE; ++slot)
+        {
+          const uint32_t w = ent_words[(size_t)b * NE + slot];
+          uint32_t      &g = out.grp[(size_t)b * 27 + brick_group_of(slot, E1)];
+          if (w != kInvalid && (g == kInvalid || (w & kIndex) < (g & kIndex)))
+            g = w;
+        }
+    out.ent_off.assign(NE, kInvalid);
+    for (int grp = 0; grp < 27; ++grp)
+      for (uint32_t b = 0; b < n_bricks; ++b)
+        {
+          const uint32_t g = out.grp[(size_t)b * 27 + grp];
+          if (g == kInvalid)
+            continue;
+          for (int slot = 0; slot < NE; ++slot)
+            {
+              const uint32_t w = ent_words[(size_t)b * NE + slot];
+              if (brick_group_of(slot, E1) == grp && w != kInvalid)
+                out.ent_off[slot] = (w & kIndex) - (g & kIndex);
+            }
+          break;
+        }
+    uint64_t mismatches = 0;
+#pragma omp parallel for schedule(static) reduction(+ : mismatches)
+    for (uint32_t b = 0; b < n_bricks; ++b)
+      for (int slot = 0; slot < NE; ++slot)
+        mismatches += expand_group_word(&out.grp[(size_t)b * 27], out.ent_off.data(), slot, E1) != ent_words[(size_t)b * NE + slot];
+    if (mismatches != 0)
+      {
+        why = std::to_string(mismatches) + " entity words differ from the expansion of 27 group words per brick";
+        out = GroupHost();
+        return false;
+      }
+    std::vector<uint32_t> map2;
+    build_item_map2(p, map2);
+    const size_t                                  n_int = (size_t)(G - 2) * (G - 2) * (G - 2);
+    std::vector<std::pair<uint32_t, uint32_t>> surf;
+    out.item_map.reserve(map2.size());
+    for (size_t i = 0; i < map2.size(); ++i)
+      {
+        const int      slot = (int)(map2[i] & 1023u), grp = brick_group_of(slot, E1);
+        const uint32_t pnt = (map2[i] >> 10) & 8191u;
+        if (out.ent_off[slot] == kInvalid || ent_size(slot) == 0)
+          {
+            why = "an entity with DoFs is valid in no brick";
+            out = GroupHost();
+            return false;
+          }
+        const uint32_t off = out.ent_off[slot] + (map2[i] >> 23);
+        if (off >= 8192u || (i < n_int) != (grp == kGroupInterior) || (i < n_int && off != i))
+          {
+            why = i < n_int ? "the interior of a brick is not one block in item order" : "group offset beyond 13 bits";
+            out = GroupHost();
+            return false;
+          }
+        if (i < n_int)
+          out.item_map.push_back((uint32_t)grp | (off << 5) | (pnt << 18));
+        else
+          surf.push_back({((uint32_t)grp << 13) | off, pnt});
+      }
+    std::sort(surf.begin(), surf.end());
+    for (const auto &s : surf)
+      out.item_map.push_back((s.first >> 13) | ((s.first & 8191u) << 5) | (s.second << 18));
+    for (uint32_t b = 0; b < n_bricks; ++b)
+      if (out.grp[(size_t)b * 27 + kGroupInterior] == kInvalid || (out.grp[(size_t)b * 27 + kGroupInterior] >> 30) != 3u)
+        {
+          why = "a brick whose interior DoFs are missing or shared with another brick";
+          out = GroupHost();
+          return false;
+        }
+    return true;
+  }
 }
diff --git a/multigrid_amd/csrc/mgx_bricks.hpp b/multigrid_amd/csrc/mgx_bricks.hpp
--- a/multigrid_amd/csrc/mgx_bricks.hpp
+++ b/multigrid_amd/csrc/mgx_bricks.hpp
@@ -40,4 +40,23 @@
 #endif
   void build_item_map(int p, std::vector<uint32_t> &map);
   void build_item_map2(int p, std::vector<uint32_t> &map);
+
+  struct GroupHost
+  {
+    std::vector<uint32_t> grp;
+    std::vector<uint32_t> ent_off;
+    std::vector<uint32_t> item_map;
+  };
+  constexpr int kGroupInterior = 13;
+  inline int    brick_group_of(int slot, int e1)
+  {
+    auto g = [e1](int e) { return e == 0 ? 0 : (e == e1 - 1 ? 2 : 1); };
+    return (g(slot / (e1 * e1)) * 3 + g((slot / e1) % e1)) * 3 + g(slot % e1);
+  }
+  bool build_group_table(int p, uint32_t n_bricks, const uint32_t *ent_words, GroupHost &out, std::string &why);
+  inline uint32_t expand_group_word(const uint32_t *grp27, const uint32_t *ent_off, int slot, int e1)
+  {
+    const uint32_t g = grp27[brick_group_of(slot, e1)];
+    return (g == 0xFFFFFFFFu || ent_off[slot] == 0xFFFFFFFFu) ? 0xFFFFFFFFu : g + ent_off[slot];
+  }
 }
diff --git a/multigrid_amd/csrc/mgx_internal.hpp b/multigrid_amd/csrc/mgx_internal.hpp
--- a/multigrid_amd/csrc/mgx_internal.hpp
+++ b/multigrid_amd/csrc/mgx_internal.hpp
@@ -37,6 +37,7 @@
     bool     no_general_bricks = false;
     uint32_t general_brick_min = 2048;
     bool     no_macro_v2      = false;
+    bool     no_group_table   = false;
     bool     no_fused_init    = false;
     bool     no_fused_restrict = false;
     bool     no_fused_prolong = false;
@@ -99,6 +100,9 @@
     uint8_t  *ent_flags = nullptr;
     uint32_t *item_map  = nullptr;
     uint32_t *item_map2 = nullptr;
+    uint32_t *grp        = nullptr;
+    uint32_t *item_map_g = nullptr;
+    std::vector<uint32_t> item_map_g_host;
     std::vector<uint32_t> order;
     uint32_t *order_dev = nullptr;
     bool      available() const { return n_bricks > 0; }
@@ -137,6 +141,7 @@
     bool      separable     = true;
     void     *diag_items    = nullptr;
     void     *diag_items2   = nullptr;
+    void     *diag_items_g  = nullptr, *diag_items2_g = nullptr;
     bool      macro_v2      = true;
   };
 
diff --git a/multigrid_amd/csrc/mgx_macro.hip b/multigrid_amd/csrc/mgx_macro.hip
--- a/multigrid_amd/csrc/mgx_macro.hip
+++ b/multigrid_amd/csrc/mgx_macro.hip
@@ -50,7 +50,7 @@
 
 namespace mgx
 {
-  template <int P, typename T, int MODE, bool DTAB, bool FREE = false>
+  template <int P, typename T, int MODE, bool DTAB, bool FREE = false, bool GRP = false>
   __global__ void __launch_bounds__((MCfg<P, T>::THREADS), (MCfg<P, T>::MINW))
     brick_macro_kernel(const T *__restrict__ src, uint32_t brick_first, uint32_t brick_count,
                        const uint32_t *__restrict__ ent_base, const uint32_t *__restrict__ item_map,
@@ -61,7 +61,10 @@
     constexpr int NT     = C::THREADS;
     constexpr int IT     = C::IT;
     constexpr int LINES  = C::LINES;
-    constexpr int NEW    = (C::NE + NT - 1) / NT;
+    static_assert(!GRP || (!FREE && !MGX_MACRO_PAIRS && MODE != kCgUpdate), "group form: eight-colour schedule, single items");
+    constexpr int NET    = GRP ? kGroupWords : C::NE;
+    constexpr int NEW    = (NET + NT - 1) / NT;
+    constexpr int JINT   = GRP ? (G - 2) * (G - 2) * (G - 2) / NT : 0;
     constexpr int N = P + 1, NB = C::NB;
     constexpr int REM    = LINES - NT;
     constexpr bool kKeepX = is_cheb_mode(MODE) || MODE == kCgUpdate;
@@ -141,20 +144,25 @@
       for (int j = 0; j < NEW; ++j)
         {
           const int i = tid + j * NT;
-          e[j]        = ent_base[(size_t)(brick_first + brick) * C::NE + (i < C::NE ? i : 0)];
+          e[j]        = ent_base[(size_t)(brick_first + brick) * NET + (i < NET ? i : 0)];
         }
     };
     auto table_store = [&](uint32_t *E, const uint32_t(&e)[NEW]) {
 #pragma unroll
       for (int j = 0; j < NEW; ++j)
-        if (tid + j * NT < C::NE)
+        if (tid + j * NT < NET)
           E[tid + j * NT] = e[j];
     };
+    const uint32_t tb    = (uint32_t)tid * (uint32_t)sizeof(T);
+    auto           ibase = [&](const uint32_t *E) {
+      return ent_index((uint32_t)__builtin_amdgcn_readfirstlane((int)E[kGroupInterior])) * (uint32_t)sizeof(T);
+    };
+    auto ioff = [&](uint32_t ib, int it) { return tb + (ib + (uint32_t)(it * NT) * (uint32_t)sizeof(T)); };
     auto unit_offset = [&](uint32_t w, uint32_t m, int it = 0, uint32_t brick = 0) {
 #ifdef MGX_MACRO_CONTIG
       return w != kInvalid ? ((brick_first + brick) * (uint32_t)(C::NB * C::NB * C::NB * P * P * P) + (uint32_t)(tid + it * NT)) * (uint32_t)sizeof(T) : kOob;
 #else
-      return w != kInvalid ? (ent_index(w) + item_offset(m)) * (uint32_t)sizeof(T) : kOob;
+      return w != kInvalid ? (ent_index(w) + item_offset<GRP>(m)) * (uint32_t)sizeof(T) : kOob;
 #endif
     };
     constexpr bool kProlong = MODE == kChebFirstProlong;
@@ -201,6 +209,7 @@
     auto gather_issue = [&](const uint32_t *E, uint32_t brick) {
       const rsrc_t r0 = MODE == kChebInit ? (DTAB ? R.a : R.b) : rsrc;
       const rsrc_t r1 = MODE == kCgUpdate ? R.b : R.a;
+      const uint32_t ib = GRP ? ibase(E) : 0u;
 #pragma unroll
       for (int j = 0; j < JP; ++j)
         {
@@ -222,7 +231,7 @@
           g[0][v] = g[NG - 1][v] = T(0);
           if (live_s(j))
             {
-              const uint32_t off = unit_offset(E[item_slot(mw[v])], mw[v], v, brick);
+              const uint32_t off = (GRP && v < JINT) ? ioff(ib, v) : unit_offset(E[item_slot<GRP>(mw[v])], mw[v], v, brick);
               g[0][v]            = buf_ld(r0, off, T());
               if (NG == 2)
                 g[NG - 1][v] = buf_ld(r1, off, T());
@@ -240,7 +249,7 @@
           if (MODE == kCgUpdate)
             v = post.f1 == T(0) ? g[NG - 1][it] : post.f2 * g[0][it] + g[NG - 1][it];
           if (live(it))
-            U[item_point(mw[it])] = v;
+            U[item_point<GRP>(mw[it])] = v;
           if (kKeepX)
             xs[it] = v;
         }
@@ -260,7 +269,7 @@
           for (int it = 0; it < IT; ++it)
             if (live(it))
               {
-                const uint32_t pnt = item_point(mw[it]);
+                const uint32_t pnt = item_point<GRP>(mw[it]);
                 xs[kKeepX ? it : 0] += W[pnt];
                 U[pnt] = xs[kKeepX ? it : 0];
               }
@@ -479,6 +488,11 @@
           uint32_t      iw[2][kChunk];
           uint32_t      pw[2][FREE ? kChunk : 1];
           const uint32_t priv0 = FREE ? (brick_first + b) * post.n_surf : 0u;
+          const uint32_t ibc   = GRP ? ibase(ebase) : 0u;
+          auto uoff = [&](int u, uint32_t w) {
+            const int v0 = u < JP ? 2 * u : JP + u;
+            return (GRP && v0 < JINT) ? ioff(ibc, v0) : unit_offset(w, mw[v0], v0, b);
+          };
           auto slot0 = [&](int u) { return u < JP ? 2 * u : JP + u; };
           auto ulive = [&](int u) { return u < JP ? live_p(u) : live_s(u - JP); };
           auto issue = [&](int c, PostOps<T>(&o)[kChunk], uint32_t(&w)[kChunk], uint32_t(&pv)[FREE ? kChunk : 1]) {
@@ -487,8 +501,10 @@
               {
                 const int u = c * kChunk + j;
                 w[j]        = kInvalid;
-                if (u < NU && ulive(u))
-                  w[j] = ebase[item_slot(mw[slot0(u)])];
+                if (GRP && u < NU && slot0(u < NU ? u : 0) < JINT)
+                  w[j] = 0xC0000000u;
+                else if (u < NU && ulive(u))
+                  w[j] = ebase[item_slot<GRP>(mw[slot0(u)])];
                 if (FREE)
                   {
                     const uint32_t so = (u < NU && ulive(u)) ? sbase[item_slot(mw[slot0(u < NU ? u : 0)])] : kInvalid;
@@ -505,9 +521,9 @@
               {
                 const int u = c * kChunk + j;
                 if (u < JP)
-                  post_issue<T, MODE, DTAB, true>(R, w[j], unit_offset(w[j], mw[slot0(u < NU ? u : 0)], slot0(u < NU ? u : 0), b), o[j]);
+                  post_issue<T, MODE, DTAB, true>(R, w[j], uoff(u, w[j]), o[j]);
                 else if (u < NU)
-                  post_issue<T, MODE, DTAB, false>(R, w[j], unit_offset(w[j], mw[slot0(u < NU ? u : 0)], slot0(u < NU ? u : 0), b), o[j]);
+                  post_issue<T, MODE, DTAB, false>(R, w[j], uoff(u, w[j]), o[j]);
               }
           };
           issue(0, ops[0], iw[0], pw[0]);
@@ -525,9 +541,9 @@
                   val[j][0] = val[j][1] = T(0);
                   if (u < NU && ulive(u))
                     {
-                      val[j][0] = W[item_point(mw[slot0(u)])];
+                      val[j][0] = W[item_point<GRP>(mw[slot0(u)])];
                       if (u < JP)
-                        val[j][1] = W[item_point(mw[slot0(u) + 1])];
+                        val[j][1] = W[item_point<GRP>(mw[slot0(u) + 1])];
                     }
                 }
 #pragma unroll
@@ -540,7 +556,7 @@
                       const bool        pair = u < JP;
                       const uint32_t    w    = iw[c & 1][j];
                       const bool        vld  = w != kInvalid, last = vld && (w >> 31);
-                      const uint32_t    off  = unit_offset(w, mw[v0], v0, b);
+                      const uint32_t    off  = uoff(u, w);
                       const PostOps<T> &o    = ops[c & 1][j];
                       T                 res[2];
 #pragma unroll
@@ -560,9 +576,9 @@
                         {
                           if (ulive(u))
                             {
-                              W[item_point(mw[v0])] = vld ? res[0] : T(0);
+                              W[item_point<GRP>(mw[v0])] = vld ? res[0] : T(0);
                               if (pair)
-                                W[item_point(mw[v0 + 1])] = vld ? res[1] : T(0);
+                                W[item_point<GRP>(mw[v0 + 1])] = vld ? res[1] : T(0);
                             }
                         }
                       else if (MODE == kCgUpdate)
@@ -731,6 +747,25 @@
           continue;
         const uint32_t grid = std::min<uint32_t>(count, (uint32_t)(op.macro_wg_x16 ? 1 : C::WGS) * macro_cus(op));
         constexpr bool kUsesDiag = is_cheb_mode(MODE);
+        if constexpr (!MGX_MACRO_PAIRS)
+          {
+            if (bd.grp)
+              {
+                BrickPost<T> pt = post;
+                if (kUsesDiag && op.diag_items)
+                  {
+                    pt.b = (const T *)op.diag_items_g;
+                    hipLaunchKernelGGL((brick_macro_kernel<P, T, MODE, kUsesDiag, false, true>), dim3(grid), dim3(C::THREADS), 0, s,
+                                       src, first, count, bd.grp, bd.item_map_g, (const Basis1D<T> *)op.basis, (T)op.coef[0],
+                                       (T)op.coef[1], (T)op.coef[2], pt, (uint32_t)(op.n_dofs * sizeof(T)));
+                  }
+                else
+                  hipLaunchKernelGGL((brick_macro_kernel<P, T, MODE, false, false, true>), dim3(grid), dim3(C::THREADS), 0, s, src,
+                                     first, count, bd.grp, bd.item_map_g, (const Basis1D<T> *)op.basis, (T)op.coef[0],
+                                     (T)op.coef[1], (T)op.coef[2], pt, (uint32_t)(op.n_dofs * sizeof(T)));
+                continue;
+              }
+          }
         if (kUsesDiag && op.diag_items)
           {
             BrickPost<T> pt = post;
@@ -790,10 +825,29 @@
   }
 #endif
 
-  template <typename T, bool VERIFY>
-  __global__ void diag_table_kernel(const T *__restrict__ inv_diag, const uint32_t *__restrict__ ent_base,
-                                    const uint32_t *__restrict__ item_map, uint32_t ne, uint32_t npts, T *table,
-                                    uint32_t *flag)
+  template <typename T>
+  __global__ void diag_table_collect_kernel(const T *__restrict__ inv_diag, const uint32_t *__restrict__ ent_base,
+                                            const uint32_t *__restrict__ item_map, uint32_t n_bricks, uint32_t ne,
+                                            uint32_t npts, T *table)
+  {
+    const uint32_t i = blockIdx.x * blockDim.x + threadIdx.x;
+    if (i >= npts)
+      return;
+    const uint32_t m = item_map[i];
+    for (uint32_t brick = 0; brick < n_bricks; ++brick)
+      {
+        const uint32_t w = ent_base[(size_t)brick * ne + item_slot(m)];
+        if (w != kInvalid)
+          {
+            table[i] = inv_diag[ent_index(w) + item_offset(m)];
+            return;
+          }
+      }
+  }
+  template <typename T>
+  __global__ void diag_table_verify_kernel(const T *__restrict__ inv_diag, const uint32_t *__restrict__ ent_base,
+                                           const uint32_t *__restrict__ item_map, uint32_t ne, uint32_t npts,
+                                           const T *__restrict__ table, uint32_t *flag)
   {
     const uint32_t brick = blockIdx.x;
     for (uint32_t i = threadIdx.x; i < npts; i += blockDim.x)
@@ -801,18 +855,13 @@
         const uint32_t m = item_map[i], w = ent_base[(size_t)brick * ne + item_slot(m)];
         if (w == kInvalid)
           continue;
-        const T v = inv_diag[ent_index(w) + item_offset(m)];
-        if (!VERIFY)
-          table[i] = v;
-        else
-          {
-            const T    t   = table[i];
-            const T    tol = (sizeof(T) == 8 ? T(1e-14) : T(2e-6)) * (t < 0 ? -t : t);
-            const T    dvt = v - t;
-            const bool same = (dvt < 0 ? -dvt : dvt) <= tol;
-            if (!same)
-              atomicOr(flag, 1u);
-          }
+        const T    v   = inv_diag[ent_index(w) + item_offset(m)];
+        const T    t   = table[i];
+        const T    tol = (sizeof(T) == 8 ? T(1e-14) : T(2e-6)) * (t < 0 ? -t : t);
+        const T    dvt = v - t;
+        const bool same = (dvt < 0 ? -dvt : dvt) <= tol;
+        if (!same)
+          atomicOr(flag, 1u);
       }
   }
 
@@ -824,10 +873,10 @@
     using T             = MGX_MACRO_T;
     const BrickData &bd = op.bricks;
     const uint32_t   nb = op.p <= 4 ? 4 : 2, g = nb * op.p + 1, npts = g * g * g, e1 = 2 * nb + 1, ne = e1 * e1 * e1;
-    hipLaunchKernelGGL((diag_table_kernel<T, false>), dim3(bd.n_bricks), dim3(256), 0, s, (const T *)op.inv_diag,
-                       bd.ent_base, item_map, ne, npts, (T *)table, flag_dev);
-    hipLaunchKernelGGL((diag_table_kernel<T, true>), dim3(bd.n_bricks), dim3(256), 0, s, (const T *)op.inv_diag,
-                       bd.ent_base, item_map, ne, npts, (T *)table, flag_dev);
+    hipLaunchKernelGGL((diag_table_collect_kernel<T>), dim3((npts + 255) / 256), dim3(256), 0, s, (const T *)op.inv_diag,
+                       bd.ent_base, item_map, bd.n_bricks, ne, npts, (T *)table);
+    hipLaunchKernelGGL((diag_table_verify_kernel<T>), dim3(bd.n_bricks), dim3(256), 0, s, (const T *)op.inv_diag,
+                       bd.ent_base, item_map, ne, npts, (const T *)table, flag_dev);
   }
 
   bool MGX_CAT(launch_macro_cg_update_, MGX_MACRO_SUFFIX)(hipStream_t s, const OperatorData &op, double alpha, double beta,
diff --git a/multigrid_amd/csrc/mgx_macro2.hip b/multigrid_amd/csrc/mgx_macro2.hip
--- a/multigrid_amd/csrc/mgx_macro2.hip
+++ b/multigrid_amd/csrc/mgx_macro2.hip
@@ -222,7 +222,7 @@
     return mode == kPlain || mode == kResidual || ((mode == kResidualRestrict || mode == kChebInit) && p <= 4) || mode == kChebOldInit;
   }
 
-  template <int P, typename T, int MODE>
+  template <int P, typename T, int MODE, bool GRP = false>
   __global__ void __launch_bounds__((M2Cfg<P, T>::THREADS), (M2Cfg<P, T>::MINW))
     brick_macro2_kernel(const T *__restrict__ src, uint32_t brick_first, uint32_t brick_count,
                         const uint32_t *__restrict__ ent_base, const uint32_t *__restrict__ item_map,
@@ -231,12 +231,19 @@
     static_assert(macro2_covers(MODE, (MODE == kResidualRestrict || MODE == kChebInit) ? 4 : P), "form not covered by this pipeline");
     using C            = M2Cfg<P, T>;
     constexpr int NT   = C::THREADS, IT = C::IT, JINT = C::JINT, JSURF = C::JSURF, NE = C::NE;
-    constexpr int NEW  = (NE + NT - 1) / NT;
+    const int     tid  = threadIdx.x;
+    constexpr int NET  = GRP ? kGroupWords : NE;
+    constexpr int NEW  = (NET + NT - 1) / NT;
     __shared__ T        U[C::ASZ];
     __shared__ T        W[C::ASZ];
-    __shared__ uint32_t E[NE];
-
-    const int tid = threadIdx.x;
+    __shared__ uint32_t E[GRP ? 64 : NE];
+    const uint32_t *Ec = E, *En = E + 32;
+    const uint32_t  tb = (uint32_t)tid * (uint32_t)sizeof(T);
+    auto ibase = [&](const uint32_t *tab) {
+      return ent_index((uint32_t)__builtin_amdgcn_readfirstlane((int)tab[kGroupInterior])) * (uint32_t)sizeof(T);
+    };
+    auto isoff = [&](uint32_t ib, int j) { return ib + (uint32_t)(j * NT) * (uint32_t)sizeof(T); };
+
     uint32_t  b   = blockIdx.x;
     if (b >= brick_count)
       return;
@@ -268,26 +275,29 @@
       for (int j = 0; j < NEW; ++j)
         {
           const int i = tid + j * NT;
-          e[j]        = ent_base[(size_t)(brick_first + brick) * NE + (i < NE ? i : 0)];
+          e[j]        = ent_base[(size_t)(brick_first + brick) * NET + (i < NET ? i : 0)];
         }
     };
     auto table_store = [&](uint32_t *dst, const uint32_t(&e)[NEW]) {
 #pragma unroll
       for (int j = 0; j < NEW; ++j)
-        if (tid + j * NT < NE)
+        if (tid + j * NT < NET)
           dst[tid + j * NT] = e[j];
     };
     auto unit_offset = [&](uint32_t w, uint32_t m) {
-      return w != kInvalid ? (ent_index(w) + item_offset(m)) * (uint32_t)sizeof(T) : kOob;
+      return w != kInvalid ? (ent_index(w) + item_offset<GRP>(m)) * (uint32_t)sizeof(T) : kOob;
     };
     T    g[IT];
     auto gather_issue = [&](const uint32_t *tab) {
+      const uint32_t ib = GRP ? ibase(tab) : 0u;
 #pragma unroll
       for (int j = 0; j < IT; ++j)
         {
           g[j] = T(0);
-          if (live(j))
-            g[j] = buf_ld(MODE == kChebInit ? r_a : rsrc, unit_offset(tab[item_slot(mw[j])], mw[j]), T());
+          if (GRP && j < JINT)
+            g[j] = buf_ld(MODE == kChebInit ? r_a : rsrc, tb, isoff(ib, j), T());
+          else if (live(j))
+            g[j] = buf_ld(MODE == kChebInit ? r_a : rsrc, unit_offset(tab[item_slot<GRP>(mw[j])], mw[j]), T());
         }
     };
     T    xs[kKeepX ? IT : 1];
@@ -299,7 +309,7 @@
           if (MODE == kChebInit)
             v = post.f0 * dv[kKeepX ? j : 0] * g[j];
           if (live(j))
-            U[item_point(mw[j])] = v;
+            U[item_point<GRP>(mw[j])] = v;
           if (kKeepX)
             xs[kKeepX ? j : 0] = v;
         }
@@ -314,7 +324,7 @@
           if (!kCarrier)
             continue;
 #ifndef MGX_MACRO_NOCARRIER
-          const uint32_t w    = live(j) ? E[item_slot(mw[j])] : kInvalid;
+          const uint32_t w    = live(j) ? Ec[item_slot<GRP>(mw[j])] : kInvalid;
           const bool     need = w != kInvalid && !(w & 0x40000000u);
           if (__builtin_amdgcn_ballot_w64(need) != 0)
             pp[j - JINT] = buf_ld(r_partial, need ? unit_offset(w, mw[j]) : kOob, T());
@@ -327,10 +337,16 @@
     auto           rhs_issue = [&]() {
       if (kRhs)
         {
+          const uint32_t ib = GRP ? ibase(Ec) : 0u;
 #pragma unroll
           for (int j = 0; j < IT; ++j)
             {
-              const uint32_t w    = live(j) ? E[item_slot(mw[j])] : kInvalid;
+              if (GRP && j < JINT)
+                {
+                  av[kRhs ? j : 0] = buf_ld(r_a, tb, isoff(ib, j), T());
+                  continue;
+                }
+              const uint32_t w    = live(j) ? Ec[item_slot<GRP>(mw[j])] : kInvalid;
               const bool     last = w != kInvalid && (j < JINT || (w >> 31));
               av[kRhs ? j : 0]    = buf_ld(r_a, last ? unit_offset(w, mw[j]) : kOob, T());
             }
@@ -343,6 +359,12 @@
       if (b + gridDim.x < brick_count)
         table_load(b + gridDim.x, en);
       table_store(E, e0);
+      if (GRP)
+        {
+          table_store(E + 32, en);
+          if (b + 2 * gridDim.x < brick_count)
+            table_load(b + 2 * gridDim.x, en);
+        }
       lds_barrier();
       MGX_STAMP(1);
       gather_issue(E);
@@ -383,10 +405,16 @@
         MGX_STAMP_IT(7);
         if (has_next)
           {
-            table_store(reinterpret_cast<uint32_t *>(U), en);
-            lds_barrier();
-            gather_issue(reinterpret_cast<const uint32_t *>(U));
-          }
+            if (GRP)
+              gather_issue(En);
+            else
+              {
+                table_store(reinterpret_cast<uint32_t *>(U), en);
+                lds_barrier();
+                gather_issue(reinterpret_cast<const uint32_t *>(U));
+              }
+          }
+        const uint32_t ibc = GRP ? ibase(Ec) : 0u;
         MGX_STAMP_IT(8);
 
         if constexpr (kKeepX)
@@ -403,8 +431,10 @@
               for (int k = 0; k < kChunk; ++k)
                 {
                   const int j = c * kChunk + k;
-                  if (j < IT)
-                    o[k].w = live(j) ? E[item_slot(mw[j])] : kInvalid;
+                  if (GRP && j < JINT)
+                    o[k].w = 0xC0000000u;
+                  else if (j < IT)
+                    o[k].w = live(j) ? Ec[item_slot<GRP>(mw[j])] : kInvalid;
                 }
 #pragma unroll
               for (int k = 0; k < kChunk; ++k)
@@ -412,6 +442,13 @@
                   const int j = c * kChunk + k;
                   if (j >= IT)
                     continue;
+                  if (GRP && j < JINT)
+                    {
+                      o[k].off = 0u;
+                      o[k].av  = buf_ld(r_a, tb, isoff(ibc, j), T());
+                      o[k].ov  = MODE == kCheb ? buf_ld(r_old, tb, isoff(ibc, j), T()) : T(0);
+                      continue;
+                    }
                   if (j < JINT && o[k].w != kInvalid)
                     o[k].w |= 0xC0000000u;
                   const bool last  = o[k].w != kInvalid && (o[k].w >> 31);
@@ -433,7 +470,7 @@
                 for (int k = 0; k < kChunk; ++k)
                   {
                     const int j = c * kChunk + k;
-                    val[k]      = (j < IT && live(j)) ? W[item_point(mw[j])] : T(0);
+                    val[k]      = (j < IT && live(j)) ? W[item_point<GRP>(mw[j])] : T(0);
                   }
 #pragma unroll
                 for (int k = 0; k < kChunk; ++k)
@@ -445,7 +482,9 @@
                     const bool vld = o.w != kInvalid, last = vld && (o.w >> 31);
                     const T    res = post_finish<T, MODE>(post, j >= JINT ? pp[j >= JINT ? j - JINT : 0] : T(0), o.av, o.ov,
                                                           dv[kKeepX ? j : 0], last, val[k], xs[kKeepX ? j : 0]);
-                    if (j < JINT)
+                    if (GRP && j < JINT)
+                      buf_st(r_out, tb, isoff(ibc, j), res);
+                    else if (j < JINT)
                       buf_st(r_out, o.off, res);
                     else
                       {
@@ -464,22 +503,31 @@
           {
             uint32_t w[IT];
   #pragma unroll
-            for (int j = 0; j < IT; ++j)
-              w[j] = live(j) ? E[item_slot(mw[j])] : kInvalid;
+            for (int j = GRP ? JINT : 0; j < IT; ++j)
+              w[j] = live(j) ? Ec[item_slot<GRP>(mw[j])] : kInvalid;
   #pragma unroll
             for (int j = 0; j < IT; ++j)
               {
+                if (GRP && j < JINT)
+                  {
+                    T val = W[item_point<GRP>(mw[j])];
+                    if (MODE == kResidualRestrict)
+                      W[item_point<GRP>(mw[j])] = av[kRhs ? j : 0] - val;
+                    else
+                      buf_st<kAuxNt>(r_out, tb, isoff(ibc, j), MODE == kResidual ? av[kRhs ? j : 0] - val : val);
+                    continue;
+                  }
                 if (j < JINT && w[j] != kInvalid)
                   w[j] |= 0xC0000000u;
                 const bool     vld = w[j] != kInvalid, last = vld && (w[j] >> 31);
                 const uint32_t off = unit_offset(w[j], mw[j]);
-                T              val = live(j) ? W[item_point(mw[j])] : T(0);
+                T              val = live(j) ? W[item_point<GRP>(mw[j])] : T(0);
                 if (j >= JINT && kCarrier)
                   val += pp[j >= JINT ? j - JINT : 0];
                 if (MODE == kResidualRestrict)
                   {
                     if (live(j))
-                      W[item_point(mw[j])] = vld ? (last ? av[kRhs ? j : 0] : T(0)) - val : T(0);
+                      W[item_point<GRP>(mw[j])] = vld ? (last ? av[kRhs ? j : 0] : T(0)) - val : T(0);
                     continue;
                   }
                 if (MODE == kResidual && last)
@@ -513,9 +561,21 @@
           break;
         lds_barrier();
         gather_land();
-        table_store(E, en);
-        if (bn + gridDim.x < brick_count)
-          table_load(bn + gridDim.x, en);
+        if (GRP)
+          {
+            table_store(const_cast<uint32_t *>(Ec), en);
+            if (bn + 2 * gridDim.x < brick_count)
+              table_load(bn + 2 * gridDim.x, en);
+            const uint32_t *t = Ec;
+            Ec                = En;
+            En                = t;
+          }
+        else
+          {
+            table_store(E, en);
+            if (bn + gridDim.x < brick_count)
+              table_load(bn + gridDim.x, en);
+          }
         MGX_STAMP_IT(10);
         lds_barrier();
         b = bn;
@@ -542,7 +602,7 @@
   }
 
   template <int P, typename T, int MODE>
-  static void macro2_launch(hipStream_t s, const OperatorData &op, const T *src, const BrickPost<T> &post, int g0, int g1)
+  static void macro2_launch(hipStream_t s, const OperatorData &op, const T *src, const BrickPost<T> &post, int g0, int g1, bool grp)
   {
     using C             = M2Cfg<P, T>;
     const BrickData &bd = op.bricks;
@@ -559,27 +619,33 @@
         if (count == 0)
           continue;
         const uint32_t grid = std::min<uint32_t>(count, (uint32_t)(op.macro_wg_x16 ? 1 : C::WGS) * macro2_cus(op));
-        hipLaunchKernelGGL((brick_macro2_kernel<P, T, MODE>), dim3(grid), dim3(C::THREADS), 0, s, src, first, count, bd.ent_base,
-                           bd.item_map2, (const Basis1D<T> *)op.basis, (T)op.coef[0], (T)op.coef[1], (T)op.coef[2], post,
-                           (uint32_t)(op.n_dofs * sizeof(T)));
+        if (grp)
+          hipLaunchKernelGGL((brick_macro2_kernel<P, T, MODE, true>), dim3(grid), dim3(C::THREADS), 0, s, src, first, count, bd.grp,
+                             bd.item_map_g, (const Basis1D<T> *)op.basis, (T)op.coef[0], (T)op.coef[1], (T)op.coef[2], post,
+                             (uint32_t)(op.n_dofs * sizeof(T)));
+        else
+          hipLaunchKernelGGL((brick_macro2_kernel<P, T, MODE>), dim3(grid), dim3(C::THREADS), 0, s, src, first, count, bd.ent_base,
+                             bd.item_map2, (const Basis1D<T> *)op.basis, (T)op.coef[0], (T)op.coef[1], (T)op.coef[2], post,
+                             (uint32_t)(op.n_dofs * sizeof(T)));
       }
   }
 
   template <int P, typename T>
-  static void macro2_modes(hipStream_t s, const OperatorData &op, int mode, const T *src, const BrickPost<T> &post, int g0, int g1)
+  static void macro2_modes(hipStream_t s, const OperatorData &op, int mode, const T *src, const BrickPost<T> &post, int g0, int g1,
+                           bool grp)
   {
     switch (mode)
       {
-        case kPlain: macro2_launch<P, T, kPlain>(s, op, src, post, g0, g1); break;
-        case kResidual: macro2_launch<P, T, kResidual>(s, op, src, post, g0, g1); break;
+        case kPlain: macro2_launch<P, T, kPlain>(s, op, src, post, g0, g1, grp); break;
+        case kResidual: macro2_launch<P, T, kResidual>(s, op, src, post, g0, g1, grp); break;
         case kChebInit:
           if constexpr (P <= 4)
-            macro2_launch<P, T, kChebInit>(s, op, src, post, g0, g1);
+            macro2_launch<P, T, kChebInit>(s, op, src, post, g0, g1, grp);
           break;
-        case kChebOldInit: macro2_launch<P, T, kChebOldInit>(s, op, src, post, g0, g1); break;
+        case kChebOldInit: macro2_launch<P, T, kChebOldInit>(s, op, src, post, g0, g1, grp); break;
         case kResidualRestrict:
           if constexpr (P <= 4)
-            macro2_launch<P, T, kResidualRestrict>(s, op, src, post, g0, g1);
+            macro2_launch<P, T, kResidualRestrict>(s, op, src, post, g0, g1, grp);
           break;
         default: break;
       }
@@ -596,8 +662,9 @@
       return false;
     if (is_cheb_mode(mode) && !op.diag_items2)
       return false;
+    const bool   grp = op.bricks.grp != nullptr;
     BrickPost<T> post{};
-    post.b   = (const T *)op.diag_items2;
+    post.b   = (const T *)(grp ? op.diag_items2_g : op.diag_items2);
     post.old = (const T *)old;
     post.f1  = (T)f1;
     post.f2  = (T)f2;
@@ -611,17 +678,17 @@
     switch (op.p)
       {
 #ifdef MGX_MACRO_ONLY_P
-        case MGX_MACRO_ONLY_P: macro2_modes<MGX_MACRO_ONLY_P, T>(s, op, mode, (const T *)src, post, g0, g1); break;
+        case MGX_MACRO_ONLY_P: macro2_modes<MGX_MACRO_ONLY_P, T>(s, op, mode, (const T *)src, post, g0, g1, grp); break;
 #else
-        case 1: macro2_modes<1, T>(s, op, mode, (const T *)src, post, g0, g1); break;
-        case 2: macro2_modes<2, T>(s, op, mode, (const T *)src, post, g0, g1); break;
-        case 3: macro2_modes<3, T>(s, op, mode, (const T *)src, post, g0, g1); break;
-        case 4: macro2_modes<4, T>(s, op, mode, (const T *)src, post, g0, g1); break;
-        case 5: macro2_modes<5, T>(s, op, mode, (const T *)src, post, g0, g1); break;
-        case 6: macro2_modes<6, T>(s, op, mode, (const T *)src, post, g0, g1); break;
-        case 7: macro2_modes<7, T>(s, op, mode, (const T *)src, post, g0, g1); break;
-        case 8: macro2_modes<8, T>(s, op, mode, (const T *)src, post, g0, g1); break;
-        case 9: macro2_modes<9, T>(s, op, mode, (const T *)src, post, g0, g1); break;
+        case 1: macro2_modes<1, T>(s, op, mode, (const T *)src, post, g0, g1, grp); break;
+        case 2: macro2_modes<2, T>(s, op, mode, (const T *)src, post, g0, g1, grp); break;
+        case 3: macro2_modes<3, T>(s, op, mode, (const T *)src, post, g0, g1, grp); break;
+        case 4: macro2_modes<4, T>(s, op, mode, (const T *)src, post, g0, g1, grp); break;
+        case 5: macro2_modes<5, T>(s, op, mode, (const T *)src, post, g0, g1, grp); break;
+        case 6: macro2_modes<6, T>(s, op, mode, (const T *)src, post, g0, g1, grp); break;
+        case 7: macro2_modes<7, T>(s, op, mode, (const T *)src, post, g0, g1, grp); break;
+        case 8: macro2_modes<8, T>(s, op, mode, (const T *)src, post, g0, g1, grp); break;
+        case 9: macro2_modes<9, T>(s, op, mode, (const T *)src, post, g0, g1, grp); break;
 #endif
         default: return false;
       }
diff --git a/multigrid_amd/csrc/mgx_macro_device.hpp b/multigrid_amd/csrc/mgx_macro_device.hpp
--- a/multigrid_amd/csrc/mgx_macro_device.hpp
+++ b/multigrid_amd/csrc/mgx_macro_device.hpp
@@ -280,6 +280,13 @@
   __device__ __forceinline__ uint32_t item_slot(uint32_t m) { return m & 1023u; }
   __device__ __forceinline__ uint32_t item_point(uint32_t m) { return (m >> 10) & 8191u; }
   __device__ __forceinline__ uint32_t item_offset(uint32_t m) { return m >> 23; }
+  template <bool GRP>
+  __device__ __forceinline__ uint32_t item_slot(uint32_t m) { return GRP ? (m & 31u) : item_slot(m); }
+  template <bool GRP>
+  __device__ __forceinline__ uint32_t item_point(uint32_t m) { return GRP ? (m >> 18) : item_point(m); }
+  template <bool GRP>
+  __device__ __forceinline__ uint32_t item_offset(uint32_t m) { return GRP ? ((m >> 5) & 8191u) : item_offset(m); }
+  constexpr int kGroupWords = 27;
 
   __host__ __device__ constexpr bool is_cheb_mode(int mode)
   {
@@ -301,6 +308,24 @@
   __device__ __forceinline__ float buf_ld(rsrc_t r, uint32_t off, float)
   {
     return __builtin_bit_cast(float, __builtin_amdgcn_raw_buffer_load_b32(r, off, 0, 0));
+  }
+  __device__ __forceinline__ double buf_ld(rsrc_t r, uint32_t off, uint32_t soff, double)
+  {
+    return __builtin_bit_cast(double, __builtin_amdgcn_raw_buffer_load_b64(r, off, soff, 0));
+  }
+  __device__ __forceinline__ float buf_ld(rsrc_t r, uint32_t off, uint32_t soff, float)
+  {
+    return __builtin_bit_cast(float, __builtin_amdgcn_raw_buffer_load_b32(r, off, soff, 0));
+  }
+  template <int AUX = 0>
+  __device__ __forceinline__ void buf_st(rsrc_t r, uint32_t off, uint32_t soff, double v)
+  {
+    __builtin_amdgcn_raw_buffer_store_b64(__builtin_bit_cast(u32x2_t, v), r, off, soff, AUX);
+  }
+  template <int AUX = 0>
+  __device__ __forceinline__ void buf_st(rsrc_t r, uint32_t off, uint32_t soff, float v)
+  {
+    __builtin_amdgcn_raw_buffer_store_b32(__builtin_bit_cast(unsigned int, v), r, off, soff, AUX);
   }
   template <int AUX = 0>
   __device__ __forceinline__ void buf_st(rsrc_t r, uint32_t off, double v)
```

Result: faster. 15.33 billion DoFs/s (median of 6 runs) (+3.3%).
